# MisEty/RTG-SLAM

Measured on AMD Instinct MI355X. Metric: hot_path_units_per_sec, higher is better.
Workload: dtype f32; 1 GPU; `value` counts UNITS, not SLAM frames (the SLAM frame rate by the reference's definition is `slam_frames_per_sec`, from the `slam_sequence` leg of --full).  One UNIT per step = 1 ICP track (3 levels x 5 GN iters, 1200x680, on a second HIP stream) + 1 map-optimisation iteration (raster fwd + masked L1 colour / gated depth loss + attach regulariser + raster bwd + fused Adam) over 1200000 random Gaus; gaussians=1200000, mode=single, parallelism=1 GPU

## Files before the change

### include/rtgs_raster.h

```cpp
#ifndef RTGS_RASTER_H
#define RTGS_RASTER_H

#include <stddef.h>
#include <stdint.h>

#ifdef __cplusplus
extern "C" {
#endif

#define RTGS_OK 0
#define RTGS_E_INVALID (-1)
#define RTGS_E_HIP (-2)
#define RTGS_E_ALLOC (-3)

#define RTGS_TILE 16

typedef struct rtgs_raster_settings {
  int32_t image_height;
  int32_t image_width;
  float tanfovx;
  float tanfovy;
  const float* bg;
  float scale_modifier;
  const float* viewmatrix;
// ... 100 lines not shown
                                  const int32_t* out_depth_index,
                                  const float* dL_dcolor, const float* dL_ddepth,
                                  float* dL_dmeans3D, float* dL_dopacities, float* dL_dshs,
                                  float* dL_dscales, float* dL_drotations, float* dL_dnormal_w,
                                  void* grad_scratch, uint8_t* row_state, int32_t train_begin, int32_t train_end, void* stream);
int rtgs_raster_backward_walk_ctx(rtgs_ctx* ctx, const rtgs_raster_settings* settings, int32_t P, int32_t sh_coeffs,
                                  int64_t num_rendered,
                                  const float* means3D, const float* opacities, const float* shs,
                                  const float* scales, const float* rotations, const float* normal_w,
                                  void* geom_buffer, void* binning_buffer,
                                  const void* image_buffer, const float* out_color, const float* out_T,
                                  const int32_t* out_depth_index,
                                  const float* dL_dcolor, const float* dL_ddepth,
                                  float* dL_dmeans3D, float* dL_dopacities, float* dL_dshs,
                                  float* dL_dscales, float* dL_drotations, float* dL_dnormal_w,
                                  void* grad_scratch, uint8_t* row_state, int32_t train_begin, int32_t train_end, void* stream);

size_t rtgs_raster_geom_bytes(int32_t P, int32_t image_height, int32_t image_width);
size_t rtgs_raster_geom_bytes_ctx(rtgs_ctx* ctx, int32_t P, int32_t image_height, int32_t image_width);
size_t rtgs_raster_binning_bytes(int64_t num_rendered, int32_t image_height, int32_t image_width);
size_t rtgs_raster_image_bytes(int32_t image_height, int32_t image_width);

int rtgs_raster_last_stats(int64_t* stats8_host);
int rtgs_raster_last_stats_ctx(rtgs_ctx* ctx, int64_t* stats8_host);

int rtgs_raster_last_slice_stats(int64_t* out4_host);
int rtgs_raster_last_slice_stats_ctx(rtgs_ctx* ctx, int64_t* out4_host);
int rtgs_raster_forward_verify_ctx(rtgs_ctx* ctx, int64_t* num_rendered_host);
const uint32_t* rtgs_raster_spec_fail_ptr_ctx(rtgs_ctx* ctx);
void rtgs_raster_set_speculation_ctx(rtgs_ctx* ctx, int enable);
int rtgs_raster_speculation_stats_ctx(rtgs_ctx* ctx, int64_t* out3_host);
void rtgs_raster_set_plain_onepass_ctx(rtgs_ctx* ctx, int enable);
int rtgs_raster_plain_stats_ctx(rtgs_ctx* ctx, int64_t* out2_host);
int rtgs_raster_image_offsets(int32_t image_height, int32_t image_width, size_t* out6_host);

int rtgs_fused_adam(float* params, const float* grads, float* exp_avg, float* exp_avg_sq,
                    const float* lr_per_column, int64_t rows, int32_t cols, int32_t step,
                    float beta1, float beta2, float eps, void* stream);

int rtgs_fused_adam_rows(float* params, const float* grads, float* exp_avg, float* exp_avg_sq,
                         const float* lr_per_column, uint8_t* ever_touched, const uint8_t* row_state, int64_t rows,
                         int32_t cols, int32_t step, float beta1, float beta2, float eps, void* stream);

int rtgs_map_activate8_forward(const float* raw8, int64_t n, float* opacity, float* scales, float* rotations,
                               float* normal, void* stream);
int rtgs_map_activate8_backward(const float* raw8, int64_t n, const float* g_opacity, const float* g_scales,
                                const float* g_rotations, const float* g_normal, float* g_raw8, void* stream);
int rtgs_map_activate8_backward_rows(const float* raw8, int64_t n, const float* g_opacity, const float* g_scales,
                                     const float* g_rotations, const float* g_normal, const uint8_t* row_state,
                                     float* g_raw8, void* stream);

typedef struct rtgs_attach {
  const float* init_xyz;
  const float* init_raw8;
  float* attach_info;
} rtgs_attach;
int rtgs_attach_prepare(const float* xyz, const float* raw8, const rtgs_attach* attach, int64_t rows, void* stream);

int rtgs_history_merge(float* xyz, float* shs, float* raw8, const float* then_xyz, const float* then_shs,
                       const float* then_raw8, const float* conf_then, const float* conf_now, int64_t rows,
                       float max_weight, void* stream);

typedef struct rtgs_activated {
  float *opacity, *scales, *rotations, *normal;
} rtgs_activated;
int rtgs_map_tail_rows(float* xyz, float* shs, float* raw8, const float* g_opacity, const float* g_scales,
                       const float* g_rotations, const float* g_normal, const float* g_xyz, const float* g_shs,
                       float* g_raw8, const uint8_t* row_state, float* m_xyz, float* v_xyz, float* m_shs, float* v_shs,
                       float* m_raw8, float* v_raw8, const float* lr_xyz, const float* lr_shs, const float* lr_raw8,
                       uint8_t* ever_xyz, uint8_t* ever_shs, uint8_t* ever_raw8, int64_t rows, int32_t step, float beta1,
                       float beta2, float eps, const rtgs_attach* attach, float* confidence, const uint32_t* skip_flag,
                       const rtgs_activated* refresh, void* stream);

typedef struct rtgs_loss_cfg {
  float color_weight, depth_weight, ssim_weight, add_depth_thres;
  const uint8_t* render_mask;
  int32_t sums_zeroed;
} rtgs_loss_cfg;
size_t rtgs_slam_loss_scratch_bytes(int32_t H, int32_t W, int32_t with_ssim);
int rtgs_slam_loss(const float* color, const float* depth, const int32_t* depth_index, const float* gt_color,
                   const float* gt_depth, int32_t H, int32_t W, const rtgs_loss_cfg* cfg, void* scratch,
                   float* loss_out4, float* g_color, float* g_depth, void* stream);
int rtgs_slam_loss_sums(const float* color, const float* depth, const int32_t* depth_index, const float* gt_color,
                        const float* gt_depth, int32_t H, int32_t W, const rtgs_loss_cfg* cfg, void* scratch, void* stream);
int rtgs_slam_loss_grads(const float* color, const float* depth, const int32_t* depth_index, const float* gt_color,
                         const float* gt_depth, int32_t H, int32_t W, const rtgs_loss_cfg* cfg, void* scratch,
                         float* loss_out4, float* g_color, float* g_depth, void* stream);

typedef struct rtgs_map_step_args {
  const rtgs_raster_settings* settings;
  int32_t P, sh_coeffs;
  float *xyz, *shs, *raw8;
  const int32_t* tile_mask;
  const float *gt_color, *gt_depth;
  rtgs_loss_cfg loss;
  void* loss_scratch;
  float *opacity, *scales, *rotations, *normal;
  float *out_color, *out_depth;
  int32_t *out_color_index, *out_depth_index;
  float *out_color_weight, *out_depth_weight, *out_T;
  int32_t* out_radii;
  float *dL_dcolor, *dL_ddepth, *loss4;
  float *d_xyz, *d_opacity, *d_shs, *d_scales, *d_rotations, *d_normal, *d_raw8;
  void* grad_scratch;
  uint8_t* row_state;
  float *m_xyz, *v_xyz, *m_shs, *v_shs, *m_raw8, *v_raw8;
  const float *lr_xyz, *lr_shs, *lr_raw8;
  uint8_t *ever_xyz, *ever_shs, *ever_raw8;
  int32_t step;
  float beta1, beta2, eps;
  const rtgs_attach* attach;
  float* confidence;
  int32_t activated_valid;
  rtgs_resize_fn geom_resize; void* geom_user;
  rtgs_resize_fn binning_resize; void* binning_user;
  rtgs_resize_fn image_resize; void* image_user;
  float normal_weight;
  const float* gt_normal;
  int32_t train_begin, train_end;
  int32_t tail_mode;
  uint32_t* live_counts;
} rtgs_map_step_args;
int rtgs_slam_normal_loss(const float* normal_w, const int32_t* depth_index, const float* gt_normal,
                          const uint8_t* render_mask, int32_t H, int32_t W, float normal_weight, float* scratch2,
                          float* loss_out4, float* d_normal, uint8_t* row_state, const uint32_t* skip_flag, void* stream);
int rtgs_slam_normal_loss_range(const float* normal_w, const int32_t* depth_index, const float* gt_normal,
                                const uint8_t* render_mask, int32_t H, int32_t W, float normal_weight, float* scratch2,
                                float* loss_out4, float* d_normal, uint8_t* row_state, const uint32_t* skip_flag,
                                int32_t train_begin, int32_t train_end, void* stream);
int rtgs_slam_normal_loss_sums(const float* normal_w, const int32_t* depth_index, const float* gt_normal,
                               const uint8_t* render_mask, int32_t H, int32_t W, float* scratch2, const uint32_t* skip_flag,
                               void* stream);
int rtgs_slam_normal_loss_grads(const float* normal_w, const int32_t* depth_index, const float* gt_normal,
                                const uint8_t* render_mask, int32_t H, int32_t W, float normal_weight, const float* sums2,
                                float* loss_out4, float* d_normal, uint8_t* row_state, const uint32_t* skip_flag,
                                int32_t train_begin, int32_t train_end, void* stream);
int rtgs_slam_map_step(const rtgs_map_step_args* args, int64_t* num_rendered_host, void* stream);
void* rtgs_stream_create_reserving(int32_t reserve_cus);
void rtgs_stream_destroy(void* stream);
int rtgs_map_fused_tail(const rtgs_raster_settings* settings, const rtgs_map_step_args* args, void* geom_buffer,
                        const void* image_buffer, const uint32_t* spec_fail, uint32_t* live_counts2, void* stream);
int rtgs_map_fused_tail_hint(const rtgs_raster_settings* settings, const rtgs_map_step_args* args, void* geom_buffer,
                             const void* image_buffer, const uint32_t* spec_fail, uint32_t* live_counts2,
                             uint32_t listed_hint, void* stream);
uint32_t rtgs_raster_last_listed_ctx(rtgs_ctx* ctx);
int rtgs_raster_backward_buffers(int32_t P, int32_t image_height, int32_t image_width, size_t* out8_host);
int rtgs_raster_last_buffers_ctx(rtgs_ctx* ctx, void** out3_host);
void rtgs_raster_set_aux_zero_ctx(rtgs_ctx* ctx, void* eight_words);
int rtgs_slam_map_step_front(const rtgs_map_step_args* args, int64_t* num_rendered_host, void* stream);
int rtgs_slam_map_step_ctx(rtgs_ctx* ctx, const rtgs_map_step_args* args, int64_t* num_rendered_host, void* stream);
int rtgs_slam_map_step_front_ctx(rtgs_ctx* ctx, const rtgs_map_step_args* args, int64_t* num_rendered_host, void* stream);

int rtgs_rows_pack(const uint8_t* row_state, int32_t P, float* d_xyz, float* d_shs, float* d_opacity, float* d_scales,
                   float* d_rotations, float* d_normal, float* out_list, int32_t capacity, uint32_t* count_scratch,
                   void* stream);
int rtgs_rows_overflow(const float* gathered_lists, int32_t world, int32_t capacity, uint32_t* flag_and_counts, void* stream);
int rtgs_rows_apply(const float* list, int32_t capacity, int32_t mode, float* d_xyz, float* d_shs, float* d_opacity,
                    float* d_scales, float* d_rotations, float* d_normal, uint8_t* row_state, const uint32_t* skip_flag,
                    void* stream);

size_t rtgs_map_step_args_size(void);
size_t rtgs_raster_settings_size(void);

const char* rtgs_version(void);

#ifdef __cplusplus
}
#endif
#endif
```

### rtg_slam_amd/_lib.py

```python
from __future__ import annotations

import ctypes as C
import os
import threading

_HERE = os.path.dirname(os.path.abspath(__file__))
LIB_PATH = os.environ.get("RTGS_LIB_PATH") or os.path.join(_HERE, "librtgs_hip.so")

RESIZE_FN = C.CFUNCTYPE(C.c_void_p, C.c_void_p, C.c_size_t)
FWD_NO_BACKWARD = 1


class RasterSettingsC(C.Structure):
    _fields_ = [
        ("image_height", C.c_int32), ("image_width", C.c_int32),
        ("tanfovx", C.c_float), ("tanfovy", C.c_float),
        ("bg", C.c_void_p), ("scale_modifier", C.c_float),
        ("viewmatrix", C.c_void_p), ("projmatrix", C.c_void_p),
        ("sh_degree", C.c_int32), ("campos", C.c_void_p),
        ("opaque_threshold", C.c_float), ("depth_threshold", C.c_float),
        ("normal_threshold", C.c_float), ("color_sigma", C.c_float),
        ("prefiltered", C.c_int32), ("debug", C.c_int32),
        ("cx", C.c_float), ("cy", C.c_float), ("T_threshold", C.c_float),
    ]
# ... 12 lines not shown

_P = C.c_void_p


class LossCfgC(C.Structure):
    _fields_ = [("color_weight", C.c_float), ("depth_weight", C.c_float), ("ssim_weight", C.c_float),
                ("add_depth_thres", C.c_float), ("render_mask", C.c_void_p), ("sums_zeroed", C.c_int32)]


class AttachC(C.Structure):
    _fields_ = [("init_xyz", C.c_void_p), ("init_raw8", C.c_void_p), ("attach_info", C.c_void_p)]


class ActivatedC(C.Structure):
    _fields_ = [(n, C.c_void_p) for n in ("opacity", "scales", "rotations", "normal")]


class MapStepArgsC(C.Structure):
    _fields_ = (
        [("settings", C.POINTER(RasterSettingsC)), ("P", C.c_int32), ("sh_coeffs", C.c_int32)]
        + [(n, C.c_void_p) for n in ("xyz", "shs", "raw8", "tile_mask", "gt_color", "gt_depth")]
        + [("loss", LossCfgC), ("loss_scratch", C.c_void_p)]
        + [(n, C.c_void_p) for n in (
            "opacity", "scales", "rotations", "normal", "out_color", "out_depth", "out_color_index", "out_depth_index",
            "out_color_weight", "out_depth_weight", "out_T", "out_radii", "dL_dcolor", "dL_ddepth", "loss4",
            "d_xyz", "d_opacity", "d_shs", "d_scales", "d_rotations", "d_normal", "d_raw8", "grad_scratch", "row_state",
            "m_xyz", "v_xyz", "m_shs", "v_shs", "m_raw8", "v_raw8", "lr_xyz", "lr_shs", "lr_raw8",
            "ever_xyz", "ever_shs", "ever_raw8")]
        + [("step", C.c_int32), ("beta1", C.c_float), ("beta2", C.c_float), ("eps", C.c_float)]
        + [("attach", C.POINTER(AttachC)), ("confidence", C.c_void_p), ("activated_valid", C.c_int32)]
        + [("geom_resize", RESIZE_FN), ("geom_user", C.c_void_p), ("binning_resize", RESIZE_FN),
           ("binning_user", C.c_void_p), ("image_resize", RESIZE_FN), ("image_user", C.c_void_p)]
        + [("normal_weight", C.c_float), ("gt_normal", C.c_void_p), ("train_begin", C.c_int32), ("train_end", C.c_int32),
           ("tail_mode", C.c_int32), ("live_counts", C.c_void_p)])


_SIGNATURES = {
    "rtgs_version": (C.c_char_p, []),
    "rtgs_raster_forward": (C.c_int, [C.POINTER(RasterSettingsC), C.c_int32, C.c_int32] + [_P] * 6 + [_P]
                            + [_P] * 8 + [RESIZE_FN, _P, RESIZE_FN, _P, RESIZE_FN, _P,
                                          C.POINTER(C.c_int64), _P]),
    "rtgs_raster_backward": (C.c_int, [C.POINTER(RasterSettingsC), C.c_int32, C.c_int32, C.c_int64] + [_P] * 6
                             + [_P] * 3 + [_P, _P, _P] + [_P, _P] + [_P] * 6 + [_P, _P]),
    "rtgs_raster_backward_rows": (C.c_int, [C.POINTER(RasterSettingsC), C.c_int32, C.c_int32, C.c_int64] + [_P] * 6
                                  + [_P] * 3 + [_P, _P, _P] + [_P, _P] + [_P] * 6 + [_P, _P, _P]),
    "rtgs_raster_backward_scratch_bytes": (C.c_size_t, [C.c_int32]),
    "rtgs_raster_geom_bytes": (C.c_size_t, [C.c_int32, C.c_int32, C.c_int32]),
    "rtgs_raster_binning_bytes": (C.c_size_t, [C.c_int64, C.c_int32, C.c_int32]),
    "rtgs_raster_image_bytes": (C.c_size_t, [C.c_int32, C.c_int32]),
    "rtgs_raster_last_stats": (C.c_int, [C.POINTER(C.c_int64)]),
    "rtgs_raster_set_counters": (None, [_P]),
    "rtgs_fused_adam": (C.c_int, [_P, _P, _P, _P, _P, C.c_int64, C.c_int32, C.c_int32, C.c_float, C.c_float, C.c_float, _P]),
    "rtgs_fused_adam_rows": (C.c_int, [_P, _P, _P, _P, _P, _P, _P, C.c_int64, C.c_int32, C.c_int32, C.c_float, C.c_float, C.c_float, _P]),
    "rtgs_map_activate8_forward": (C.c_int, [_P, C.c_int64, _P, _P, _P, _P, _P]),
    "rtgs_map_activate8_backward": (C.c_int, [_P, C.c_int64, _P, _P, _P, _P, _P, _P]),
    "rtgs_map_activate8_backward_rows": (C.c_int, [_P, C.c_int64, _P, _P, _P, _P, _P, _P, _P]),
    "rtgs_map_tail_rows": (C.c_int, [_P] * 23 + [C.c_int64, C.c_int32, C.c_float, C.c_float, C.c_float,
                                     C.POINTER(AttachC), _P, _P, C.POINTER(ActivatedC), _P]),
    "rtgs_attach_prepare": (C.c_int, [_P, _P, C.POINTER(AttachC), C.c_int64, _P]),
    "rtgs_history_merge": (C.c_int, [_P] * 8 + [C.c_int64, C.c_float, _P]),
    "rtgs_map_fused_tail": (C.c_int, [C.POINTER(RasterSettingsC), C.POINTER(MapStepArgsC), _P, _P, _P, _P, _P]),
    "rtgs_map_fused_tail_hint": (C.c_int, [C.POINTER(RasterSettingsC), C.POINTER(MapStepArgsC), _P, _P, _P, _P, C.c_uint32, _P]),
    "rtgs_raster_last_listed_ctx": (C.c_uint32, [_P]),
    "rtgs_stream_create_reserving": (C.c_void_p, [C.c_int]),
    "rtgs_stream_destroy": (None, [_P]),
    "rtgs_raster_backward_buffers": (C.c_int, [C.c_int32, C.c_int32, C.c_int32, C.POINTER(C.c_size_t)]),
    "rtgs_raster_last_buffers_ctx": (C.c_int, [_P, C.POINTER(C.c_void_p)]),
    "rtgs_raster_set_aux_zero_ctx": (None, [_P, _P]),
    "rtgs_raster_backward_walk_ctx": (C.c_int, [_P, C.POINTER(RasterSettingsC), C.c_int32, C.c_int32, C.c_int64] + [_P] * 6
                                      + [_P] * 3 + [_P, _P, _P] + [_P, _P] + [_P] * 6 + [_P, _P, C.c_int32, C.c_int32, _P]),
    "rtgs_slam_loss_scratch_bytes": (C.c_size_t, [C.c_int32, C.c_int32, C.c_int32]),
    "rtgs_slam_map_step_front": (C.c_int, [C.POINTER(MapStepArgsC), C.POINTER(C.c_int64), _P]),
    "rtgs_rows_pack": (C.c_int, [_P, C.c_int32] + [_P] * 7 + [C.c_int32, _P, _P]),
    "rtgs_rows_overflow": (C.c_int, [_P, C.c_int32, C.c_int32, _P, _P]),
    "rtgs_rows_apply": (C.c_int, [_P, C.c_int32, C.c_int32] + [_P] * 7 + [_P, _P]),
    "rtgs_map_step_args_size": (C.c_size_t, []),
    "rtgs_raster_settings_size": (C.c_size_t, []),
    "rtgs_slam_map_step": (C.c_int, [C.POINTER(MapStepArgsC), C.POINTER(C.c_int64), _P]),
    "rtgs_slam_loss": (C.c_int, [_P, _P, _P, _P, _P, C.c_int32, C.c_int32, C.POINTER(LossCfgC), _P, _P, _P, _P, _P]),
    "rtgs_slam_normal_loss": (C.c_int, [_P, _P, _P, _P, C.c_int32, C.c_int32, C.c_float, _P, _P, _P, _P, _P, _P]),
    "rtgs_slam_loss_sums": (C.c_int, [_P, _P, _P, _P, _P, C.c_int32, C.c_int32, C.POINTER(LossCfgC), _P, _P]),
    "rtgs_slam_loss_grads": (C.c_int, [_P, _P, _P, _P, _P, C.c_int32, C.c_int32, C.POINTER(LossCfgC), _P, _P, _P, _P, _P]),
    "rtgs_raster_set_profiling": (None, [C.c_int]),
    "rtgs_raster_force_sort_path": (None, [C.c_int]),
    "rtgs_raster_set_near_slice": (None, [C.c_int, C.c_int]),
    "rtgs_raster_last_slice_stats": (C.c_int, [C.POINTER(C.c_int64)]),
    "rtgs_raster_last_timings": (C.c_int, [C.POINTER(C.c_float)]),
    "rtgs_ctx_create": (C.c_void_p, []),
    "rtgs_ctx_destroy": (None, [_P]),
    "rtgs_raster_forward_ctx": (C.c_int, [_P, C.POINTER(RasterSettingsC), C.c_int32, C.c_int32] + [_P] * 6 + [_P]
                                + [_P] * 8 + [RESIZE_FN, _P, RESIZE_FN, _P, RESIZE_FN, _P, C.POINTER(C.c_int64),
                                              C.c_int32, _P]),
    "rtgs_raster_backward_ctx": (C.c_int, [_P, C.POINTER(RasterSettingsC), C.c_int32, C.c_int32, C.c_int64] + [_P] * 6
                                 + [_P] * 3 + [_P, _P, _P] + [_P, _P] + [_P] * 6 + [_P, _P]),
    "rtgs_raster_backward_rows_ctx": (C.c_int, [_P, C.POINTER(RasterSettingsC), C.c_int32, C.c_int32, C.c_int64] + [_P] * 6
                                      + [_P] * 3 + [_P, _P, _P] + [_P, _P] + [_P] * 6 + [_P, _P, _P]),
# ... 141 lines not shown
```

### rtg_slam_amd/csrc/map_fused.hip

```cpp
#include "../../include/rtgs_raster.h"
#include "raster_common.h"
#include "raster_chain.h"
#include "adam_common.h"
#include "activate_common.h"

#include <math.h>

namespace rtgs {

struct FusedArgs {
  RasterParams p;
  const float *opac, *scales, *rots, *normal_w;
  const uint8_t* clamped;
  const BwdInfo* info;
  const uint32_t* gbase;
  uint32_t* slot_count;
  uint8_t* touched;
  SplatGrad* records;
  float *xyz, *shs, *raw8;
  float *m_xyz, *v_xyz, *m_shs, *v_shs, *m_raw8, *v_raw8;
  const float *lr_xyz, *lr_shs, *lr_raw8;
  uint8_t *ever_xyz, *ever_shs, *ever_raw8;
  float beta1, beta2, eps, bc1, bc2_sqrt;
  const float* init_xyz;
  const float4* init_raw8;
  const float* attach_info;
  float* confidence;
  float *act_opacity, *act_scales, *act_normal;
  float4* act_rots;
  uint32_t* live_counts;
  int t0, rows;
};

constexpr int BIG_RUN = 8;

__device__ __forceinline__ bool attach_sel(const float4 init_lo) {
  return 1.f / (1.f + __expf(-init_lo.x)) < 0.9f;
}

template <int FCHUNK, int RPW = 64>
__global__ void __launch_bounds__(256) map_fused_tail_kernel(FusedArgs a) {
  __shared__ uint32_t s_list[FCHUNK];
  __shared__ uint32_t s_n;
  __shared__ float s_big[4][64][16];
  __shared__ float s_sh[4][64][20];
  __shared__ int s_rows[4][64];
  if (spec_failed(a.p.spec_fail)) return;
  const int tid = threadIdx.x, lane = tid & 63, wv = tid >> 6;
  const bool use_slots = a.info->use_slots != 0;
  const float* __restrict__ slots = reinterpret_cast<const float*>(a.info->slot_grads);
  uint32_t n_grad = 0, n_step = 0;
  for (int c0 = blockIdx.x * FCHUNK; c0 < a.rows; c0 += gridDim.x * FCHUNK) {
    __syncthreads();
    if (tid == 0) s_n = 0;
    __syncthreads();
    constexpr int PASSES = FCHUNK >= 256 ? FCHUNK / 256 : 1;
    uint32_t flags = 0;
#pragma unroll
    for (int k = 0; k < PASSES; ++k) {
      const int rl = min(c0 + k * 256 + tid, a.rows - 1);
      const uint32_t f = (uint32_t)a.touched[a.t0 + rl] | (uint32_t)a.ever_raw8[rl] | (uint32_t)a.ever_xyz[rl] | (uint32_t)a.ever_shs[rl];
      flags |= (f != 0u ? 1u : 0u) << k;
    }
// ... 84 lines not shown
      } else if (rgrad) {
        g = a.records[r];
        float4* z = reinterpret_cast<float4*>(a.records + r);
        z[0] = z[1] = z[2] = z[3] = make_float4(0.f, 0.f, 0.f, 0.f);
      }
      if (rgrad) {
        a.touched[r] = 0;
        rgrad = (g.du != 0.f) | (g.dv != 0.f) | (g.dca != 0.f) | (g.dcb != 0.f) | (g.dcc != 0.f) | (g.dop != 0.f) |
                (g.dr != 0.f) | (g.dg != 0.f) | (g.db != 0.f) | (g.dnx != 0.f) | (g.dny != 0.f) | (g.dnz != 0.f) | (g.dpd != 0.f);
      }
      bool need_sh = false;
      if (have) {
        const uint8_t e_raw8 = a.ever_raw8[rl], e_xyz = a.ever_xyz[rl], e_shs = a.ever_shs[rl];
        ChainOut o{};
        if (rgrad) chain_rule(a.p, r, a.xyz, a.shs, a.scales, a.rots, a.normal_w, a.clamped, g, o, nullptr);
        const float4* raw8_4 = reinterpret_cast<const float4*>(a.raw8);
        float4 at_lo = make_float4(0.f, 0.f, 0.f, 0.f), at_hi = at_lo;
        float at[3] = {0.f, 0.f, 0.f};
        bool sel = false;
        if (a.init_raw8 && (rgrad || e_raw8 != 0 || e_xyz != 0)) {
          const float4 i_lo = a.init_raw8[2 * (size_t)rl];
          sel = attach_sel(i_lo);
          if (sel) {
            const float4 i_hi = a.init_raw8[2 * (size_t)rl + 1], c_lo = raw8_4[2 * (size_t)r], c_hi = raw8_4[2 * (size_t)r + 1];
            const float n = fmaxf(a.attach_info[0], 1.f);
            const float k3 = 2000.f / (n * 3.f), k4 = 2000.f / (n * 4.f);
            at_lo = make_float4(0.f, k3 * (c_lo.y - i_lo.y), k3 * (c_lo.z - i_lo.z), k3 * (c_lo.w - i_lo.w));
            at_hi = make_float4(k4 * (c_hi.x - i_hi.x), k4 * (c_hi.y - i_hi.y), k4 * (c_hi.z - i_hi.z), k4 * (c_hi.w - i_hi.w));
#pragma unroll
            for (int c = 0; c < 3; ++c) at[c] = k3 * (a.xyz[(size_t)r * 3 + c] - a.init_xyz[(size_t)rl * 3 + c]);
          }
        }
        const bool grad = rgrad || sel;
        if (grad || e_raw8 != 0) {
          float4 lo = make_float4(0.f, 0.f, 0.f, 0.f), hi = lo;
          if (rgrad)
            activate8_bwd_row(raw8_4[2 * (size_t)r], raw8_4[2 * (size_t)r + 1], o.dop, o.ds[0], o.ds[1], o.ds[2], o.dq, o.dn[0],
                              o.dn[1], o.dn[2], lo, hi);
          lo.y += at_lo.y; lo.z += at_lo.z; lo.w += at_lo.w;
          hi.x += at_hi.x; hi.y += at_hi.y; hi.z += at_hi.z; hi.w += at_hi.w;
          if (e_raw8 == 0) a.ever_raw8[rl] = 1;
          float4* p4 = reinterpret_cast<float4*>(a.raw8) + 2 * (size_t)r;
          float4* m4 = reinterpret_cast<float4*>(a.m_raw8) + 2 * (size_t)rl;
          float4* v4 = reinterpret_cast<float4*>(a.v_raw8) + 2 * (size_t)rl;
          const float gg[8] = {lo.x, lo.y, lo.z, lo.w, hi.x, hi.y, hi.z, hi.w};
          float4 pp[2] = {p4[0], p4[1]}, mm[2] = {m4[0], m4[1]}, vv[2] = {v4[0], v4[1]};
          float* pf = reinterpret_cast<float*>(pp); float* mf = reinterpret_cast<float*>(mm); float* vf = reinterpret_cast<float*>(vv);
#pragma unroll
          for (int c = 0; c < 8; ++c) pf[c] = adam1(pf[c], gg[c], mf[c], vf[c], a.lr_raw8[c], a.beta1, a.beta2, a.eps, a.bc1, a.bc2_sqrt);
          p4[0] = pp[0]; p4[1] = pp[1]; m4[0] = mm[0]; m4[1] = mm[1]; v4[0] = vv[0]; v4[1] = vv[1];
          if (a.act_opacity) activate8_row_store(pp[0], pp[1], r, a.act_opacity, a.act_scales, a.act_rots, a.act_normal);
        }
        if (grad || e_xyz != 0) {
          if (e_xyz == 0) a.ever_xyz[rl] = 1;
#pragma unroll
          for (int c = 0; c < 3; ++c) {
            const size_t op = (size_t)r * 3 + c, os = (size_t)rl * 3 + c;
            float mi = a.m_xyz[os], vi = a.v_xyz[os];
            a.xyz[op] = adam1(a.xyz[op], (rgrad ? o.dm[c] : 0.f) + at[c], mi, vi, a.lr_xyz[c], a.beta1, a.beta2, a.eps, a.bc1, a.bc2_sqrt);
            a.m_xyz[os] = mi; a.v_xyz[os] = vi;
          }
        }
        if (a.confidence && rgrad) {
          if (o.basis[0] * o.gc[0] != 0.f || o.basis[0] * o.gc[1] != 0.f || o.basis[0] * o.gc[2] != 0.f) a.confidence[rl] += 1.f;
        }
        need_sh = rgrad || e_shs != 0;
// ... 30 lines not shown
            gi.w = sh[3 + (c0 + 3) / 3] * sh[(c0 + 3) % 3];
          }
          const float4 pi = reinterpret_cast<const float4*>(a.shs)[op];
          float4 mi = reinterpret_cast<float4*>(a.m_shs)[os], vi = reinterpret_cast<float4*>(a.v_shs)[os], po;
          po.x = adam1(pi.x, gi.x, mi.x, vi.x, a.lr_shs[4 * sub], a.beta1, a.beta2, a.eps, a.bc1, a.bc2_sqrt);
          po.y = adam1(pi.y, gi.y, mi.y, vi.y, a.lr_shs[4 * sub + 1], a.beta1, a.beta2, a.eps, a.bc1, a.bc2_sqrt);
          po.z = adam1(pi.z, gi.z, mi.z, vi.z, a.lr_shs[4 * sub + 2], a.beta1, a.beta2, a.eps, a.bc1, a.bc2_sqrt);
          po.w = adam1(pi.w, gi.w, mi.w, vi.w, a.lr_shs[4 * sub + 3], a.beta1, a.beta2, a.eps, a.bc1, a.bc2_sqrt);
          reinterpret_cast<float4*>(a.shs)[op] = po;
          reinterpret_cast<float4*>(a.m_shs)[os] = mi;
          reinterpret_cast<float4*>(a.v_shs)[os] = vi;
        }
      }
      __builtin_amdgcn_wave_barrier();
    }
  }
  if (a.live_counts) {
#pragma unroll
    for (int off = 32; off > 0; off >>= 1) { n_grad += (uint32_t)__shfl_xor((int)n_grad, off); n_step += (uint32_t)__shfl_xor((int)n_step, off); }
    if (lane == 0 && (n_grad | n_step)) { atomicAdd(&a.live_counts[0], n_grad); atomicAdd(&a.live_counts[1], n_step); }
  }
}

}

extern "C" int rtgs_map_fused_tail(const rtgs_raster_settings* settings, const rtgs_map_step_args* s, void* geom_buffer,
                                   const void* image_buffer, const uint32_t* spec_fail, uint32_t* live_counts2, void* stream) {
  return rtgs_map_fused_tail_hint(settings, s, geom_buffer, image_buffer, spec_fail, live_counts2, 0, stream);
}

extern "C" int rtgs_map_fused_tail_hint(const rtgs_raster_settings* settings, const rtgs_map_step_args* s, void* geom_buffer,
                                        const void* image_buffer, const uint32_t* spec_fail, uint32_t* live_counts2,
                                        uint32_t listed_hint, void* stream) {
  using namespace rtgs;
  if (!settings || !s || !geom_buffer || !image_buffer) return RTGS_E_INVALID;
  const int32_t P = s->P;
  if (P <= 0 || s->sh_coeffs != 16 || s->step < 1) return RTGS_E_INVALID;
  int32_t t0 = 0, t1 = P;
  if (s->train_begin != 0 || s->train_end != 0) { t0 = s->train_begin; t1 = s->train_end; }
  if (t0 < 0 || t1 > P || t1 < t0) return RTGS_E_INVALID;
  if (t1 == t0) return RTGS_OK;
  FusedArgs a{};
  RasterParams& p = a.p;
  p.H = settings->image_height; p.W = settings->image_width;
  p.gx = (p.W + TILE - 1) / TILE; p.gy = (p.H + TILE - 1) / TILE;
  p.P = P; p.M = 16; p.deg = settings->sh_degree;
  p.tanfovx = settings->tanfovx; p.tanfovy = settings->tanfovy;
  p.fx = (float)(p.W / (2.0 * (double)settings->tanfovx));
  p.fy = (float)(p.H / (2.0 * (double)settings->tanfovy));
  p.cx = settings->cx > 0.f ? settings->cx : 0.5f * (float)(p.W - 1);
  p.cy = settings->cy > 0.f ? settings->cy : 0.5f * (float)(p.H - 1);
  p.scale_modifier = settings->scale_modifier;
  p.opaque_thr = settings->opaque_threshold; p.depth_thr = settings->depth_threshold; p.normal_thr = settings->normal_threshold;
  p.color_sigma = settings->color_sigma; p.T_thr = settings->T_threshold;
  p.view = settings->viewmatrix; p.campos = settings->campos; p.bg = settings->bg;
  p.spec_fail = spec_fail;
  size_t off[8];
  if (rtgs_raster_backward_buffers(P, p.H, p.W, off) != RTGS_OK) return RTGS_E_INVALID;
  const char* geom = (const char*)geom_buffer;
  const char* img = (const char*)image_buffer;
  a.opac = s->opacity; a.scales = s->scales; a.rots = s->rotations; a.normal_w = s->normal;
  a.clamped = (const uint8_t*)(geom + off[0]);
  a.gbase = (const uint32_t*)(geom + off[1]);
  a.slot_count = (uint32_t*)(geom + off[2]);
  a.info = (const BwdInfo*)(img + off[3]);
  a.records = (SplatGrad*)s->grad_scratch;
  a.touched = (uint8_t*)s->grad_scratch + off[4];
  a.xyz = s->xyz; a.shs = s->shs; a.raw8 = s->raw8;
  a.m_xyz = s->m_xyz; a.v_xyz = s->v_xyz; a.m_shs = s->m_shs; a.v_shs = s->v_shs; a.m_raw8 = s->m_raw8; a.v_raw8 = s->v_raw8;
  a.lr_xyz = s->lr_xyz; a.lr_shs = s->lr_shs; a.lr_raw8 = s->lr_raw8;
  a.ever_xyz = s->ever_xyz; a.ever_shs = s->ever_shs; a.ever_raw8 = s->ever_raw8;
  a.beta1 = s->beta1; a.beta2 = s->beta2; a.eps = s->eps;
  a.bc1 = 1.f - powf(s->beta1, (float)s->step);
  a.bc2_sqrt = sqrtf(1.f - powf(s->beta2, (float)s->step));
  if (s->attach) {
    if (!s->attach->init_xyz || !s->attach->init_raw8 || !s->attach->attach_info) return RTGS_E_INVALID;
    a.init_xyz = s->attach->init_xyz; a.init_raw8 = (const float4*)s->attach->init_raw8; a.attach_info = s->attach->attach_info;
  }
  a.confidence = s->confidence;
  a.act_opacity = s->opacity; a.act_scales = s->scales; a.act_normal = s->normal; a.act_rots = (float4*)s->rotations;
  a.live_counts = live_counts2;
  a.t0 = t0; a.rows = t1 - t0;
  static const int forced = [] { const char* e = getenv("RTGS_FUSED_CHUNK"); return e ? atoi(e) : 0; }();
  int chunk = 1024;
  if (forced == 512 || forced == 1024 || forced == 2048) chunk = forced;
  else if (listed_hint > 0u) {
    const double per_row = (double)listed_hint / (double)(P > 0 ? P : 1);
    chunk = per_row * 2048.0 <= 64.0 ? 2048 : (per_row * 1024.0 <= 64.0 ? 1024 : 512);
  }
  if (forced == 64 || (forced == 0 && a.rows <= 65536)) chunk = 64;
  int blocks = (a.rows + chunk - 1) / chunk;
  if (blocks > 4096) blocks = 4096;
  if (chunk == 64) hipLaunchKernelGGL((map_fused_tail_kernel<64, 16>), dim3(blocks), dim3(256), 0, (hipStream_t)stream, a);
  else if (chunk == 2048) hipLaunchKernelGGL(map_fused_tail_kernel<2048>, dim3(blocks), dim3(256), 0, (hipStream_t)stream, a);
  else if (chunk == 512) hipLaunchKernelGGL(map_fused_tail_kernel<512>, dim3(blocks), dim3(256), 0, (hipStream_t)stream, a);
  else hipLaunchKernelGGL(map_fused_tail_kernel<1024>, dim3(blocks), dim3(256), 0, (hipStream_t)stream, a);
  return hipGetLastError() == hipSuccess ? RTGS_OK : RTGS_E_HIP;
}
```

### rtg_slam_amd/csrc/map_ops.hip

```cpp
#include "../../include/rtgs_raster.h"
#include <hip/hip_runtime.h>
#include <math.h>
#include <stdint.h>
#include "adam_common.h"
#include "activate_common.h"


namespace rtgs {

__global__ void __launch_bounds__(256) activate8_fwd_kernel(const float4* __restrict__ raw8, int64_t n,
                                                            float* __restrict__ opacity, float* __restrict__ scales,
                                                            float4* __restrict__ rots, float* __restrict__ normal) {
  for (int64_t i = (int64_t)blockIdx.x * blockDim.x + threadIdx.x; i < n; i += (int64_t)gridDim.x * blockDim.x)
    activate8_row_store(raw8[2 * i], raw8[2 * i + 1], i, opacity, scales, rots, normal);
}

__global__ void __launch_bounds__(256) activate8_bwd_kernel(const float4* __restrict__ raw8, int64_t n,
                                                            const float* __restrict__ g_op, const float* __restrict__ g_sc,
                                                            const float4* __restrict__ g_rot, const float* __restrict__ g_nrm,
                                                            const uint8_t* __restrict__ row_state,
                                                            float4* __restrict__ g_raw8) {
  for (int64_t i = (int64_t)blockIdx.x * blockDim.x + threadIdx.x; i < n; i += (int64_t)gridDim.x * blockDim.x) {
    if (row_state) {
      const uint8_t s = row_state[i];
// ... 37 lines not shown
                                                const float* g_rotations, const float* g_normal, const uint8_t* row_state,
                                                float* g_raw8, void* stream) {
  if (n < 0 || (n > 0 && (!raw8 || !g_opacity || !g_scales || !g_rotations || !g_normal || !row_state || !g_raw8))) return -1;
  if (n == 0) return 0;
  int64_t blocks = (n + 255) / 256;
  if (blocks > 8192) blocks = 8192;
  hipLaunchKernelGGL(rtgs::activate8_bwd_kernel, dim3((unsigned)blocks), dim3(256), 0, (hipStream_t)stream,
                     (const float4*)raw8, n, g_opacity, g_scales, (const float4*)g_rotations, g_normal, row_state,
                     (float4*)g_raw8);
  return hipGetLastError() == hipSuccess ? 0 : -2;
}

namespace rtgs {

struct TailArgs {
  const float4* raw8_in;
  float *xyz, *shs, *raw8;
  const float *g_op, *g_sc, *g_nrm, *g_xyz, *g_shs;
  const float4* g_rot;
  float4* g_raw8;
  const uint8_t* row_state;
  float *m_xyz, *v_xyz, *m_shs, *v_shs, *m_raw8, *v_raw8;
  const float *lr_xyz, *lr_shs, *lr_raw8;
  uint8_t *ever_xyz, *ever_shs, *ever_raw8;
  long long rows;
  float beta1, beta2, eps, bc1, bc2_sqrt;
  const float* init_xyz;
  const float4* init_raw8;
  const float* attach_info;
  float* confidence;
  const uint32_t* skip_flag;
  float *act_opacity, *act_scales, *act_normal;
  float4* act_rots;
};

__device__ __forceinline__ bool attach_selected(const float4 init_lo) {
  return 1.f / (1.f + __expf(-init_lo.x)) < 0.9f;
}

__global__ void __launch_bounds__(256) map_tail_rows_kernel(TailArgs a) {
  __shared__ int s_rows[4][64];
  if (a.skip_flag && a.skip_flag[0] != 0u) return;
  const int lane = threadIdx.x & 63, wv = threadIdx.x >> 6;
  const long long wave0 = (long long)blockIdx.x * 4 + wv, nwaves = (long long)gridDim.x * 4;
  for (long long base = wave0 * 64; base < a.rows; base += nwaves * 64) {
    const long long r = base + lane;
    bool need_sh = false, has_grad = false;
    if (r < a.rows) {
      const uint8_t st = a.row_state[r];
      const uint8_t e_raw8 = a.ever_raw8[r], e_xyz = a.ever_xyz[r], e_shs = a.ever_shs[r];
      const bool rgrad = st == 1;
      has_grad = rgrad;
      float4 at_lo = make_float4(0.f, 0.f, 0.f, 0.f), at_hi = at_lo;
      float at_x = 0.f, at_y = 0.f, at_z = 0.f;
      bool sel = false;
      if (a.init_raw8 && (rgrad || e_raw8 != 0 || e_xyz != 0)) {
        const float4 i_lo = a.init_raw8[2 * r];
        sel = attach_selected(i_lo);
        if (sel) {
          const float4 i_hi = a.init_raw8[2 * r + 1], c_lo = a.raw8_in[2 * r], c_hi = a.raw8_in[2 * r + 1];
          const float n = fmaxf(a.attach_info[0], 1.f);
          const float k3 = 2000.f / (n * 3.f), k4 = 2000.f / (n * 4.f);
          at_lo = make_float4(0.f, k3 * (c_lo.y - i_lo.y), k3 * (c_lo.z - i_lo.z), k3 * (c_lo.w - i_lo.w));
          at_hi = make_float4(k4 * (c_hi.x - i_hi.x), k4 * (c_hi.y - i_hi.y), k4 * (c_hi.z - i_hi.z), k4 * (c_hi.w - i_hi.w));
          at_x = k3 * (a.xyz[(size_t)r * 3] - a.init_xyz[(size_t)r * 3]);
          at_y = k3 * (a.xyz[(size_t)r * 3 + 1] - a.init_xyz[(size_t)r * 3 + 1]);
          at_z = k3 * (a.xyz[(size_t)r * 3 + 2] - a.init_xyz[(size_t)r * 3 + 2]);
        }
      }
      const bool grad = rgrad || sel;
      float4 lo = make_float4(0.f, 0.f, 0.f, 0.f), hi = lo;
      if (st != 0 || sel) {
        if (rgrad)
          activate8_bwd_row(a.raw8_in[2 * r], a.raw8_in[2 * r + 1], a.g_op[r], a.g_sc[r * 3], a.g_sc[r * 3 + 1],
                            a.g_sc[r * 3 + 2], a.g_rot[r], a.g_nrm[r * 3], a.g_nrm[r * 3 + 1], a.g_nrm[r * 3 + 2], lo, hi);
        lo.y += at_lo.y; lo.z += at_lo.z; lo.w += at_lo.w;
        hi.x += at_hi.x; hi.y += at_hi.y; hi.z += at_hi.z; hi.w += at_hi.w;
        a.g_raw8[2 * r] = lo; a.g_raw8[2 * r + 1] = hi;
      }
      if (grad || e_raw8 != 0) {
        if (e_raw8 == 0) a.ever_raw8[r] = 1;
        const float4 g0 = lo, g1 = hi;
        float4* p4 = reinterpret_cast<float4*>(a.raw8) + 2 * r;
        float4* m4 = reinterpret_cast<float4*>(a.m_raw8) + 2 * r;
        float4* v4 = reinterpret_cast<float4*>(a.v_raw8) + 2 * r;
        const float gg[8] = {g0.x, g0.y, g0.z, g0.w, g1.x, g1.y, g1.z, g1.w};
        float4 pp[2] = {p4[0], p4[1]}, mm[2] = {m4[0], m4[1]}, vv[2] = {v4[0], v4[1]};
        float* pf = reinterpret_cast<float*>(pp); float* mf = reinterpret_cast<float*>(mm); float* vf = reinterpret_cast<float*>(vv);
#pragma unroll
        for (int c = 0; c < 8; ++c) pf[c] = adam1(pf[c], gg[c], mf[c], vf[c], a.lr_raw8[c], a.beta1, a.beta2, a.eps, a.bc1, a.bc2_sqrt);
        p4[0] = pp[0]; p4[1] = pp[1]; m4[0] = mm[0]; m4[1] = mm[1]; v4[0] = vv[0]; v4[1] = vv[1];
        if (a.act_opacity) activate8_row_store(pp[0], pp[1], r, a.act_opacity, a.act_scales, a.act_rots, a.act_normal);
      }
      if (grad || e_xyz != 0) {
        if (e_xyz == 0) a.ever_xyz[r] = 1;
        const float at[3] = {at_x, at_y, at_z};
#pragma unroll
        for (int c = 0; c < 3; ++c) {
          const size_t o = (size_t)r * 3 + c;
          float mi = a.m_xyz[o], vi = a.v_xyz[o];
          a.xyz[o] = adam1(a.xyz[o], (rgrad ? a.g_xyz[o] : 0.f) + at[c], mi, vi, a.lr_xyz[c], a.beta1, a.beta2, a.eps, a.bc1, a.bc2_sqrt);
          a.m_xyz[o] = mi; a.v_xyz[o] = vi;
        }
      }
      if (a.confidence && rgrad) {
        const size_t o = (size_t)r * 48;
        if (a.g_shs[o] != 0.f || a.g_shs[o + 1] != 0.f || a.g_shs[o + 2] != 0.f) a.confidence[r] += 1.f;
      }
      need_sh = rgrad || e_shs != 0;
      if (need_sh && e_shs == 0) a.ever_shs[r] = 1;
    }
    const unsigned long long mask = __builtin_amdgcn_ballot_w64(need_sh);
// ... 121 lines not shown
  if (!xyz || !shs || !raw8 || !then_xyz || !then_shs || !then_raw8 || !conf_then || !conf_now) return -1;
  long long blocks = (rows + 255) / 256;
  if (blocks > 8192) blocks = 8192;
  hipLaunchKernelGGL(rtgs::history_merge_kernel, dim3((unsigned)blocks), dim3(256), 0, (hipStream_t)stream, xyz, (float4*)shs,
                     (float4*)raw8, then_xyz, (const float4*)then_shs, (const float4*)then_raw8, conf_then, conf_now,
                     (long long)rows, max_weight);
  return hipGetLastError() == hipSuccess ? 0 : -2;
}

extern "C" int rtgs_attach_prepare(const float* xyz, const float* raw8, const rtgs_attach* attach, int64_t rows, void* stream) {
  if (!attach || !attach->init_xyz || !attach->init_raw8 || !attach->attach_info || rows < 0) return -1;
  if (rows > 0 && (!xyz || !raw8)) return -1;
  hipStream_t st = (hipStream_t)stream;
  float* info = attach->attach_info;
  if (hipMemsetAsync(info, 0, 6 * sizeof(float), st) != hipSuccess) return -2;
  if (rows > 0) {
    long long blocks = (rows + 255) / 256;
    if (blocks > 192) blocks = 192;
    hipLaunchKernelGGL(rtgs::attach_sums_kernel, dim3((unsigned)blocks), dim3(256), 0, st, xyz, (const float4*)raw8,
                       attach->init_xyz, (const float4*)attach->init_raw8, (long long)rows, info + 2);
  }
  hipLaunchKernelGGL(rtgs::attach_finish_kernel, dim3(1), dim3(1), 0, st, (const float*)(info + 2), info);
  return hipGetLastError() == hipSuccess ? 0 : -2;
}

extern "C" int rtgs_map_tail_rows(float* xyz, float* shs, float* raw8, const float* g_opacity, const float* g_scales,
                                  const float* g_rotations, const float* g_normal, const float* g_xyz, const float* g_shs,
                                  float* g_raw8, const uint8_t* row_state, float* m_xyz, float* v_xyz, float* m_shs,
                                  float* v_shs, float* m_raw8, float* v_raw8, const float* lr_xyz, const float* lr_shs,
                                  const float* lr_raw8, uint8_t* ever_xyz, uint8_t* ever_shs, uint8_t* ever_raw8,
                                  int64_t rows, int32_t step, float beta1, float beta2, float eps,
                                  const rtgs_attach* attach, float* confidence, const uint32_t* skip_flag,
                                  const rtgs_activated* refresh, void* stream) {
  if (rows < 0 || step < 1) return -1;
  if (rows == 0) return 0;
  if (!xyz || !shs || !raw8 || !g_opacity || !g_scales || !g_rotations || !g_normal || !g_xyz || !g_shs || !g_raw8 ||
      !row_state || !m_xyz || !v_xyz || !m_shs || !v_shs || !m_raw8 || !v_raw8 || !lr_xyz || !lr_shs || !lr_raw8 ||
      !ever_xyz || !ever_shs || !ever_raw8)
    return -1;
  rtgs::TailArgs a;
  a.raw8_in = (const float4*)raw8; a.xyz = xyz; a.shs = shs; a.raw8 = raw8;
  a.g_op = g_opacity; a.g_sc = g_scales; a.g_nrm = g_normal; a.g_xyz = g_xyz; a.g_shs = g_shs;
  a.g_rot = (const float4*)g_rotations; a.g_raw8 = (float4*)g_raw8; a.row_state = row_state;
  a.m_xyz = m_xyz; a.v_xyz = v_xyz; a.m_shs = m_shs; a.v_shs = v_shs; a.m_raw8 = m_raw8; a.v_raw8 = v_raw8;
  a.lr_xyz = lr_xyz; a.lr_shs = lr_shs; a.lr_raw8 = lr_raw8;
  a.ever_xyz = ever_xyz; a.ever_shs = ever_shs; a.ever_raw8 = ever_raw8;
  a.rows = rows; a.beta1 = beta1; a.beta2 = beta2; a.eps = eps;
  a.init_xyz = nullptr; a.init_raw8 = nullptr; a.attach_info = nullptr; a.confidence = confidence;
  a.skip_flag = skip_flag;
  a.act_opacity = a.act_scales = a.act_normal = nullptr; a.act_rots = nullptr;
  if (refresh) {
    if (!refresh->opacity || !refresh->scales || !refresh->rotations || !refresh->normal) return -1;
    a.act_opacity = refresh->opacity; a.act_scales = refresh->scales; a.act_normal = refresh->normal;
    a.act_rots = (float4*)refresh->rotations;
  }
  if (attach) {
    if (!attach->init_xyz || !attach->init_raw8 || !attach->attach_info) return -1;
    a.init_xyz = attach->init_xyz; a.init_raw8 = (const float4*)attach->init_raw8; a.attach_info = attach->attach_info;
  }
  a.bc1 = 1.f - powf(beta1, (float)step);
  a.bc2_sqrt = sqrtf(1.f - powf(beta2, (float)step));
  long long blocks = (rows + 255) / 256;
  if (blocks > 16384) blocks = 16384;
  hipLaunchKernelGGL(rtgs::map_tail_rows_kernel, dim3((unsigned)blocks), dim3(256), 0, (hipStream_t)stream, a);
  return hipGetLastError() == hipSuccess ? 0 : -2;
}

namespace rtgs {

constexpr int PACK_CHUNK = 8192;
constexpr int ROW_WORDS = 64;

struct ArenaPtrs {
  float *d_xyz, *d_shs, *d_opac, *d_scales, *d_rots, *d_normal;
};
__device__ __forceinline__ float* arena_word(const ArenaPtrs& a, uint32_t id, int w) {
  if (w < 4) return a.d_xyz + (size_t)id * 3 + (w - 1);
  if (w < 52) return a.d_shs + (size_t)id * 48 + (w - 4);
  if (w < 53) return a.d_opac + id;
  if (w < 56) return a.d_scales + (size_t)id * 3 + (w - 53);
  if (w < 60) return a.d_rots + (size_t)id * 4 + (w - 56);
  return a.d_normal + (size_t)id * 3 + (w - 60);
// ... 515 lines not shown
```

### rtg_slam_amd/csrc/map_step.hip

```cpp
#include <hip/hip_runtime.h>

#include "../../include/rtgs_raster.h"

static int map_step_front(rtgs_ctx* ctx, const rtgs_map_step_args* a, int64_t* num_rendered_host, int32_t fwd_flags,
                          void* stream, bool walk_only = false) {
  if (!a || !num_rendered_host || !a->settings) return RTGS_E_INVALID;
  const int32_t P = a->P, M = a->sh_coeffs;
  if (P <= 0 || M != 16 || a->step < 1) return RTGS_E_INVALID;
  if (!a->xyz || !a->shs || !a->raw8 || !a->tile_mask || !a->gt_color || !a->gt_depth) return RTGS_E_INVALID;
  const int32_t H = a->settings->image_height, W = a->settings->image_width;
  int rc = 0;
  if (!a->activated_valid) {
    rc = rtgs_map_activate8_forward(a->raw8, P, a->opacity, a->scales, a->rotations, a->normal, stream);
    if (rc != 0) return RTGS_E_HIP;
  }
  if (!a->loss_scratch || !a->loss4) return RTGS_E_INVALID;
  rtgs_raster_set_aux_zero_ctx(ctx, a->loss_scratch);
  rc = rtgs_raster_forward_ctx(ctx, a->settings, P, M, a->xyz, a->opacity, a->shs, a->scales, a->rotations, a->normal,
                           a->tile_mask, a->out_color, a->out_depth, a->out_color_index, a->out_depth_index,
                           a->out_color_weight, a->out_depth_weight, a->out_T, a->out_radii, a->geom_resize,
                           a->geom_user, a->binning_resize, a->binning_user, a->image_resize, a->image_user,
                           num_rendered_host, fwd_flags, stream);
  if (rc != RTGS_OK) return rc;
  void* bufs[3];
// ... 3 lines not shown
  lcfg.sums_zeroed = P > 0 ? 1 : 0;
  rc = rtgs_slam_loss(a->out_color, a->out_depth, a->out_depth_index, a->gt_color, a->gt_depth, H, W, &lcfg,
                      a->loss_scratch, a->loss4, a->dL_dcolor, a->dL_ddepth, stream);
  if (rc != 0) return RTGS_E_HIP;
  int32_t t0 = 0, t1 = P;
  if (a->train_begin != 0 || a->train_end != 0) { t0 = a->train_begin; t1 = a->train_end; }
  if (t0 < 0 || t1 > P || t1 < t0) return RTGS_E_INVALID;
  if (t1 == t0) return RTGS_OK;
  rc = (walk_only ? rtgs_raster_backward_walk_ctx : rtgs_raster_backward_range_ctx)(
      ctx, a->settings, P, M, *num_rendered_host, a->xyz, a->opacity, a->shs, a->scales, a->rotations, a->normal, geom, bin, img,
      a->out_color, a->out_T, a->out_depth_index, a->dL_dcolor, a->dL_ddepth, a->d_xyz, a->d_opacity, a->d_shs, a->d_scales,
      a->d_rotations, a->d_normal, a->grad_scratch, a->row_state, t0, t1, stream);
  if (rc != RTGS_OK) return rc;
  if (a->normal_weight > 0.f && a->gt_normal) {
    rc = rtgs_slam_normal_loss_range(a->normal, a->out_depth_index, a->gt_normal, a->loss.render_mask, H, W, a->normal_weight,
                                     reinterpret_cast<float*>(a->loss_scratch) + 5, a->loss4, a->d_normal, a->row_state,
                                     rtgs_raster_spec_fail_ptr_ctx(ctx), t0, t1, stream);
    if (rc != 0) return RTGS_E_HIP;
  }
  return RTGS_OK;
}

extern "C" int rtgs_slam_map_step_front_ctx(rtgs_ctx* ctx, const rtgs_map_step_args* a, int64_t* num_rendered_host,
                                            void* stream) {
  return map_step_front(ctx, a, num_rendered_host, 0, stream);
}

extern "C" int rtgs_slam_map_step_front(const rtgs_map_step_args* a, int64_t* num_rendered_host, void* stream) {
  return rtgs_slam_map_step_front_ctx(nullptr, a, num_rendered_host, stream);
}

static int map_step_once(rtgs_ctx* ctx, const rtgs_map_step_args* a, int64_t* num_rendered_host, bool speculate, void* stream) {
  const bool fused = a->tail_mode == 0 && !(a->normal_weight > 0.f && a->gt_normal);
  int rc = map_step_front(ctx, a, num_rendered_host, speculate ? RTGS_FWD_SPECULATE : 0, stream, fused);
  if (rc != RTGS_OK) return rc;
  if ((a->train_begin != 0 || a->train_end != 0) && a->train_end == a->train_begin) return RTGS_OK;
  if (fused) {
    void* bufs[3];
    if (rtgs_raster_last_buffers_ctx(ctx, bufs) != RTGS_OK) return RTGS_E_ALLOC;
    return rtgs_map_fused_tail_hint(a->settings, a, bufs[0], bufs[2], rtgs_raster_spec_fail_ptr_ctx(ctx), a->live_counts,
                                    rtgs_raster_last_listed_ctx(ctx), stream);
  }
  const int32_t P = a->P;
  int32_t t0 = 0, t1 = P;
  if (a->train_begin != 0 || a->train_end != 0) { t0 = a->train_begin; t1 = a->train_end; }
  const size_t o = (size_t)t0;
  const rtgs_activated act{a->opacity + o, a->scales + 3 * o, a->rotations + 4 * o, a->normal + 3 * o};
  rc = rtgs_map_tail_rows(a->xyz + 3 * o, a->shs + 48 * o, a->raw8 + 8 * o, a->d_opacity + o, a->d_scales + 3 * o,
                          a->d_rotations + 4 * o, a->d_normal + 3 * o, a->d_xyz + 3 * o, a->d_shs + 48 * o, a->d_raw8 + 8 * o,
                          a->row_state + o, a->m_xyz, a->v_xyz, a->m_shs, a->v_shs, a->m_raw8, a->v_raw8,
                          a->lr_xyz, a->lr_shs, a->lr_raw8, a->ever_xyz, a->ever_shs, a->ever_raw8, (int64_t)(t1 - t0), a->step,
                          a->beta1, a->beta2, a->eps, a->attach, a->confidence, rtgs_raster_spec_fail_ptr_ctx(ctx), &act, stream);
  return rc != 0 ? RTGS_E_HIP : RTGS_OK;
}

extern "C" int rtgs_slam_map_step_ctx(rtgs_ctx* ctx, const rtgs_map_step_args* a, int64_t* num_rendered_host, void* stream) {
  int rc = map_step_once(ctx, a, num_rendered_host, true, stream);
  const int v = rtgs_raster_forward_verify_ctx(ctx, num_rendered_host);
  if (rc != RTGS_OK) return rc;
  if (v < 0) return v;
  if (v == 1) rc = map_step_once(ctx, a, num_rendered_host, false, stream);
  return rc;
}

extern "C" int rtgs_slam_map_step(const rtgs_map_step_args* a, int64_t* num_rendered_host, void* stream) {
  return rtgs_slam_map_step_ctx(nullptr, a, num_rendered_host, stream);
}

extern "C" size_t rtgs_map_step_args_size(void) { return sizeof(rtgs_map_step_args); }
extern "C" size_t rtgs_raster_settings_size(void) { return sizeof(rtgs_raster_settings); }

extern "C" void* rtgs_stream_create_reserving(int32_t reserve_cus) {
  int dev = 0, cus = 0;
  if (hipGetDevice(&dev) != hipSuccess) return nullptr;
  if (hipDeviceGetAttribute(&cus, hipDeviceAttributeMultiprocessorCount, dev) != hipSuccess) return nullptr;
  if (reserve_cus <= 0 || reserve_cus >= cus || cus > 1024) return nullptr;
  uint32_t mask[32] = {0};
  const int words = (cus + 31) / 32;
  for (int i = 0; i < cus - reserve_cus; ++i) mask[i >> 5] |= 1u << (i & 31);
  hipStream_t s = nullptr;
  if (hipExtStreamCreateWithCUMask(&s, (uint32_t)words, mask) != hipSuccess) return nullptr;
  return (void*)s;
}
extern "C" void rtgs_stream_destroy(void* stream) {
  if (stream) (void)hipStreamDestroy((hipStream_t)stream);
// ... 2 lines not shown
```

### rtg_slam_amd/csrc/raster_api.hip

```cpp
#include "../../include/rtgs_raster.h"
#include "../../include/rtgs_debug.h"
#include "raster_common.h"

#include <rocprim/device/device_radix_sort.hpp>
#include <rocprim/device/device_scan.hpp>
#include <math.h>
#include <new>
#include <stdlib.h>
#include <string.h>

namespace rtgs {
void launch_mask_sat(const int32_t*, int, int, int32_t*, hipStream_t);
void launch_preprocess_fwd(const RasterParams&, const float*, const float*, const float*, const float*, const float*,
                           const float*, const int32_t*, Splat*, uint32_t*, int32_t*, uint8_t*, int32_t*, uint32_t*, int,
                           uint8_t*, hipStream_t);
void launch_emit_keys(const RasterParams&, const Splat*, const int32_t*, const uint32_t*, const int32_t*, uint64_t*,
                      uint32_t*, hipStream_t);
void launch_tile_ranges(int64_t, const uint64_t*, uint2*, hipStream_t);
void set_fwd_stamps(void* dev);
void set_bwd_debug(int bits);
void set_bwd_stamps(void* dev);
void launch_blend_fwd(const RasterParams&, const uint2*, const uint32_t*, const Splat*, float*, float*, int32_t*,
                      int32_t*, float*, float*, float*, uint32_t*, unsigned long long*, SlicePass, uint32_t*, uint32_t*, uint32_t*, int, uint32_t*,
                      TileCache, uint32_t, hipStream_t);
void launch_blend_bwd(const RasterParams&, const uint2*, const uint32_t*, const Splat*, const float*, const float*,
                      const uint32_t*, const int32_t*, const float*, const float*, const uint32_t*, uint32_t*,
                      const BwdInfo*, SplatGrad*, uint8_t*, const uint32_t*, int, uint32_t, uint32_t, hipStream_t);
void launch_blend_bwd_entry(const RasterParams&, const uint2*, const uint32_t*, const Splat*, const float*, const uint32_t*,
                            const int32_t*, const uint32_t*, const uint32_t*, const float*, const float*, const uint32_t*, uint32_t*,
                            const BwdInfo*, SplatGrad*, uint8_t*, const uint32_t*, uint32_t, uint32_t, TileCache, uint32_t, hipStream_t);
void launch_grad_reduce(int, const uint8_t*, const uint32_t*, uint32_t*, const BwdInfo*, SplatGrad*, const uint32_t*, hipStream_t);
void launch_preprocess_bwd(const RasterParams&, const float*, const float*, const float*, const float*, const float*,
                           const float*, const int32_t*, const uint8_t*, SplatGrad*, uint8_t*, uint8_t*, float*, float*,
                           float*, float*, float*, float*, hipStream_t);

size_t bin_lds_limit_tiles();
int bin_sort_capacity();
size_t bin_block_counts_bytes(int, int);
int launch_bin_count(const RasterParams&, const Splat*, const int32_t*, const int32_t*, uint32_t*, uint16_t*, SliceSel,
                     SliceList, size_t, hipStream_t);
size_t bin_slice_block_counts_bytes(int, size_t, int);
size_t bin_list_block_counts_bytes(int, int);
void launch_visible_compact(int, const uint8_t*, uint32_t*, uint32_t*, const uint32_t*, uint32_t*, uint32_t*, const uint32_t*, hipStream_t,
                            const SliceSel* = nullptr, int32_t* = nullptr, uint32_t* = nullptr);
void launch_slice_compact(int, SliceSel, uint32_t*, uint32_t*, const uint32_t*, uint32_t*, uint32_t*, uint32_t*, uint32_t, uint32_t*, hipStream_t);
void launch_slice_publish(int, const int32_t*, const int32_t*, const uint32_t*, uint32_t*, uint32_t*, uint32_t, uint32_t*, hipStream_t,
                          const uint32_t* seg_count = nullptr);
void launch_preprocess_cull(const RasterParams&, const float*, const float*, const float*, uint32_t*, int32_t*, int32_t*,
                            uint32_t*, int, uint8_t*, float2*, hipStream_t);
void launch_preprocess_shade(const RasterParams&, const float*, const float*, const float*, const float*, const float*,
                             const float*, Splat*, int32_t*, uint8_t*, float2*, SliceList, SliceSel, size_t, hipStream_t);
void launch_bin_tilescan(int, const uint32_t*, uint2*, uint32_t*, uint32_t*, uint32_t*, const uint32_t*, const uint32_t*,
                         const uint32_t*, const uint32_t*, uint32_t, SpecCaps, hipStream_t);
void launch_bin_scatter(const RasterParams&, const Splat*, const int32_t*, const int32_t*, const uint16_t*, uint32_t*,
                        unsigned long long*, SliceSel, SliceList, size_t, hipStream_t);
void launch_slice_hist(int, const uint8_t*, const uint32_t*, const int32_t*, uint32_t*, unsigned long long*, hipStream_t,
                       BwdInfoInit bi = BwdInfoInit{nullptr, nullptr, 0u, 0u});
void launch_bin_tilesort(int, uint32_t, const uint2*, const unsigned long long*, uint32_t*, const uint32_t*, hipStream_t,
                         const uint32_t* seg_count = nullptr, uint32_t seg = 0, uint2* ranges_out = nullptr,
                         const BinFinish* finish = nullptr);
void launch_bin_place(const RasterParams&, const Splat*, const int32_t*, const int32_t*, uint32_t*, unsigned long long*, uint32_t,
                      uint32_t*, SliceSel, SliceList, size_t, hipStream_t);

}

enum { EV_F0 = 0, EV_PRE, EV_SL_BIN, EV_SL_BLEND, EV_SCAN, EV_BIN0, EV_EMIT, EV_SORT, EV_RANGES, EV_BLEND0, EV_BLEND, EV_B0,
       EV_BWALK, EV_BBLEND, EV_BPRE, EV_N };
struct rtgs_ctx {
  int64_t stats[8] = {0};
  int slice_mode = 2;
  int slice_budget = 384;
  int64_t slice_stats[4] = {0};
  unsigned long long* counters = nullptr;
  uint32_t last_listed = 0;
  bool onepass = true;
  bool prof = false;
  bool force_sort_path = false;
  int bwd_walk = 0;
  bool ev_init = false;
  hipEvent_t ev[EV_N];
  bool ev_set[EV_N] = {false};
  uint32_t* info_host = nullptr;
// ... 4 lines not shown
  void *last_geom = nullptr, *last_bin = nullptr, *last_img = nullptr;
  uint32_t* aux_zero = nullptr;
  bool ask_first = false;
  struct Plan {
    bool valid = false;
    int32_t P = 0, H = 0, W = 0;
    int kind = -1;
    int slice_mode = 0, slice_budget = 0;
    uint32_t R = 0, R1 = 0, longest = 0, slots = 0, n_fin = 0;
    uint32_t R_hi = 0, longest_hi = 0, slots_hi = 0;
    void note(uint32_t r, uint32_t l, uint32_t s) {
      R = r; longest = l; slots = s;
      R_hi = r > R_hi - R_hi / 16 ? r : R_hi - R_hi / 16;
      longest_hi = l > longest_hi - longest_hi / 16 ? l : longest_hi - longest_hi / 16;
      slots_hi = s > slots_hi - slots_hi / 16 ? s : slots_hi - slots_hi / 16;
    }
  } plan;
  struct Spec {
    bool pending = false;
    int kind = -1;
    uint32_t seq = 0, capR = 0, capL = 0, capS = 0;
    const void* geom = nullptr;
    const uint32_t* fail_dev = nullptr;
    void* stream = nullptr;
    int32_t ntiles = 0;
    int64_t G_total = 0, B_total = 0, I_total = 0;
  } spec;
  bool speculation = true;
  int64_t spec_stats[3] = {0, 0, 0};
  Plan plan_plain;
  Plan plan_plain0;
  bool plain_onepass = true;
  int64_t plain_stats[2] = {0, 0};
};

namespace rtgs {

static rtgs_ctx* default_ctx() {
  static rtgs_ctx* c = [] {
    rtgs_ctx* n = new rtgs_ctx();
    if (const char* e = getenv("RTGS_NEAR_SLICE")) n->slice_mode = atoi(e);
    if (const char* e = getenv("RTGS_NEAR_SLICE_BUDGET")) { const int b = atoi(e); if (b > 0) n->slice_budget = b; }
    if (const char* e = getenv("RTGS_SPECULATE")) n->speculation = atoi(e) != 0;
    if (const char* e = getenv("RTGS_BIN_ONEPASS")) n->onepass = atoi(e) != 0;
    if (const char* e = getenv("RTGS_PLAIN_ONEPASS")) n->plain_onepass = atoi(e) != 0;
    if (const char* e = getenv("RTGS_BWD_WALK")) { const int m = atoi(e); n->bwd_walk = (m >= 1 && m <= 4) ? m : 0; }
    return n;
  }();
  return c;
}
static inline rtgs_ctx* use(rtgs_ctx* c) { return c ? c : default_ctx(); }

static void prof_mark(rtgs_ctx* c, int which, hipStream_t st) {
  if (!c->prof) return;
  if (!c->ev_init) {
    for (int i = 0; i < EV_N; ++i) (void)hipEventCreate(&c->ev[i]);
    c->ev_init = true;
  }
  (void)hipEventRecord(c->ev[which], st);
  c->ev_set[which] = true;
}

static int bits_for(uint32_t n) {
  int b = 0;
  while ((1ull << b) < (unsigned long long)n) ++b;
  return b < 1 ? 1 : b;
}

static int wait_published_words(uint32_t* info_host, uint32_t seq, hipStream_t st, uint32_t (&pub)[7]) {
  volatile uint32_t* h = info_host;
  auto snapshot_ok = [&]() -> bool {
    if (h[7] != seq) return false;
    __atomic_thread_fence(__ATOMIC_ACQUIRE);
    uint32_t w[7];
    for (int k = 0; k < 7; ++k) w[k] = h[k];
    if (h[8] != host_checksum(seq, w)) return false;
    for (int k = 0; k < 7; ++k) pub[k] = w[k];
    return true;
  };
// ... 11 lines not shown
  for (uint32_t c : classes) if (want <= c) return c;
  return 16384u;
}

__global__ void bwd_info_kernel(BwdInfo* dst, SplatGrad* slot_grads, uint32_t slots, uint32_t use_slots) {
  dst->slot_grads = slot_grads; dst->slots = slots; dst->use_slots = use_slots;
}

static int large_map_min() {
  static const int v = [] { const char* e = getenv("RTGS_LARGE_MAP_MIN"); const int x = e ? atoi(e) : 100000; return x > 0 ? x : 100000; }();
  return v;
}

static GeomLayout geom_layout(int32_t P, int gx, int gy, int budget) {
  GeomLayout L{};
  size_t off = 0;
  const size_t Pn = (size_t)(P > 0 ? P : 1);
  L.splats = off; off = align_up(off + Pn * sizeof(Splat));
  L.tiles_touched = off; off = align_up(off + Pn * sizeof(uint32_t));
  L.offsets = off; off = align_up(off + Pn * sizeof(uint32_t));
  L.radii = off; off = align_up(off + Pn * sizeof(int32_t));
  L.clamped = off; off = align_up(off + Pn);
  L.sat = off; off = align_up(off + (size_t)(gx + 1) * (gy + 1) * sizeof(int32_t));
  L.tile_count = off; off = align_up(off + (size_t)gx * gy * sizeof(uint32_t));
  L.cursor = off; off = align_up(off + (size_t)gx * gy * sizeof(uint32_t));
  L.info = off; off = align_up(off + 4 * sizeof(uint32_t));
  L.block_counts = off; off = align_up(off + bin_block_counts_bytes((int)Pn, gx * gy));
  {
    const size_t nt = (size_t)gx * gy;
    L.zero_begin = L.tile_count;
    off = L.tile_count + nt * sizeof(uint32_t);
    L.tile_count1 = off; off += nt * sizeof(uint32_t);
    L.ranges1_bwd = off; off += nt * sizeof(uint2);
    L.slice_hist = off; off += 2 * SLICE_BINS * sizeof(uint32_t);
    L.slice_cover = off; off += SLICE_BINS * sizeof(unsigned long long);
    L.slice_ctr = off; off += 8 * sizeof(uint32_t);
    L.slot_count = off; off += Pn * sizeof(uint32_t);
    L.zero_end = off; off = align_up(off);
    L.cursor = off; off = align_up(off + nt * sizeof(uint32_t));
    L.info = off; off = align_up(off + 4 * sizeof(uint32_t));
    L.block_counts = off; off = align_up(off + bin_block_counts_bytes((int)Pn, gx * gy));
    L.zbin = off; off = align_up(off + Pn);
    L.cursor1 = off; off = align_up(off + nt * sizeof(uint32_t));
    L.ranges1 = off; off = align_up(off + nt * sizeof(uint2));
    L.mask2 = off; off = align_up(off + nt * sizeof(int32_t));
    L.uv = off; off = align_up(off + Pn * sizeof(float2));
    L.slice_cap = nt * (size_t)(budget > 0 ? budget : 1);
    L.slice_max_list = L.slice_cap < 65536 ? L.slice_cap : 65536;
    if (L.slice_max_list > Pn) L.slice_max_list = Pn;
    L.vis_ids = off; off = align_up(off + Pn * sizeof(uint32_t));
    L.block_counts_vis = off; off = align_up(off + bin_list_block_counts_bytes((int)Pn, gx * gy));
    L.slice_seg = (Pn >= (size_t)large_map_min() && nt >= 256) ? (size_t)SLICE_MAX_LIST : 0;
    const size_t cap1 = L.slice_seg ? (nt * L.slice_seg > L.slice_cap ? nt * L.slice_seg : L.slice_cap) : L.slice_cap;
    L.list1 = off; off = align_up(off + cap1 * sizeof(uint32_t));
    L.block_counts1 = off; off = align_up(off + bin_slice_block_counts_bytes((int)Pn, L.slice_max_list, gx * gy));
    L.slice_ids = off; off = align_up(off + L.slice_max_list * sizeof(uint32_t));
    L.bucket1 = off; off = align_up(off + cap1 * sizeof(uint64_t));
  }
  size_t tb = 0, tb2 = 0;
  (void)rocprim::inclusive_scan(nullptr, tb, (uint32_t*)nullptr, (uint32_t*)nullptr, Pn, rocprim::plus<uint32_t>());
  (void)rocprim::exclusive_scan(nullptr, tb2, (uint32_t*)nullptr, (uint32_t*)nullptr, 0u, Pn, rocprim::plus<uint32_t>());
  if (tb2 > tb) tb = tb2;
  L.scan_temp_bytes = tb;
  L.scan_temp = off; off = align_up(off + tb);
  L.total = off;
  return L;
}

static BinLayout bin_layout(int64_t R, int ntiles, bool sort_path, size_t slots) {
  BinLayout L{};
  size_t off = 0;
  const size_t Rn = (size_t)(R > 0 ? R : 1);
  L.vals_b = off; off = align_up(off + Rn * sizeof(uint32_t));
  L.keys_a = off; off = align_up(off + Rn * sizeof(uint64_t));
  if (!sort_path) {
    L.keys_b = L.vals_a = L.sort_temp = off; L.sort_temp_bytes = 0;
    if (slots > 0) { L.slot_grads = off; off = align_up(off + slots * sizeof(SplatGrad)); }
    L.total = off;
    return L;
// ... 45 lines not shown
  p.spec_fail = nullptr;
  return RTGS_OK;
}

#define HIP_TRY(expr)                         \
  do {                                        \
    hipError_t e_ = (expr);                   \
    if (e_ != hipSuccess) return RTGS_E_HIP;  \
  } while (0)

static int dbg_sync(const rtgs_raster_settings* s, hipStream_t st) {
  if (s->debug) {
    HIP_TRY(hipStreamSynchronize(st));
    HIP_TRY(hipGetLastError());
  }
  return RTGS_OK;
}
#define DBG(s, st)                              \
  do {                                          \
    int r_ = dbg_sync(s, st);                   \
    if (r_ != RTGS_OK) return r_;               \
  } while (0)

}

using namespace rtgs;

extern "C" {

const char* rtgs_version(void) { return "rtgs-hip 0.2.0 (gfx950)"; }

rtgs_ctx* rtgs_ctx_create(void) {
  rtgs_ctx* c = new (std::nothrow) rtgs_ctx();
  if (c) { c->slice_mode = default_ctx()->slice_mode; c->slice_budget = default_ctx()->slice_budget; c->bwd_walk = default_ctx()->bwd_walk; c->onepass = default_ctx()->onepass; c->speculation = default_ctx()->speculation; c->plain_onepass = default_ctx()->plain_onepass; }
  return c;
}
void rtgs_ctx_destroy(rtgs_ctx* c) {
  if (!c || c == default_ctx()) return;
  if (c->ev_init) for (int i = 0; i < EV_N; ++i) (void)hipEventDestroy(c->ev[i]);
  if (c->info_host) (void)hipHostFree(c->info_host);
  delete c;
}

size_t rtgs_raster_geom_bytes_ctx(rtgs_ctx* c, int32_t P, int32_t H, int32_t W) {
  return geom_layout(P, (W + TILE - 1) / TILE, (H + TILE - 1) / TILE, use(c)->slice_budget).total;
}
size_t rtgs_raster_geom_bytes(int32_t P, int32_t H, int32_t W) { return rtgs_raster_geom_bytes_ctx(nullptr, P, H, W); }
size_t rtgs_raster_binning_bytes(int64_t R, int32_t H, int32_t W) {
  const int gx = (W + TILE - 1) / TILE, gy = (H + TILE - 1) / TILE;
  return bin_layout(R, gx * gy, true, 0).total;
}
size_t rtgs_raster_image_bytes(int32_t H, int32_t W) {
  const int gx = (W + TILE - 1) / TILE, gy = (H + TILE - 1) / TILE;
  return img_layout(H, W, gx * gy).total;
}
size_t rtgs_raster_backward_scratch_bytes(int32_t P) {
  const size_t n = (size_t)(P > 0 ? P : 1);
  return align_up(n * sizeof(SplatGrad)) + align_up(n);
}

int rtgs_raster_last_stats_ctx(rtgs_ctx* c, int64_t* out) {
  if (!out) return RTGS_E_INVALID;
  memcpy(out, use(c)->stats, sizeof(use(c)->stats));
  return RTGS_OK;
}
void rtgs_raster_set_counters_ctx(rtgs_ctx* c, void* counters) { use(c)->counters = (unsigned long long*)counters; }

int rtgs_raster_forward_ctx(rtgs_ctx* ctx, const rtgs_raster_settings* s, int32_t P, int32_t M, const float* means3D,
                            const float* opacities, const float* shs, const float* scales, const float* rotations,
                            const float* normal_w, const int32_t* tile_mask, float* out_color, float* out_depth,
                            int32_t* out_cidx, int32_t* out_didx, float* out_cw, float* out_dw, float* out_T,
                            int32_t* out_radii, rtgs_resize_fn geom_resize, void* geom_user,
                            rtgs_resize_fn binning_resize, void* binning_user, rtgs_resize_fn image_resize,
                            void* image_user, int64_t* num_rendered_host, int32_t flags, void* stream) {
  rtgs_ctx* c = use(ctx);
  uint32_t* const aux_zero = c->aux_zero;
  c->aux_zero = nullptr;
  RasterParams p;
  int rc = make_params(s, P, M, p);
  if (rc != RTGS_OK) return rc;
  if (P > 0 && (!means3D || !opacities || !shs || !scales || !rotations || !normal_w)) return RTGS_E_INVALID;
  if (!tile_mask || !out_color || !out_depth || !out_cidx || !out_didx || !out_cw || !out_dw || !out_T)
    return RTGS_E_INVALID;
  if (!geom_resize || !binning_resize || !image_resize || !num_rendered_host) return RTGS_E_INVALID;
  hipStream_t st = (hipStream_t)stream;
  const int ntiles = p.gx * p.gy;

  const GeomLayout G = geom_layout(P, p.gx, p.gy, c->slice_budget);
  char* geom = (char*)geom_resize(geom_user, G.total);
  const ImgLayout I = img_layout(p.H, p.W, ntiles);
  char* img = (char*)image_resize(image_user, I.total);
  if (!geom || !img) return RTGS_E_ALLOC;
  Splat* splats = (Splat*)(geom + G.splats);
  uint32_t* tiles_touched = (uint32_t*)(geom + G.tiles_touched);
  uint32_t* offsets = (uint32_t*)(geom + G.offsets);
  int32_t* radii = (int32_t*)(geom + G.radii);
  uint8_t* clamped = (uint8_t*)(geom + G.clamped);
  int32_t* sat = (int32_t*)(geom + G.sat);
  uint2* ranges = (uint2*)(img + I.ranges);
  uint32_t* n_contrib = (uint32_t*)(img + I.n_contrib);
  uint32_t* depth_pos = (uint32_t*)(img + I.depth_pos);
  uint32_t* tile_last = (uint32_t*)(img + I.tile_last);
  uint32_t* const tile_mode = (uint32_t*)(img + I.tile_mode);
  const int fwd_walk = c->bwd_walk == 0 || c->bwd_walk == 3 ? 2 : (c->bwd_walk == 4 ? -1 : c->bwd_walk - 1);
  c->last_geom = geom; c->last_img = img; c->last_bin = nullptr;
  const TileCache tcache = (flags & RTGS_FWD_NO_BACKWARD) ? TileCache{nullptr, nullptr, nullptr}
                                                          : TileCache{(float4*)(img + I.tile_recs), (uint16_t*)(img + I.tile_masks), (float2*)(img + I.depth_aux)};

  int64_t R = 0, R1 = 0;
  for (int i = 0; i < EV_B0; ++i) c->ev_set[i] = false;
// ... 32 lines not shown
  if (!c->info_host) {
    HIP_TRY(hipHostMalloc((void**)&c->info_host, HOST_WORDS * sizeof(uint32_t), hipHostMallocCoherent));
    memset(c->info_host, 0, HOST_WORDS * sizeof(uint32_t));
  }
  uint32_t* const info_host = c->info_host;
  uint32_t pub[7] = {0, 0, 0, 0, 0, 0, 0};
  auto wait_published = [&](uint32_t seq) -> int { return wait_published_words(info_host, seq, st, pub); };
  const int32_t* mask_main = tile_mask;
  uint32_t n_left = 0, n_fin = 0;

  if (c->spec.pending) return RTGS_E_INVALID;
  c->spec.geom = nullptr; c->spec.fail_dev = nullptr;
  {
    rtgs_ctx::Plan& pp = sliced ? c->plan_plain : c->plan_plain0;
    const bool immediate = !(flags & RTGS_FWD_SPECULATE) && !want_bwd && c->speculation && c->plain_onepass && c->onepass &&
                           P > 0 && !sort_path && !s->debug && pp.valid && (sliced ? (pp.kind == 2 && G.slice_seg) : pp.kind == 0) &&
                           pp.H == p.H && pp.W == p.W && pp.slice_mode == c->slice_mode && pp.slice_budget == c->slice_budget;
    const rtgs_ctx::Plan& pl = immediate ? pp : c->plan;
    const bool eligible = immediate ||
                          ((flags & RTGS_FWD_SPECULATE) && c->speculation && want_bwd && P > 0 && !sort_path && !s->debug &&
                           pl.valid && pl.P == P && pl.H == p.H && pl.W == p.W && pl.slice_mode == c->slice_mode &&
                           pl.slice_budget == c->slice_budget && (pl.kind == 0 ? !sliced : (pl.kind == 1 || pl.kind == 2) && sliced));
    const uint32_t capR = pl.R_hi + pl.R_hi / 8u + 8192u, capL = sort_class_cap(pl.longest_hi),
                   capS = immediate ? 0u : pl.slots_hi + pl.slots_hi / 8u + 8192u;
    if ((flags & RTGS_FWD_SPECULATE) && !(eligible && (pl.kind == 1 || capS <= SLOTS_MAX))) ++c->spec_stats[2];
    if (eligible && (pl.kind == 1 || capS <= SLOTS_MAX)) {
      uint32_t* const fail = slice_ctr + 6;
      const SliceSel sel1{1, zbin, slice_hist, (uint32_t)G.slice_cap, (uint32_t)G.slice_max_list, slice_ctr, nullptr, nullptr,
                          slice_cover, (uint32_t)ntiles * (uint32_t)(TILE * TILE), slice_auto ? 1 : 0};
      const SpecCaps nocaps{nullptr, 0u, 0u, 0u, nullptr};
      if (++c->seq == 0u) c->seq = 1u;
      size_t b_total = 0;
      bool seg_main = false;
      if (pl.kind == 1) {
        launch_preprocess_cull(p, means3D, scales, rotations, tiles_touched, radii, out_radii, zero_words, zero_n, zbin,
                               (float2*)(geom + G.uv), st);
        prof_mark(c, EV_PRE, st);
        const uint32_t sl = (uint32_t)G.slice_cap;
        const bool use_sl = sl > 0 && sl <= SLOTS_MAX;
        const BinLayout B = bin_layout(0, ntiles, false, use_sl ? (size_t)sl : 0);
        char* bin = (char*)binning_resize(binning_user, B.total);
        if (!bin) return RTGS_E_ALLOC;
        c->last_bin = bin;
        b_total = B.total;
        launch_slice_hist(P, zbin, tiles_touched, radii, slice_hist, slice_cover, st,
                          BwdInfoInit{(BwdInfo*)(img + I.bwd_info), (SplatGrad*)(bin + B.slot_grads), use_sl ? sl : 0u, use_sl ? 1u : 0u});
        launch_slice_compact(P, sel1, (uint32_t*)(geom + G.slice_ids), slice_ctr + 2, tiles_touched, offsets, slice_ctr + 4,
                             nullptr, 0u, nullptr, st);
        const SliceList work{(const uint32_t*)(geom + G.slice_ids), slice_ctr + 2};
        launch_preprocess_shade(p, means3D, opacities, shs, scales, rotations, normal_w, splats, radii, clamped,
                                (float2*)(geom + G.uv), work, sel1, G.slice_max_list, st);
        if (seg1) {
          launch_bin_place(p, splats, radii, tile_mask, tile_count1, (unsigned long long*)(geom + G.bucket1), seg1, nullptr,
                           sel1, work, G.slice_max_list, st);
          launch_bin_tilesort(ntiles, (uint32_t)SLICE_MAX_LIST, ranges1, (const unsigned long long*)(geom + G.bucket1), list1,
                              nullptr, st, tile_count1, seg1, ranges1);
        } else {
        if (launch_bin_count(p, splats, radii, tile_mask, tile_count1, (uint16_t*)(geom + G.block_counts1), sel1, work,
                             G.slice_max_list, st) != 0)
          return RTGS_E_HIP;
        launch_bin_tilescan(ntiles, tile_count1, ranges1, (uint32_t*)(geom + G.cursor1), info + 2, nullptr, nullptr,
                            nullptr, nullptr, nullptr, 0u, nocaps, st);
        launch_bin_scatter(p, splats, radii, tile_mask, (const uint16_t*)(geom + G.block_counts1),
                           (uint32_t*)(geom + G.cursor1), (unsigned long long*)(geom + G.bucket1), sel1, work,
                           G.slice_max_list, st);
        launch_bin_tilesort(ntiles, (uint32_t)SLICE_MAX_LIST, ranges1, (const unsigned long long*)(geom + G.bucket1), list1,
                            nullptr, st);
        }
        prof_mark(c, EV_SL_BIN, st);
        const SlicePass pass1{1, tile_mask, mask2, ranges1_bwd, ranges};
        launch_blend_fwd(p, ranges1, list1, splats, out_color, out_depth, out_cidx, out_didx, out_cw, out_dw, out_T,
                         n_contrib, c->counters, pass1, tile_mode, depth_pos, tile_last, fwd_walk, aux_zero, tcache, seg1, st);
        prof_mark(c, EV_SL_BLEND, st);
        launch_slice_publish(ntiles, tile_mask, mask2, info + 2, slice_ctr, info_host, c->seq, fail, st, seg1 ? tile_count1 : nullptr);
        prof_mark(c, EV_BLEND0, st); prof_mark(c, EV_BLEND, st);
        c->hint_slice_lists = true; c->hint_main_lists = false;
        c->slice_stats[0] = 1; c->slice_stats[1] = pl.R1; c->slice_stats[2] = pl.n_fin; c->slice_stats[3] = 0;
      } else {
        const uint32_t seg2 = (c->onepass && ((pl.kind == 2 && G.slice_seg) || (immediate && pl.kind == 0))) ? capL : 0u;
        const BinLayout B = bin_layout(seg2 ? (int64_t)ntiles * (int64_t)seg2 : (int64_t)capR, ntiles, false, (size_t)capS);
        seg_main = seg2 != 0u;
        char* bin = (char*)binning_resize(binning_user, B.total);
        if (!bin) return RTGS_E_ALLOC;
        c->last_bin = bin;
        b_total = B.total;
        RasterParams pg = p;
        pg.spec_fail = fail;
        SliceList vl{nullptr, nullptr};
        if (pl.kind == 2) {
          launch_preprocess_cull(p, means3D, scales, rotations, tiles_touched, radii, out_radii, zero_words, zero_n, zbin,
                                 (float2*)(geom + G.uv), st);
          prof_mark(c, EV_PRE, st);
          launch_slice_hist(P, zbin, tiles_touched, radii, slice_hist, slice_cover, st,
                            BwdInfoInit{(BwdInfo*)(img + I.bwd_info), (SplatGrad*)(bin + B.slot_grads), capS, immediate ? 0u : 1u});
          vl = SliceList{(const uint32_t*)(geom + G.vis_ids), slice_ctr + 4};
          launch_visible_compact(P, zbin, (uint32_t*)(geom + G.vis_ids), slice_ctr + 4, tiles_touched, offsets, slice_ctr + 5, fail, st,
                                 &sel1, (int32_t*)(slice_ctr + 3), fail);
          launch_preprocess_shade(pg, means3D, opacities, shs, scales, rotations, normal_w, splats, radii, clamped,
                                  (float2*)(geom + G.uv), vl, sel1, (size_t)P, st);
        } else {
          launch_preprocess_fwd(p, means3D, opacities, shs, scales, rotations, normal_w, nullptr, splats, tiles_touched, radii,
                                clamped, out_radii, zero_words, zero_n, nullptr, st);
          if (!immediate && (rc = scan_all()) != RTGS_OK) return rc;
          prof_mark(c, EV_PRE, st);
        }
        const SliceSel sel2{0, nullptr, nullptr, 0u, 0u, slice_ctr, nullptr, (const float2*)(geom + G.uv), nullptr, 0u, 0};
        if (seg2) {
          if (pl.kind != 2)
            hipLaunchKernelGGL(bwd_info_kernel, dim3(1), dim3(1), 0, st, (BwdInfo*)(img + I.bwd_info),
                               (SplatGrad*)(bin + B.slot_grads), capS, immediate ? 0u : 1u);
          launch_bin_place(pg, splats, radii, tile_mask, tile_count, (unsigned long long*)(bin + B.keys_a), seg2, fail, sel2, vl,
                           (size_t)P, st);
          prof_mark(c, EV_SCAN, st); prof_mark(c, EV_BIN0, st); prof_mark(c, EV_EMIT, st);
          const BinFinish fin{tile_count, ntiles, info, info_host, slice_ctr + 5, nullptr, slice_ctr + 4, c->seq,
                              SpecCaps{fail, 0xffffffffu, capL, immediate ? 0xffffffffu : capS,
                                       pl.kind == 2 ? (const int32_t*)(slice_ctr + 3) : nullptr}};
          launch_bin_tilesort(ntiles, capL, ranges, (const unsigned long long*)(bin + B.keys_a), (uint32_t*)(bin + B.vals_b), fail, st,
                              tile_count, seg2, ranges, &fin);
        } else {
        if (launch_bin_count(pg, splats, radii, tile_mask, tile_count, vl.ids ? (uint16_t*)(geom + G.block_counts_vis) : block_counts,
                             sel2, vl, (size_t)P, st) != 0)
          return RTGS_E_HIP;
        const SpecCaps caps{fail, capR, capL, immediate ? 0xffffffffu : capS, pl.kind == 2 ? (const int32_t*)(slice_ctr + 3) : nullptr};
        launch_bin_tilescan(ntiles, tile_count, ranges, cursor, info, info_host, nullptr, nullptr,
                            vl.ids ? slice_ctr + 5 : offsets + (P - 1), vl.ids ? nullptr : tiles_touched + (P - 1), c->seq, caps, st);
        prof_mark(c, EV_SCAN, st);
        if (pl.kind != 2)
// ... 27 lines not shown
          c->stats[0] = (int64_t)pub[0]; c->stats[1] = 32 + bits_for((uint32_t)ntiles); c->stats[2] = ntiles;
          c->stats[3] = (int64_t)G.total; c->stats[4] = (int64_t)b_total; c->stats[5] = (int64_t)I.total; c->stats[6] = 1;
          c->stats[7] = (int64_t)pub[1];
          *num_rendered_host = (int64_t)pub[0];
          return RTGS_OK;
        }
        pp.valid = false;
        ++c->plain_stats[1];
      } else {
      c->spec.pending = true; c->spec.kind = pl.kind; c->spec.seq = c->seq; c->spec.capR = seg_main ? 0xffffffffu : capR; c->spec.capL = capL;
      c->spec.capS = capS; c->spec.geom = geom; c->spec.fail_dev = fail; c->spec.stream = stream; c->spec.ntiles = ntiles;
      c->spec.G_total = (int64_t)G.total; c->spec.B_total = (int64_t)b_total; c->spec.I_total = (int64_t)I.total;
      ++c->spec_stats[0];
      *num_rendered_host = (int64_t)pl.R + (int64_t)pl.R1;
      if (*num_rendered_host < 1) *num_rendered_host = 1;
      return RTGS_OK;
      }
    }
  }
  if (P == 0) HIP_TRY(hipMemsetAsync(zero_words, 0, (size_t)zero_n * sizeof(uint32_t), st));
  if (P > 0) {
    if (sort_path) {
      launch_mask_sat(tile_mask, p.gx, p.gy, sat, st);
      DBG(s, st);
    }
    const SliceSel sel1{1, zbin, slice_hist, (uint32_t)G.slice_cap, (uint32_t)G.slice_max_list, slice_ctr, nullptr, nullptr,
                        slice_cover, (uint32_t)ntiles * (uint32_t)(TILE * TILE), slice_auto ? 1 : 0};
    if (!sliced) {
      launch_preprocess_fwd(p, means3D, opacities, shs, scales, rotations, normal_w, sort_path ? sat : nullptr, splats,
                            tiles_touched, radii, clamped, out_radii, zero_words, zero_n, nullptr, st);
      if (!sort_path && want_bwd && (rc = scan_all()) != RTGS_OK) return rc;
    } else {
      launch_preprocess_cull(p, means3D, scales, rotations, tiles_touched, radii, out_radii, zero_words, zero_n, zbin,
                             (float2*)(geom + G.uv), st);
    }
    DBG(s, st);
    prof_mark(c, EV_PRE, st);
    if (sliced) {
      launch_slice_hist(P, zbin, tiles_touched, radii, slice_hist, slice_cover, st);
      const bool ask = slice_auto && c->ask_first;
      if (ask && ++c->seq == 0u) c->seq = 1u;
      launch_slice_compact(P, sel1, (uint32_t*)(geom + G.slice_ids), slice_ctr + 2, tiles_touched, offsets, slice_ctr + 4,
                           ask ? info_host : nullptr, c->seq, nullptr, st);
      if (ask) {
        if ((rc = wait_published(c->seq)) != RTGS_OK) return rc;
        declined = (int32_t)pub[6] < 0;
      }
    }
    if (sliced && declined) {
      vis = SliceList{(const uint32_t*)(geom + G.vis_ids), slice_ctr + 4};
      launch_visible_compact(P, zbin, (uint32_t*)(geom + G.vis_ids), slice_ctr + 4, tiles_touched, offsets, slice_ctr + 5, nullptr, st);
      launch_preprocess_shade(p, means3D, opacities, shs, scales, rotations, normal_w, splats, radii, clamped,
                              (float2*)(geom + G.uv), vis, sel1, (size_t)P, st);
      sliced = false;
      considered = true;
    }
    if (sliced) {
      const SliceList work{(const uint32_t*)(geom + G.slice_ids), slice_ctr + 2};
      launch_preprocess_shade(p, means3D, opacities, shs, scales, rotations, normal_w, splats, radii, clamped,
                              (float2*)(geom + G.uv), work, sel1, G.slice_max_list, st);
      if (seg1) {
        launch_bin_place(p, splats, radii, tile_mask, tile_count1, (unsigned long long*)(geom + G.bucket1), seg1, nullptr,
                         sel1, work, G.slice_max_list, st);
        launch_bin_tilesort(ntiles, (uint32_t)SLICE_MAX_LIST, ranges1, (const unsigned long long*)(geom + G.bucket1), list1,
                            nullptr, st, tile_count1, seg1, ranges1);
      } else {
      if (launch_bin_count(p, splats, radii, tile_mask, tile_count1, (uint16_t*)(geom + G.block_counts1), sel1, work,
// ... 269 lines not shown
                                   const float* rotations, const float* normal_w, void* geom_buffer,
                                   void* binning_buffer, const void* image_buffer, const float* out_color,
                                   const float* out_T, const int32_t* out_didx, const float* dL_dcolor,
                                   const float* dL_ddepth, float* dL_dmeans3D, float* dL_dopacities, float* dL_dshs,
                                   float* dL_dscales, float* dL_drotations, float* dL_dnormal_w, void* grad_scratch,
                                   uint8_t* row_state, int32_t train_begin, int32_t train_end, void* stream) {
  return backward_impl(ctx, s, P, M, R, means3D, opacities, shs, scales, rotations, normal_w, geom_buffer, binning_buffer,
                       image_buffer, out_color, out_T, out_didx, dL_dcolor, dL_ddepth, dL_dmeans3D, dL_dopacities,
                       dL_dshs, dL_dscales, dL_drotations, dL_dnormal_w, grad_scratch, row_state, train_begin, train_end, stream, true);
}

void rtgs_raster_set_profiling_ctx(rtgs_ctx* c, int enable) { use(c)->prof = enable != 0; }
void rtgs_raster_set_near_slice_ctx(rtgs_ctx* c, int mode, int budget_per_tile) {
  use(c)->slice_mode = mode;
  if (budget_per_tile > 0) use(c)->slice_budget = budget_per_tile;
}
int rtgs_raster_last_slice_stats_ctx(rtgs_ctx* c, int64_t* out) {
  if (!out) return RTGS_E_INVALID;
  memcpy(out, use(c)->slice_stats, sizeof(use(c)->slice_stats));
  return RTGS_OK;
}
void rtgs_raster_force_sort_path_ctx(rtgs_ctx* c, int enable) { use(c)->force_sort_path = enable != 0; }
int rtgs_raster_forward_verify_ctx(rtgs_ctx* ctx, int64_t* num_rendered_host) {
  rtgs_ctx* c = use(ctx);
  if (!c->spec.pending) return 0;
  c->spec.pending = false;
  uint32_t pub[7] = {0, 0, 0, 0, 0, 0, 0};
  const int rc = wait_published_words(c->info_host, c->spec.seq, (hipStream_t)c->spec.stream, pub);
  if (rc != RTGS_OK) { c->plan.valid = false; return rc; }
  rtgs_ctx::Plan& pl = c->plan;
  bool ok;
  if (c->spec.kind == 1) {
    const uint32_t n_left = pub[2];
    ok = n_left == 0u;
    pl.R1 = pub[4]; pl.n_fin = pub[3]; pl.R = 0; pl.longest = 0;
    c->last_listed = pub[0];
    c->slice_stats[1] = pub[4]; c->slice_stats[2] = pub[3]; c->slice_stats[3] = n_left;
  } else {
    ok = pub[0] <= c->spec.capR && pub[1] <= c->spec.capL && pub[5] <= c->spec.capS && (c->spec.kind != 2 || (int32_t)pub[6] < 0);
    pl.note(pub[0], pub[1], pub[5]); pl.R1 = 0;
    c->last_listed = pub[2];
  }
  c->stats[0] = (int64_t)pl.R + (int64_t)pl.R1; c->stats[1] = 32 + bits_for((uint32_t)c->spec.ntiles); c->stats[2] = c->spec.ntiles;
  c->stats[3] = c->spec.G_total; c->stats[4] = c->spec.B_total; c->stats[5] = c->spec.I_total; c->stats[6] = 1;
  c->stats[7] = (int64_t)pl.longest;
  if (num_rendered_host) *num_rendered_host = c->stats[0] > 0 ? c->stats[0] : 1;
  if (!ok) { pl.valid = false; ++c->spec_stats[1]; }
  return ok ? 0 : 1;
}
const uint32_t* rtgs_raster_spec_fail_ptr_ctx(rtgs_ctx* ctx) {
  rtgs_ctx* c = use(ctx);
  return c->spec.pending ? c->spec.fail_dev : nullptr;
}
void rtgs_raster_set_speculation_ctx(rtgs_ctx* ctx, int enable) {
  rtgs_ctx* c = use(ctx);
  c->speculation = enable != 0;
  c->plan = rtgs_ctx::Plan();
}
int rtgs_raster_speculation_stats_ctx(rtgs_ctx* ctx, int64_t* out3) {
  if (!out3) return RTGS_E_INVALID;
  memcpy(out3, use(ctx)->spec_stats, sizeof(use(ctx)->spec_stats));
  return RTGS_OK;
}
int rtgs_raster_plain_stats_ctx(rtgs_ctx* ctx, int64_t* out2) {
  if (!out2) return RTGS_E_INVALID;
  memcpy(out2, use(ctx)->plain_stats, sizeof(use(ctx)->plain_stats));
  return RTGS_OK;
}
void rtgs_raster_set_plain_onepass_ctx(rtgs_ctx* ctx, int enable) {
  rtgs_ctx* c = use(ctx);
  c->plain_onepass = enable != 0;
  c->plan_plain = rtgs_ctx::Plan();
  c->plan_plain0 = rtgs_ctx::Plan();
}
uint32_t rtgs_raster_last_listed_ctx(rtgs_ctx* c) { return use(c)->last_listed; }
void rtgs_raster_set_bwd_debug(int bits) { rtgs::set_bwd_debug(bits); }
void rtgs_raster_set_bwd_stamps(void* dev) { rtgs::set_bwd_stamps(dev); }
void rtgs_raster_set_fwd_stamps(void* dev) { rtgs::set_fwd_stamps(dev); }
void rtgs_raster_set_onepass_ctx(rtgs_ctx* c, int on) { use(c)->onepass = on != 0; use(c)->plan.valid = false; }
void rtgs_raster_set_bwd_walk_ctx(rtgs_ctx* c, int mode) { use(c)->bwd_walk = (mode >= 1 && mode <= 4) ? mode : 0; }
void rtgs_raster_set_aux_zero_ctx(rtgs_ctx* ctx, void* eight_words) { use(ctx)->aux_zero = (uint32_t*)eight_words; }
int rtgs_raster_last_buffers_ctx(rtgs_ctx* ctx, void** out3) {
  rtgs_ctx* c = use(ctx);
  if (!out3 || !c->last_geom || !c->last_bin || !c->last_img) return RTGS_E_INVALID;
  out3[0] = c->last_geom; out3[1] = c->last_bin; out3[2] = c->last_img;
  return RTGS_OK;
}
int rtgs_raster_backward_buffers(int32_t P, int32_t H, int32_t W, size_t* out) {
  if (!out || P < 0 || H <= 0 || W <= 0) return RTGS_E_INVALID;
  const int gx = (W + TILE - 1) / TILE, gy = (H + TILE - 1) / TILE;
  const GeomLayout G = geom_layout(P, gx, gy, 1);
  const ImgLayout I = img_layout(H, W, gx * gy);
  out[0] = G.clamped; out[1] = G.offsets; out[2] = G.slot_count; out[3] = I.bwd_info;
  out[4] = align_up((size_t)(P > 0 ? P : 1) * sizeof(SplatGrad)); out[5] = G.radii; out[6] = 0; out[7] = 0;
  return RTGS_OK;
}
int rtgs_raster_image_offsets(int32_t H, int32_t W, size_t* out) {
  if (!out || H <= 0 || W <= 0) return RTGS_E_INVALID;
  const int gx = (W + TILE - 1) / TILE, gy = (H + TILE - 1) / TILE;
  const ImgLayout I = img_layout(H, W, gx * gy);
  out[0] = I.ranges; out[1] = I.n_contrib; out[2] = I.bwd_info; out[3] = I.tile_mode; out[4] = I.total; out[5] = I.depth_pos;
  return RTGS_OK;
}

int rtgs_raster_last_timings_ctx(rtgs_ctx* ctx, float* ms) {
  rtgs_ctx* c = use(ctx);
  if (!ms) return RTGS_E_INVALID;
  for (int i = 0; i < 12; ++i) ms[i] = -1.f;
  if (!c->ev_init) return RTGS_OK;
  const int pre_end = c->ev_set[EV_SL_BLEND] ? EV_SL_BLEND : EV_PRE;
  const int pairs[11][2] = {{EV_F0, EV_PRE}, {pre_end, EV_SCAN}, {EV_BIN0, EV_EMIT}, {EV_EMIT, EV_SORT},
                            {EV_SORT, EV_RANGES}, {EV_BLEND0, EV_BLEND}, {EV_B0, EV_BWALK}, {EV_BBLEND, EV_BPRE},
                            {EV_PRE, EV_SL_BIN}, {EV_SL_BIN, EV_SL_BLEND}, {EV_BWALK, EV_BBLEND}};
  for (int i = 0; i < 11; ++i) {
    const int a = pairs[i][0], b = pairs[i][1];
    if (!c->ev_set[a] || !c->ev_set[b]) continue;
    if (hipEventSynchronize(c->ev[b]) != hipSuccess) return RTGS_E_HIP;
    float t = 0.f;
    if (hipEventElapsedTime(&t, c->ev[a], c->ev[b]) == hipSuccess) ms[i] = t;
  }
  return RTGS_OK;
}

int rtgs_raster_forward(const rtgs_raster_settings* s, int32_t P, int32_t M, const float* means3D,
                        const float* opacities, const float* shs, const float* scales, const float* rotations,
                        const float* normal_w, const int32_t* tile_mask, float* out_color, float* out_depth,
                        int32_t* out_cidx, int32_t* out_didx, float* out_cw, float* out_dw, float* out_T,
// ... 41 lines not shown
```

### rtg_slam_amd/csrc/raster_bin.hip

```cpp
#include "raster_common.h"
#include <mutex>

namespace rtgs {

struct LdsGrant {
  std::mutex m;
  size_t got[64];
  explicit LdsGrant(size_t base) { for (size_t& g : got) g = base; }
  void ensure(const void* fn, size_t lds) {
    int dev = 0;
    (void)hipGetDevice(&dev);
    if (dev < 0 || dev >= 64) { (void)hipFuncSetAttribute(fn, hipFuncAttributeMaxDynamicSharedMemorySize, (int)lds); return; }
    std::lock_guard<std::mutex> lk(m);
    if (lds > got[dev]) {
      (void)hipFuncSetAttribute(fn, hipFuncAttributeMaxDynamicSharedMemorySize, (int)lds);
      got[dev] = lds;
    }
  }
};

constexpr int GPB = 1024;
#ifndef RTGS_SLICE_GPB
#define RTGS_SLICE_GPB 32
#endif
// ... 171 lines not shown
                                                            SpecCaps caps) {
  __shared__ uint32_t s_sum[1024];
  __shared__ uint32_t s_max[1024];
  const int tid = threadIdx.x;
  const int per = (ntiles + 1023) / 1024;
  const int lo = min(ntiles, tid * per), hi = min(ntiles, lo + per);
  uint32_t sum = 0, mx = 0;
  for (int t = lo; t < hi; ++t) { const uint32_t c = tile_count[t]; sum += c; mx = max(mx, c); }
  s_sum[tid] = sum; s_max[tid] = mx;
  __syncthreads();
  for (int off = 1; off < 1024; off <<= 1) {
    const uint32_t a = (tid >= off) ? s_sum[tid - off] : 0u;
    const uint32_t m = (tid >= off) ? s_max[tid - off] : 0u;
    __syncthreads();
    s_sum[tid] += a; s_max[tid] = max(s_max[tid], m);
    __syncthreads();
  }
  uint32_t start = s_sum[tid] - sum;
  for (int t = lo; t < hi; ++t) {
    const uint32_t c = tile_count[t];
    ranges[t] = make_uint2(start, start + c);
    cursor[t] = start;
    start += c;
  }
  if (tid == 1023) {
    info[0] = s_sum[1023]; info[1] = s_max[1023];
    const uint32_t slots_total = (slot_a ? slot_a[0] : 0u) + (slot_b ? slot_b[0] : 0u);
    const int32_t cut = caps.cut ? *caps.cut : 0;
    if (caps.fail)
      *caps.fail = (*caps.fail != 0u || s_sum[1023] > caps.R || s_max[1023] > caps.longest || slots_total > caps.slots ||
                    (caps.cut && cut >= 0)) ? 1u : 0u;
    if (info_host) {
      const uint32_t w[7] = {s_sum[1023], s_max[1023], extra_src ? extra_src[0] : 0u, extra_src ? extra_src[1] : 0u,
                             extra_src2 ? extra_src2[0] : 0u,
                             slots_total, (uint32_t)cut};
      publish_to_host(info_host, w, seq);
    }
  }
}

__global__ void __launch_bounds__(256) bin_scatter_kernel(RasterParams p, const Splat* __restrict__ splats,
                                                          const int32_t* __restrict__ radii,
                                                          const int32_t* __restrict__ mask,
                                                          const uint16_t* __restrict__ block_counts,
                                                          uint32_t* __restrict__ cursor,
                                                          unsigned long long* __restrict__ bucket, SliceSel sel,
                                                          SliceList list, int gpb) {
  extern __shared__ uint32_t s_mem[];
  __shared__ WaveBin s_wb[BLOCK / 64];
  const int ntiles = p.gx * p.gy;
  if (spec_failed(p.spec_fail)) return;
  if (list.ids && blockIdx.x * gpb >= (int)*list.count) return;
  uint32_t* s_cnt = s_mem;
  uint32_t* s_base = s_mem + ntiles;
  const uint16_t* row = block_counts + (size_t)blockIdx.x * ntiles;
  for (int t = threadIdx.x; t < ntiles; t += BLOCK) {
    const uint32_t c = row[t];
    s_base[t] = c ? atomicAdd(&cursor[t], c) : 0xffffffffu;
    s_cnt[t] = 0;
  }
  __syncthreads();
  enumerate_balanced(p, splats, radii, mask, nullptr, 0, list, gpb, sel.mode == 2 ? sel.sat : nullptr, sel.uv,
                     &s_wb[threadIdx.x >> 6], [&](bool hit, int t, int owner) {
    const uint32_t base = hit ? s_base[t] : 0xffffffffu;
    if (base != 0xffffffffu) {
      const uint32_t* r = s_wb[threadIdx.x >> 6].rec + owner * GREC;
      const uint32_t slot = base + atomicAdd(&s_cnt[t], 1u);
// ... 62 lines not shown
    const uint32_t e = stage[k];
    const uint32_t t = (e >> 6) & 0x3fffu;
    const uint32_t slot = s_cnt[t] + (e >> 20);
    const uint32_t* r = rec + (e & 63u) * GREC;
    if (slot < sb.seg) sb.bucket[(size_t)t * sb.seg + slot] = ((unsigned long long)r[11] << 32) | r[10];
  }
}

struct TileSeg { const uint32_t* count; uint32_t seg; uint2* ranges_out; };
__device__ __forceinline__ uint2 tile_range(const uint2* __restrict__ ranges, const TileSeg& ts, bool writer) {
  if (!ts.count) return ranges[blockIdx.x];
  const uint32_t x = blockIdx.x * ts.seg;
  const uint2 r = make_uint2(x, x + ts.count[blockIdx.x]);
  if (writer && ts.ranges_out) ts.ranges_out[blockIdx.x] = r;
  return r;
}

__device__ __forceinline__ void bin_finish(const BinFinish& f) {
  __shared__ uint32_t s_sum[2], s_max[2];
  uint32_t sum = 0, mx = 0;
  for (int t = threadIdx.x; t < f.ntiles; t += 128) { const uint32_t c = f.count[t]; sum += c; mx = max(mx, c); }
#pragma unroll
  for (int off = 32; off > 0; off >>= 1) { sum += (uint32_t)__shfl_xor((int)sum, off); mx = max(mx, (uint32_t)__shfl_xor((int)mx, off)); }
  if ((threadIdx.x & 63) == 0) { s_sum[threadIdx.x >> 6] = sum; s_max[threadIdx.x >> 6] = mx; }
  __syncthreads();
  if (threadIdx.x != 0) return;
  const uint32_t R = s_sum[0] + s_sum[1], longest = max(s_max[0], s_max[1]);
  f.info[0] = R; f.info[1] = longest;
  const uint32_t slots_total = (f.slot_a ? f.slot_a[0] : 0u) + (f.slot_b ? f.slot_b[0] : 0u);
  const int32_t cut = f.caps.cut ? *f.caps.cut : 0;
  if (f.caps.fail && (R > f.caps.R || longest > f.caps.longest || slots_total > f.caps.slots || (f.caps.cut && cut >= 0)))
    *f.caps.fail = 1u;
  if (f.info_host) {
    const uint32_t w[7] = {R, longest, f.listed ? f.listed[0] : 0u, 0u, 0u, slots_total, (uint32_t)cut};
    publish_to_host(f.info_host, w, f.seq);
  }
}

template <int THREADS>
__global__ void __launch_bounds__(THREADS) bin_tilesort_kernel(const uint2* __restrict__ ranges,
                                                               const unsigned long long* __restrict__ bucket,
                                                               uint32_t* __restrict__ point_list, int lo, int hi,
                                                               const uint32_t* __restrict__ spec_fail, TileSeg ts,
                                                               BinFinish fin) {
  extern __shared__ unsigned long long s_key[];
  if (fin.count && (int)blockIdx.x == fin.ntiles) { bin_finish(fin); return; }
  if (spec_failed(spec_fail)) return;
  const uint2 r = tile_range(ranges, ts, threadIdx.x == 0);
  const int n = (int)(r.y - r.x);
  if (n < lo || n >= hi) return;
  const int tid = threadIdx.x;
  if (n == 1) { if (tid == 0) point_list[r.x] = (uint32_t)bucket[r.x]; return; }
  int n2 = 2;
  while (n2 < n) n2 <<= 1;
  for (int i = tid; i < n2; i += THREADS) s_key[i] = (i < n) ? bucket[r.x + i] : ~0ull;
  __syncthreads();
  for (int k = 2; k <= n2; k <<= 1) {
    for (int j = k >> 1; j > 0; j >>= 1) {
      for (int i = tid; i < (n2 >> 1); i += THREADS) {
        const int a = ((i & ~(j - 1)) << 1) | (i & (j - 1));
        const int b = a | j;
        const unsigned long long ka = s_key[a], kb = s_key[b];
        const bool up = (a & k) == 0;
        if ((ka > kb) == up) { s_key[a] = kb; s_key[b] = ka; }
      }
      __syncthreads();
    }
// ... 436 lines not shown
```

### rtg_slam_amd/csrc/raster_common.h

```cpp
#pragma once
#include <hip/hip_runtime.h>
#include <stdint.h>
#include <stddef.h>

namespace rtgs {

constexpr int TILE = 16;
constexpr int BLOCK = TILE * TILE;
constexpr int WAVE = 64;
#ifndef RTGS_BWD_BATCH
#define RTGS_BWD_BATCH 128
#endif
constexpr int BATCH = RTGS_BWD_BATCH;

struct __attribute__((aligned(16))) Splat {
  float u, v;
  float ca, cb, cc;
  float o;
  float r, g, b;
  float nx, ny, nz;
  float pd;
  float z;
  float hx, hy;
};
// ... 9 lines not shown
  float pad0, pad1, pad2;
};
static_assert(sizeof(SplatGrad) == 64, "SplatGrad must be one 64-byte line");

struct RasterParams {
  int H, W, gx, gy, P, M, deg;
  float fx, fy, cx, cy, tanfovx, tanfovy, scale_modifier;
  float opaque_thr, depth_thr, normal_thr, color_sigma, T_thr;
  const float* view;
  const float* campos;
  const float* bg;
  const uint32_t* spec_fail;
};
__device__ __forceinline__ bool spec_failed(const uint32_t* f) { return f != nullptr && *f != 0u; }
struct SpecCaps {
  uint32_t* fail;
  uint32_t R, longest, slots;
  const int32_t* cut;
};

struct BinFinish {
  const uint32_t* count; int ntiles;
  uint32_t* info; uint32_t* info_host; const uint32_t* slot_a; const uint32_t* slot_b;
  const uint32_t* listed;
  uint32_t seq; SpecCaps caps;
};

inline size_t align_up(size_t x, size_t a = 256) { return (x + a - 1) / a * a; }

struct GeomLayout {
  size_t splats, tiles_touched, offsets, radii, clamped, sat, tile_count, cursor, info, block_counts, scan_temp, total;
  size_t scan_temp_bytes;
  size_t zero_begin, zero_end;
  size_t tile_count1, ranges1_bwd, slice_hist, slice_cover, slice_ctr;
  size_t zbin, cursor1, ranges1, mask2, block_counts1, bucket1, list1, uv, slice_ids;
  size_t vis_ids, block_counts_vis;
  size_t slot_count;
  size_t slice_seg;
  size_t slice_cap, slice_max_list;
};

constexpr int SLICE_BINS = 256;
constexpr int SLICE_MAX_LIST = 3072;
constexpr float SLICE_MIN_COVER = 24.f;
constexpr float SLICE_MIN_RATIO = 2.f;
struct SliceSel {
  int mode;
  const uint8_t* zbin;
  const uint32_t* hist;
  uint32_t cap;
  uint32_t max_list;
  const uint32_t* ctr;
  const int32_t* sat;
  const float2* uv;
  const unsigned long long* cover;
  uint32_t npix;
  int decide;
};
__device__ __forceinline__ int sat_count(const int32_t* __restrict__ sat, int gx, int x0, int y0, int x1, int y1) {
  const int sw = gx + 1;
  return sat[y1 * sw + x1] - sat[y0 * sw + x1] - sat[y1 * sw + x0] + sat[y0 * sw + x0];
}
struct SlicePass {
  int mode;
  const int32_t* user_mask;
  int32_t* mask2;
  uint2* ranges_bwd;
  uint2* ranges_main;
};
struct SliceList {
  const uint32_t* ids;
  const uint32_t* count;
};
__device__ __forceinline__ uint32_t slice_bin_of(float z) {
  const int b = (int)(__float_as_uint(z) >> 18) - (int)(0x3E4CCCCDu >> 18);
// ... 179 lines not shown
```

### rtg_slam_amd/csrc/raster_fwd.hip

```cpp
#include "raster_common.h"
#include <stdlib.h>

namespace rtgs {

constexpr int SAT_LDS = 12288;
__global__ void __launch_bounds__(256) mask_sat_kernel(const int32_t* __restrict__ mask, int gx, int gy,
                                                       int32_t* __restrict__ sat) {
  __shared__ int32_t s_sat[SAT_LDS];
  const int sw = gx + 1, n = (gy + 1) * sw;
  int32_t* const w = n <= SAT_LDS ? s_sat : sat;
  for (int i = threadIdx.x; i < n; i += blockDim.x) {
    int y = i / sw, x = i % sw;
    w[i] = (y == 0 || x == 0) ? 0 : (mask[(y - 1) * gx + (x - 1)] != 0);
  }
  __syncthreads();
  for (int y = 1 + threadIdx.x; y <= gy; y += blockDim.x) {
    int acc = 0;
    for (int x = 1; x <= gx; ++x) { acc += w[y * sw + x]; w[y * sw + x] = acc; }
  }
  __syncthreads();
  for (int x = 1 + threadIdx.x; x <= gx; x += blockDim.x) {
    int acc = 0;
    for (int y = 1; y <= gy; ++y) { acc += w[y * sw + x]; w[y * sw + x] = acc; }
  }
  if (w != sat) {
    __syncthreads();
    for (int i = threadIdx.x; i < n; i += blockDim.x) sat[i] = w[i];
  }
}

template <int MODE>
__global__ void __launch_bounds__(256) preprocess_fwd_kernel(
    RasterParams p, const float* __restrict__ means, const float* __restrict__ opac,
    const float* __restrict__ shs, const float* __restrict__ scales, const float* __restrict__ rots,
    const float* __restrict__ normal_w, const int32_t* __restrict__ sat,
    Splat* __restrict__ splats, uint32_t* __restrict__ tiles_touched, int32_t* __restrict__ radii,
    uint8_t* __restrict__ clamped, int32_t* __restrict__ out_radii, uint32_t* __restrict__ zero_words, int zero_n,
    uint8_t* __restrict__ zbin, float2* __restrict__ uv, SliceList list, SliceSel sel) {
#pragma clang fp contract(off)
  int i = blockIdx.x * blockDim.x + threadIdx.x;
  if constexpr (MODE != 2) {
    for (int t = i; t < zero_n; t += gridDim.x * blockDim.x) zero_words[t] = 0u;
    if (i >= p.P) return;
    tiles_touched[i] = 0;
    radii[i] = 0;
    if (out_radii) out_radii[i] = 0;
    if (zbin) zbin[i] = 255;
  } else {
    if (spec_failed(p.spec_fail)) return;
    if (list.ids) {
      if (i >= (int)*list.count) return;
      i = (int)list.ids[i];
    } else {
      if (sel.ctr && sel.ctr[0] == 0u) return;
      const int cut = slice_cut(sel);
      if (i >= p.P) return;
      const int zb = (int)sel.zbin[i];
      if (zb == 255 || zb <= cut) return;
      if (sel.sat) {
        const float2 c = uv[i];
        int x0, y0, x1, y1;
        tile_rect_of(c.x, c.y, radii[i], p.gx, p.gy, x0, y0, x1, y1);
        if (sat_count(sel.sat, p.gx, x0, y0, x1, y1) == 0) return;
      }
    }
  }

  const float* V = p.view;
  const float mx = means[3 * i], my = means[3 * i + 1], mz = means[3 * i + 2];
  const float pcx = V[0] * mx + V[4] * my + V[8] * mz + V[12];
  const float pcy = V[1] * mx + V[5] * my + V[9] * mz + V[13];
  const float pcz = V[2] * mx + V[6] * my + V[10] * mz + V[14];
  if (!(pcz > 0.2f)) return;

  const float4 q4 = reinterpret_cast<const float4*>(rots)[i];
  const float qr = q4.x, qx = q4.y, qy = q4.z, qz = q4.w;
  const float sx = scales[3 * i] * p.scale_modifier, sy = scales[3 * i + 1] * p.scale_modifier,
              sz = scales[3 * i + 2] * p.scale_modifier;
  const float R00 = 1.f - 2.f * (qy * qy + qz * qz), R01 = 2.f * (qx * qy - qr * qz), R02 = 2.f * (qx * qz + qr * qy);
  const float R10 = 2.f * (qx * qy + qr * qz), R11 = 1.f - 2.f * (qx * qx + qz * qz), R12 = 2.f * (qy * qz - qr * qx);
  const float R20 = 2.f * (qx * qz - qr * qy), R21 = 2.f * (qy * qz + qr * qx), R22 = 1.f - 2.f * (qx * qx + qy * qy);
  const float M00 = R00 * sx, M01 = R01 * sy, M02 = R02 * sz;
  const float M10 = R10 * sx, M11 = R11 * sy, M12 = R12 * sz;
  const float M20 = R20 * sx, M21 = R21 * sy, M22 = R22 * sz;
  const float S00 = M00 * M00 + M01 * M01 + M02 * M02;
  const float S01 = M00 * M10 + M01 * M11 + M02 * M12;
  const float S02 = M00 * M20 + M01 * M21 + M02 * M22;
  const float S11 = M10 * M10 + M11 * M11 + M12 * M12;
  const float S12 = M10 * M20 + M11 * M21 + M12 * M22;
  const float S22 = M20 * M20 + M21 * M21 + M22 * M22;

  const float limx = 1.3f * p.tanfovx, limy = 1.3f * p.tanfovy;
  const float txtz = pcx / pcz, tytz = pcy / pcz;
  const float tx = fminf(limx, fmaxf(-limx, txtz)) * pcz;
  const float ty = fminf(limy, fmaxf(-limy, tytz)) * pcz;
  const float iz = 1.f / pcz;
  const float J00 = p.fx * iz, J02 = -p.fx * tx * iz * iz;
  const float J11 = p.fy * iz, J12 = -p.fy * ty * iz * iz;
  const float T00 = J00 * V[0] + J02 * V[2], T01 = J00 * V[4] + J02 * V[6], T02 = J00 * V[8] + J02 * V[10];
  const float T10 = J11 * V[1] + J12 * V[2], T11 = J11 * V[5] + J12 * V[6], T12 = J11 * V[9] + J12 * V[10];
  const float a0 = S00 * T00 + S01 * T01 + S02 * T02;
  const float a1 = S01 * T00 + S11 * T01 + S12 * T02;
  const float a2 = S02 * T00 + S12 * T01 + S22 * T02;
  const float b0 = S00 * T10 + S01 * T11 + S02 * T12;
  const float b1 = S01 * T10 + S11 * T11 + S12 * T12;
  const float b2 = S02 * T10 + S12 * T11 + S22 * T12;
  const float ca = T00 * a0 + T01 * a1 + T02 * a2 + 0.3f;
  const float cb = T00 * b0 + T01 * b1 + T02 * b2;
  const float cc = T10 * b0 + T11 * b1 + T12 * b2 + 0.3f;
  const float det = ca * cc - cb * cb;
  if (det == 0.f) return;
  const float idet = 1.f / det;
  const float mid = 0.5f * (ca + cc);
  const float lam = mid + sqrtf(fmaxf(0.1f, mid * mid - det));
  int radius = (int)ceilf(p.color_sigma * sqrtf(lam));
  float u = p.fx * pcx / pcz + p.cx;
  float v = p.fy * pcy / pcz + p.cy;
  int touched = 0;
  if constexpr (MODE == 2) {
    const float2 t = uv[i];
    u = t.x; v = t.y; radius = radii[i];
  } else {
    int x0, y0, x1, y1;
    tile_rect_of(u, v, radius, p.gx, p.gy, x0, y0, x1, y1);
    if ((x1 - x0) * (y1 - y0) == 0) return;
    const int sw = p.gx + 1;
    touched = sat ? sat[y1 * sw + x1] - sat[y0 * sw + x1] - sat[y1 * sw + x0] + sat[y0 * sw + x0]
                  : (x1 - x0) * (y1 - y0);
  }
  if constexpr (MODE == 1) {
    radii[i] = radius;
    if (out_radii) out_radii[i] = radius;
    tiles_touched[i] = (uint32_t)touched;
    zbin[i] = (uint8_t)slice_bin_of(pcz);
    uv[i] = make_float2(u, v);
    return;
  }

  float dxw = mx - p.campos[0], dyw = my - p.campos[1], dzw = mz - p.campos[2];
  const float il = 1.f / sqrtf(dxw * dxw + dyw * dyw + dzw * dzw);
  dxw *= il; dyw *= il; dzw *= il;
  float shv[48];
  if (p.M == 16) {
    const float4* sh4 = reinterpret_cast<const float4*>(shs + (size_t)i * 48);
#pragma unroll
    for (int q = 0; q < 12; ++q) {
      const float4 t = sh4[q];
      shv[4 * q] = t.x; shv[4 * q + 1] = t.y; shv[4 * q + 2] = t.z; shv[4 * q + 3] = t.w;
    }
  } else {
    const float* shp = shs + (size_t)i * p.M * 3;
#pragma unroll
    for (int q = 0; q < 48; ++q) shv[q] = (q < p.M * 3) ? shp[q] : 0.f;
  }
  const float* sh = shv;
  float col[3];
#pragma unroll
  for (int c = 0; c < 3; ++c) {
    float r = RTGS_SH_C0 * sh[c];
    if (p.deg > 0) {
      r = r - RTGS_SH_C1 * dyw * sh[3 + c] + RTGS_SH_C1 * dzw * sh[6 + c] - RTGS_SH_C1 * dxw * sh[9 + c];
      if (p.deg > 1) {
        const float xx = dxw * dxw, yy = dyw * dyw, zz = dzw * dzw, xy = dxw * dyw, yz = dyw * dzw, xz = dxw * dzw;
        r = r + RTGS_SH_C2_0 * xy * sh[12 + c] + RTGS_SH_C2_1 * yz * sh[15 + c] +
            RTGS_SH_C2_2 * (2.f * zz - xx - yy) * sh[18 + c] + RTGS_SH_C2_3 * xz * sh[21 + c] +
            RTGS_SH_C2_4 * (xx - yy) * sh[24 + c];
        if (p.deg > 2) {
          r = r + RTGS_SH_C3_0 * dyw * (3.f * xx - yy) * sh[27 + c] + RTGS_SH_C3_1 * xy * dzw * sh[30 + c] +
// ... 406 lines not shown
    __syncthreads();
    if (tid == 0) {
      const bool add = sp.mode == 2;
      counters[2 * tile] = (add ? counters[2 * tile] : 0ull) + (unsigned long long)s_max;
      counters[2 * tile + 1] = (add ? counters[2 * tile + 1] : 0ull) + s_ev;
    }
  }
  if constexpr (STAMP) {
    if (lane == 0 && stamps != nullptr) {
      unsigned long long* o = stamps + (size_t)(tile * 4 + wv) * 8;
      o[0] = st_wall; o[1] = wall_clock64(); o[2] = st_range; o[3] = st_first; o[4] = st_walk;
      o[5] = __builtin_readcyclecounter() - st_cyc; o[6] = st_steps; o[7] = st_batches;
    }
  }
}
#undef RI


static int g_f1_occ = [] { const char* e = getenv("RTGS_F1_OCC"); const int v = e ? atoi(e) : 6; return v == 5 ? 5 : 6; }();
static int g_f1_asm = [] { const char* e = getenv("RTGS_F1_ASM"); return e ? atoi(e) : 1; }();
static unsigned long long* g_fwd_stamps = nullptr;
void set_fwd_stamps(void* dev) { g_fwd_stamps = (unsigned long long*)dev; }

void launch_mask_sat(const int32_t* mask, int gx, int gy, int32_t* sat, hipStream_t st) {
  hipLaunchKernelGGL(mask_sat_kernel, dim3(1), dim3(256), 0, st, mask, gx, gy, sat);
}
void launch_preprocess_fwd(const RasterParams& p, const float* means, const float* opac, const float* shs,
                           const float* scales, const float* rots, const float* normal_w, const int32_t* sat,
                           Splat* splats, uint32_t* tiles_touched, int32_t* radii, uint8_t* clamped,
                           int32_t* out_radii, uint32_t* zero_words, int zero_n, uint8_t* zbin, hipStream_t st) {
  if (p.P == 0) return;
  hipLaunchKernelGGL(preprocess_fwd_kernel<0>, dim3((p.P + 255) / 256), dim3(256), 0, st, p, means, opac, shs, scales,
                     rots, normal_w, sat, splats, tiles_touched, radii, clamped, out_radii, zero_words, zero_n, zbin,
                     (float2*)nullptr, SliceList{nullptr, nullptr}, SliceSel{0, nullptr, nullptr, 0u, 0u, nullptr, nullptr, nullptr});
}
void launch_preprocess_cull(const RasterParams& p, const float* means, const float* scales, const float* rots,
                            uint32_t* tiles_touched, int32_t* radii, int32_t* out_radii, uint32_t* zero_words, int zero_n,
                            uint8_t* zbin, float2* uv, hipStream_t st) {
  if (p.P == 0) return;
  hipLaunchKernelGGL(preprocess_fwd_kernel<1>, dim3((p.P + 255) / 256), dim3(256), 0, st, p, means, (const float*)nullptr,
                     (const float*)nullptr, scales, rots, (const float*)nullptr, (const int32_t*)nullptr, (Splat*)nullptr,
                     tiles_touched, radii, (uint8_t*)nullptr, out_radii, zero_words, zero_n, zbin, uv,
                     SliceList{nullptr, nullptr}, SliceSel{0, nullptr, nullptr, 0u, 0u, nullptr, nullptr, nullptr});
}
void launch_preprocess_shade(const RasterParams& p, const float* means, const float* opac, const float* shs,
                             const float* scales, const float* rots, const float* normal_w, Splat* splats,
                             int32_t* radii, uint8_t* clamped, float2* uv, SliceList list, SliceSel sel, size_t max_items,
                             hipStream_t st) {
  if (p.P == 0) return;
  const size_t n = list.ids ? (max_items < (size_t)p.P ? max_items : (size_t)p.P) : (size_t)p.P;
  hipLaunchKernelGGL(preprocess_fwd_kernel<2>, dim3((unsigned)((n + 255) / 256)), dim3(256), 0, st, p, means, opac, shs,
                     scales, rots, normal_w, (const int32_t*)nullptr, splats, (uint32_t*)nullptr, radii, clamped,
                     (int32_t*)nullptr, (uint32_t*)nullptr, 0, (uint8_t*)nullptr, uv, list, sel);
}
void launch_emit_keys(const RasterParams& p, const Splat* splats, const int32_t* radii, const uint32_t* offsets,
                      const int32_t* mask, uint64_t* keys, uint32_t* vals, hipStream_t st) {
  if (p.P == 0) return;
  hipLaunchKernelGGL(emit_keys_kernel, dim3((p.P + 255) / 256), dim3(256), 0, st, p, splats, radii, offsets, mask,
                     keys, vals);
}
void launch_tile_ranges(int64_t R, const uint64_t* keys, uint2* ranges, hipStream_t st) {
  if (R == 0) return;
  hipLaunchKernelGGL(tile_ranges_kernel, dim3((unsigned)((R + 255) / 256)), dim3(256), 0, st, R, keys, ranges);
}
__global__ void __launch_bounds__(256) slice_publish_kernel(int ntiles, const int32_t* __restrict__ user_mask,
                                                            const int32_t* __restrict__ mask2,
                                                            const uint32_t* __restrict__ r1, uint32_t* __restrict__ ctr,
                                                            uint32_t* __restrict__ host, uint32_t seq,
                                                            uint32_t* __restrict__ spec_fail,
                                                            const uint32_t* __restrict__ seg_count) {
  int left = 0, fin = 0, inst = 0;
  for (int t = threadIdx.x; t < ntiles; t += 256) {
    const bool on = user_mask[t] != 0, l = mask2[t] != 0;
    left += l ? 1 : 0;
    fin += (on && !l) ? 1 : 0;
    if (seg_count) inst += (int)seg_count[t];
  }
  __shared__ int s_l[4], s_f[4], s_i[4];
#pragma unroll
  for (int off = 32; off > 0; off >>= 1) { left += __shfl_xor(left, off); fin += __shfl_xor(fin, off); inst += __shfl_xor(inst, off); }
  if ((threadIdx.x & 63) == 0) { s_l[threadIdx.x >> 6] = left; s_f[threadIdx.x >> 6] = fin; s_i[threadIdx.x >> 6] = inst; }
  __syncthreads();
  if (threadIdx.x == 0) {
    const uint32_t L = (uint32_t)(s_l[0] + s_l[1] + s_l[2] + s_l[3]), F = (uint32_t)(s_f[0] + s_f[1] + s_f[2] + s_f[3]);
    ctr[0] = L; ctr[1] = F;
    if (spec_fail) *spec_fail = L != 0u ? 1u : 0u;
    const uint32_t R1 = seg_count ? (uint32_t)(s_i[0] + s_i[1] + s_i[2] + s_i[3]) : r1[0];
    const uint32_t w[7] = {ctr[2], 0u, L, F, R1, 0u, 0u};
    publish_to_host(host, w, seq);
  }
}
void launch_slice_publish(int ntiles, const int32_t* user_mask, const int32_t* mask2, const uint32_t* r1, uint32_t* ctr,
                          uint32_t* host, uint32_t seq, uint32_t* spec_fail, hipStream_t st, const uint32_t* seg_count) {
  hipLaunchKernelGGL(slice_publish_kernel, dim3(1), dim3(256), 0, st, ntiles, user_mask, mask2, r1, ctr, host, seq, spec_fail,
                     seg_count);
}

void launch_blend_fwd(const RasterParams& p, const uint2* ranges, const uint32_t* point_list, const Splat* splats,
                      float* out_color, float* out_depth, int32_t* out_cidx, int32_t* out_didx, float* out_cw,
                      float* out_dw, float* out_T, uint32_t* n_contrib, unsigned long long* counters,
                      SlicePass sp, uint32_t* tile_mode, uint32_t* depth_pos, uint32_t* tile_last, int walk, uint32_t* aux_zero,
                      TileCache tc, uint32_t seg, hipStream_t st) {
#define RTGS_FWD1(OCC, STAMP, COUNT, ASMW) hipLaunchKernelGGL((blend_fwd_kernel<OCC, STAMP, COUNT, ASMW>), dim3(p.gx, p.gy), dim3(BLOCK), 0, st, p, ranges, point_list, splats, \
                       out_color, out_depth, out_cidx, out_didx, out_cw, out_dw, out_T, n_contrib, counters, sp, tile_mode, \
                       depth_pos, tile_last, walk, aux_zero, tc, g_fwd_stamps, seg)
  if (g_f1_asm == 0) RTGS_FWD1(6, false, true, false);
  else if (counters) RTGS_FWD1(6, false, true, true);
  else if (g_fwd_stamps) RTGS_FWD1(6, true, false, true);
  else if (g_f1_occ == 5) RTGS_FWD1(5, false, false, true); else RTGS_FWD1(6, false, false, true);
#undef RTGS_FWD1
}

}
```

### rtg_slam_amd/map_optim.py

```python
from __future__ import annotations

import ctypes as C
import math
from typing import Callable, Dict, Optional

import torch
import torch.distributed as dist

COLS = 59
BLOCKS = (("xyz", 0, 3), ("shs", 3, 51), ("raw8", 51, 59))


def default_lr_columns(position_lr=1e-3, feature_lr=5e-4, opacity_lr=0.0, scaling_lr=4e-3, rotation_lr=1e-3):
    lr = torch.zeros(COLS)
    lr[0:3] = position_lr
    lr[3:6] = feature_lr
    lr[6:51] = feature_lr / 20.0
    lr[51:52] = opacity_lr
    lr[52:55] = scaling_lr
    lr[55:59] = rotation_lr
    return lr


def global_lr_scale(final: bool = False, feature_lr_coef: float = 1.0, scaling_lr_coef: float = 1.0,
# ... 137 lines not shown


class ShardedMapOptimizer:

    def __init__(self, packed: torch.Tensor, lr_col: Optional[torch.Tensor] = None, eps: float = 1e-15,
                 group=None, adam_fn: Optional[Callable] = None, activate_fn: Optional[Callable] = None,
                 n_frozen: int = 0, capacity: Optional[int] = None):
        self.group = group
        self.row_skip = adam_fn is None and packed.is_cuda
        self.adam_fn = adam_fn if adam_fn is not None else _adam_hip
        self.activate_fn = activate_fn if activate_fn is not None else activate8_hip
        self.world = dist.get_world_size(group) if dist.is_initialized() else 1
        self.rank = dist.get_rank(group) if dist.is_initialized() else 0
        self.backend = dist.get_backend(group) if dist.is_initialized() else "none"
        self.N = int(packed.shape[0])
        self.n_frozen = int(n_frozen)
        if not 0 <= self.n_frozen <= self.N:
            raise ValueError("n_frozen must be in [0, N]")
        self.device = packed.device
        self.lr_full = (default_lr_columns() if lr_col is None else lr_col).to(self.device).float()
        self.eps = eps
        self._use_arena = self.row_skip and activate_fn is None
        self.state = {}
        self.grad_rows = None
        self.act = None
        self._slam_ws = None
        self._slam_state = None
        self.capacity = 0
        self.aux = {}
        self._aux_spec = {}
        self._scope = "local"
        self._lr_scope = None
        self.version = 0
        self._gd_views = {}
        self._adam_dirty = None
        self._frozen_version = 0
        self._allocate(max(int(capacity) if capacity is not None else self.N, self.N, 1), packed)
        self.step_count = 0
        self.total_steps = getattr(self, "total_steps", 0)
        self.last_render = None
        self.last_num_rendered = 0
        self.attach_init = None
        self._history = None
        self._row_capacity = 16384
        self._pending = None
        self.overflow_redos = 0
        self._cap_peak, self._cap_steps, self._shrink_every = 0, 0, 32
        self._act_valid = False
        self.tail_mode = 1 if __import__("os").environ.get("RTGS_TAIL_MODE", "0") == "1" else 0
        self.live_counts = torch.zeros(2, dtype=torch.int32, device=self.device) if packed.is_cuda else None
        self._mode = None

    @property
    def n_train(self) -> int:
        return self.N - self.n_frozen

    def _active(self):
        return (self.n_frozen, 0) if self._scope == "global" else (self.N, self.n_frozen)

    @property
    def frozen_key(self):
        return (self.state["xyz"]["p"].data_ptr(), int(self.n_frozen), int(self._frozen_version))

    @property
    def n_active_train(self) -> int:
        n, t0 = self._active()
# ... 376 lines not shown
        ai, st, (N, nf) = self.attach_init, self.state, self._active()
        dev = st["xyz"]["p"].device
        attach = _lib.AttachC(ai["xyz"].data_ptr(), ai["raw8"].data_ptr(), ai["info"].data_ptr())
        with torch.cuda.device(dev):
            rc = lib.rtgs_attach_prepare(C.c_void_p(st["xyz"]["p"].data_ptr() + 12 * nf), C.c_void_p(st["raw8"]["p"].data_ptr() + 32 * nf),
                                         C.byref(attach), N - nf, C.c_void_p(torch.cuda.current_stream(dev).cuda_stream))
        _lib.check(rc, "rtgs_attach_prepare")
        return ai["info"][1]

    def step_slam(self, raster_settings, gt_color: torch.Tensor, gt_depth: torch.Tensor,
                  tile_mask: Optional[torch.Tensor] = None, color_weight: float = 0.8,
                  depth_weight: float = 1.0, ssim_weight: float = 0.2, add_depth_thres: float = 0.1,
                  render_mask: Optional[torch.Tensor] = None, confidence: Optional[torch.Tensor] = None,
                  tile_band: bool = False, normal_weight: float = 0.0,
                  gt_normal: Optional[torch.Tensor] = None) -> torch.Tensor:
        from . import _lib
        from .rasterizer import GaussianRasterizer, _Keep, current_context
        self._clean()
        if self.grad_rows is None:
            rast = GaussianRasterizer(raster_settings)

            def loss_fn(gd):
                out = rast(means3D=gd["xyz"], opacities=gd["opacity"], shs=gd["shs"], scales=gd["scales"],
                           rotations=gd["rotations"], normal_w=gd["normal"], tile_mask=tile_mask)
                return slam_losses_hip(out, gt_color, gt_depth, color_weight, depth_weight, ssim_weight, add_depth_thres,
                                       render_mask, normal_weight if gt_normal is not None else 0.0, gd["normal"], gt_normal)
            return self.step(loss_fn)
        lib = _lib.load()
        rs = raster_settings
        (N, nf), st, a = self._active(), self.state, self.grad_rows
        dev = st["xyz"]["p"].device
        if N == 0:
            raise RuntimeError("step_slam() on an empty map")
        self.version += 1
        if self._scope == "global":
            self._frozen_version += 1
        if self.world > 1:
            if self._mode == "sharded":
                raise RuntimeError("ShardedMapOptimizer: step_slam() after step() on more than one rank - the two keep "
                                   "different Adam state (replicated vs row-sharded); use one of them per optimizer")
            self._mode = "replicated"
            self._resolve_pending()
            if self._slam_state is None:
                cap = self.capacity
                self._slam_state = {
                    n: dict(m=torch.zeros(cap, c1 - c0, dtype=torch.float32, device=dev),
                            v=torch.zeros(cap, c1 - c0, dtype=torch.float32, device=dev),
                            ever=torch.zeros(cap, dtype=torch.uint8, device=dev)) for n, c0, c1 in BLOCKS}
        ad = self._slam_state if self.world > 1 else st
        H, W = int(rs.image_height), int(rs.image_width)
        ws = self._slam_ws
        if ws is None or ws["hw"] != (H, W):
            f = dict(dtype=torch.float32, device=dev)
            i = dict(dtype=torch.int32, device=dev)
            ws = self._slam_ws = dict(
                hw=(H, W), color=torch.empty(3, H, W, **f), depth=torch.empty(1, H, W, **f),
                cidx=torch.empty(1, H, W, **i), didx=torch.empty(1, H, W, **i), cw=torch.empty(1, H, W, **f),
                dw=torch.empty(1, H, W, **f), T=torch.empty(1, H, W, **f), radii=torch.empty(st["xyz"]["p"].shape[0], **i),
                g_color=torch.empty(3, H, W, **f), g_depth=torch.empty(1, H, W, **f), loss=torch.empty(4, **f),
                loss_scratch=None,
                ones=torch.ones((H + 15) // 16, (W + 15) // 16, **i),
                arenas=[_GrowArena(dev), _GrowArena(dev), _GrowArena(dev)])
        act = self.act
        if tile_mask is None:
            tile_mask = ws["ones"]
        tile_mask = tile_mask.to(device=dev, dtype=torch.int32).contiguous()
        gt_color, gt_depth = gt_color.contiguous(), gt_depth.contiguous()
        if normal_weight > 0 and gt_normal is not None:
            gt_normal = gt_normal.to(device=dev, dtype=torch.float32).contiguous()
        else:
            gt_normal = None
        rm = None if render_mask is None else (render_mask if render_mask.dtype == torch.uint8 else (render_mask != 0).to(torch.uint8)).contiguous()
        need = lib.rtgs_slam_loss_scratch_bytes(H, W, int(rm is None))
        if ws["loss_scratch"] is None or ws["loss_scratch"].numel() < need:
            ws["loss_scratch"] = torch.empty(need, dtype=torch.uint8, device=dev)
        attach = None
        if getattr(self, "attach_init", None) is not None:
            ai = self.attach_init
            attach = _lib.AttachC(ai["xyz"].data_ptr(), ai["raw8"].data_ptr(), ai["info"].data_ptr())
        keep = _Keep(rs, dev)
        self.step_count += 1
        self.total_steps = getattr(self, "total_steps", 0) + 1
        P = lambda t: t.data_ptr()
        geom, binning, img = ws["arenas"]
        args = _lib.MapStepArgsC(
            C.pointer(keep.c), N, 16, P(st["xyz"]["p"]), P(st["shs"]["p"]), P(st["raw8"]["p"]), P(tile_mask), P(gt_color),
            P(gt_depth), _lib.LossCfgC(float(color_weight), float(depth_weight), float(ssim_weight), float(add_depth_thres),
                                       rm.data_ptr() if rm is not None else None),
            P(ws["loss_scratch"]), P(act["opacity"]), P(act["scales"]), P(act["rotations"]),
            P(act["normal"]), P(ws["color"]), P(ws["depth"]), P(ws["cidx"]), P(ws["didx"]), P(ws["cw"]), P(ws["dw"]),
            P(ws["T"]), P(ws["radii"]), P(ws["g_color"]), P(ws["g_depth"]), P(ws["loss"]), P(a.d_means), P(a.d_opac),
            P(a.d_shs), P(a.d_scales), P(a.d_rots), P(a.d_normal), P(a.d_raw8), P(a.scratch), P(a.row_state),
            P(ad["xyz"]["m"]), P(ad["xyz"]["v"]), P(ad["shs"]["m"]), P(ad["shs"]["v"]), P(ad["raw8"]["m"]),
            P(ad["raw8"]["v"]), P(self._lr("xyz")), P(self._lr("shs")), P(self._lr("raw8")), P(ad["xyz"]["ever"]),
            P(ad["shs"]["ever"]), P(ad["raw8"]["ever"]), int(self.step_count), 0.9, 0.999, float(self.eps),
            C.pointer(attach) if attach is not None else None, P(confidence) if confidence is not None else None,
            int(self._act_valid), geom.cb, None, binning.cb, None, img.cb, None,
            float(normal_weight) if gt_normal is not None else 0.0, P(gt_normal) if gt_normal is not None else None,
            int(nf), int(N), int(self.tail_mode), P(self.live_counts) if self.live_counts is not None else None)
        R = C.c_int64(0)
        stream = torch.cuda.current_stream(dev).cuda_stream
        if tile_band and self.world > 1:
            if rm is None:
                raise RuntimeError("step_slam(tile_band=True) needs a render_mask (the SSIM window of the unmasked loss "
                                   "crosses band boundaries; the reference always passes one, mapper.py:196-203)")
            self._front_tileband(lib, args, ws, keep, tile_mask, rm, R, dev)
            self._exchange_and_tail(dict(step=int(self.step_count), attach=attach, confidence=confidence, keep=(keep, attach)))
        elif self.world == 1:
            self._mark_adam(0, N - nf)
            with torch.cuda.device(dev):
                rc = lib.rtgs_slam_map_step_ctx(current_context().ptr, C.byref(args), C.byref(R), C.c_void_p(stream))
            _lib.check(rc, "rtgs_slam_map_step")
        else:
            with torch.cuda.device(dev):
                rc = lib.rtgs_slam_map_step_front_ctx(current_context().ptr, C.byref(args), C.byref(R), C.c_void_p(stream))
            _lib.check(rc, "rtgs_slam_map_step_front")
            self._exchange_and_tail(dict(step=int(self.step_count), attach=attach, confidence=confidence, keep=(keep, attach)))
        a.calls = 1
        self._act_valid = True
        self.last_render = (ws["color"], ws["depth"], ws["cidx"], ws["didx"], ws["cw"], ws["dw"], ws["T"])
        self.last_num_rendered = int(R.value)
        self.last_losses = ws["loss"]
        return ws["loss"][0]

    def band_tile_mask(self, tile_mask: torch.Tensor, with_region: bool = False):
        on = (tile_mask.reshape(-1) != 0)
        cum = torch.cumsum(on.to(torch.int64), 0) - on.to(torch.int64)
        owner = ((cum * self.world) // on.sum().clamp_min(1)).clamp_max(self.world - 1)
        mine = owner == self.rank
        band = (on & mine).to(torch.int32).reshape(tile_mask.shape).contiguous()
        return (band, mine.reshape(tile_mask.shape)) if with_region else band

    def _front_tileband(self, lib, args, ws, keep, tile_mask, rm, R, dev):
        from . import _lib
        from .rasterizer import current_context
        N, t0 = self._active()
        H, W = ws["hw"]
        objs = ws.get("band_objs")
        same = (objs is not None and objs[0] is tile_mask and objs[1] is rm and objs[2] == (tile_mask._version, rm._version))
        if not same:
            band, region = self.band_tile_mask(tile_mask, with_region=True)
            pix = region.repeat_interleave(16, 0).repeat_interleave(16, 1)[:H, :W].to(torch.uint8)
            ws["band"], ws["band_rm"] = band, (pix * (rm != 0).to(torch.uint8)).contiguous()
            ws["band_objs"] = (tile_mask, rm, (tile_mask._version, rm._version))
        band, band_rm = ws["band"], ws["band_rm"]
        V = lambda t: C.c_void_p(t.data_ptr())
        st = lambda: C.c_void_p(torch.cuda.current_stream(dev).cuda_stream)
        geom, binning, img = ws["arenas"]
        x = self.state
        a = self.grad_rows
        cfg = _lib.LossCfgC(args.loss.color_weight, args.loss.depth_weight, args.loss.ssim_weight, args.loss.add_depth_thres,
                            band_rm.data_ptr())
        ctx = current_context().ptr
        act = self.act
        self._activate_rows(0, N)
        with torch.cuda.device(dev):
# ... 268 lines not shown
```

### rtg_slam_amd/rasterizer.py

```python
from __future__ import annotations

import ctypes as C
import threading
from typing import NamedTuple, Optional

import torch
import torch.nn as nn

from . import _lib


class GaussianRasterizationSettings(NamedTuple):
    image_height: int
    image_width: int
    tanfovx: float
    tanfovy: float
    bg: torch.Tensor
    scale_modifier: float
    viewmatrix: torch.Tensor
    projmatrix: torch.Tensor
    sh_degree: int
    campos: torch.Tensor
    opaque_threshold: float
    depth_threshold: float
# ... 20 lines not shown
        return cls(h, owned=True)

    def __del__(self):
        try:
            if self._owned and self.handle:
                _lib.load().rtgs_ctx_destroy(C.c_void_p(self.handle))
                self.handle = None
        except Exception:
            pass

    @property
    def ptr(self):
        return C.c_void_p(self.handle)

    def set_near_slice(self, mode: int, budget_per_tile: int = 0):
        _lib.load().rtgs_raster_set_near_slice_ctx(self.ptr, int(mode), int(budget_per_tile))

    def force_sort_path(self, enable: bool):
        _lib.load().rtgs_raster_force_sort_path_ctx(self.ptr, int(bool(enable)))

    def set_bwd_walk(self, mode: int):
        _lib.load().rtgs_raster_set_bwd_walk_ctx(self.ptr, int(mode))

    def set_onepass(self, enable: bool):
        _lib.load().rtgs_raster_set_onepass_ctx(self.ptr, int(bool(enable)))

    def set_speculation(self, enable: bool):
        _lib.load().rtgs_raster_set_speculation_ctx(self.ptr, int(bool(enable)))

    def speculation_stats(self):
        out = (C.c_int64 * 3)()
        _lib.check(_lib.load().rtgs_raster_speculation_stats_ctx(self.ptr, out), "rtgs_raster_speculation_stats")
        return dict(speculative=int(out[0]), failed=int(out[1]), not_eligible=int(out[2]))

    def set_plain_onepass(self, enable: bool):
        _lib.load().rtgs_raster_set_plain_onepass_ctx(self.ptr, int(bool(enable)))

    def plain_stats(self):
        out = (C.c_int64 * 2)()
        _lib.check(_lib.load().rtgs_raster_plain_stats_ctx(self.ptr, out), "rtgs_raster_plain_stats")
        return dict(onepass=int(out[0]), redone=int(out[1]))

    def set_profiling(self, enable: bool):
        _lib.load().rtgs_raster_set_profiling_ctx(self.ptr, int(bool(enable)))

    def set_counters(self, counters: Optional[torch.Tensor]):
        _lib.load().rtgs_raster_set_counters_ctx(self.ptr, C.c_void_p(counters.data_ptr() if counters is not None else 0))

    def last_stats(self):
        out = (C.c_int64 * 8)()
        _lib.check(_lib.load().rtgs_raster_last_stats_ctx(self.ptr, out), "rtgs_raster_last_stats")
        return [int(v) for v in out]

    def last_slice_stats(self):
        out = (C.c_int64 * 4)()
        _lib.check(_lib.load().rtgs_raster_last_slice_stats_ctx(self.ptr, out), "rtgs_raster_last_slice_stats")
        return dict(used=int(out[0]), instances=int(out[1]), tiles_finished=int(out[2]), tiles_left_to_pass2=int(out[3]))

    def last_timings(self):
        out = (C.c_float * 12)()
        _lib.check(_lib.load().rtgs_raster_last_timings_ctx(self.ptr, out), "rtgs_raster_last_timings")
        return [float(v) for v in out]


def image_buffer_views(img: torch.Tensor, H: int, W: int):
    off = (C.c_size_t * 6)()
# ... 262 lines not shown
```

Before: 2656 units/s.

## Cache preprocess cull results across map steps and recull only updated rows

```diff
diff --git a/include/rtgs_raster.h b/include/rtgs_raster.h
--- a/include/rtgs_raster.h
+++ b/include/rtgs_raster.h
@@ -156,6 +156,11 @@
 int rtgs_raster_speculation_stats_ctx(rtgs_ctx* ctx, int64_t* out3_host);
 void rtgs_raster_set_plain_onepass_ctx(rtgs_ctx* ctx, int enable);
 int rtgs_raster_plain_stats_ctx(rtgs_ctx* ctx, int64_t* out2_host);
+void rtgs_raster_set_cull_cache_ctx(rtgs_ctx* ctx, int enable);
+void rtgs_raster_set_cull_cache_check_ctx(rtgs_ctx* ctx, int enable);
+void rtgs_raster_set_map_epoch_ctx(rtgs_ctx* ctx, uint64_t epoch);
+uint8_t* rtgs_raster_cull_marks_ctx(rtgs_ctx* ctx);
+int rtgs_raster_cull_cache_stats_ctx(rtgs_ctx* ctx, int64_t* out5_host);
 int rtgs_raster_image_offsets(int32_t image_height, int32_t image_width, size_t* out6_host);
 
 int rtgs_fused_adam(float* params, const float* grads, float* exp_avg, float* exp_avg_sq,
@@ -195,6 +200,14 @@
                        uint8_t* ever_xyz, uint8_t* ever_shs, uint8_t* ever_raw8, int64_t rows, int32_t step, float beta1,
                        float beta2, float eps, const rtgs_attach* attach, float* confidence, const uint32_t* skip_flag,
                        const rtgs_activated* refresh, void* stream);
+int rtgs_map_tail_rows_marked(float* xyz, float* shs, float* raw8, const float* g_opacity, const float* g_scales,
+                              const float* g_rotations, const float* g_normal, const float* g_xyz, const float* g_shs,
+                              float* g_raw8, const uint8_t* row_state, float* m_xyz, float* v_xyz, float* m_shs,
+                              float* v_shs, float* m_raw8, float* v_raw8, const float* lr_xyz, const float* lr_shs,
+                              const float* lr_raw8, uint8_t* ever_xyz, uint8_t* ever_shs, uint8_t* ever_raw8, int64_t rows,
+                              int32_t step, float beta1, float beta2, float eps, const rtgs_attach* attach,
+                              float* confidence, const uint32_t* skip_flag, const rtgs_activated* refresh, uint8_t* marks,
+                              void* stream);
 
 typedef struct rtgs_loss_cfg {
   float color_weight, depth_weight, ssim_weight, add_depth_thres;
@@ -244,6 +257,7 @@
   int32_t train_begin, train_end;
   int32_t tail_mode;
   uint32_t* live_counts;
+  uint64_t map_epoch;
 } rtgs_map_step_args;
 int rtgs_slam_normal_loss(const float* normal_w, const int32_t* depth_index, const float* gt_normal,
                           const uint8_t* render_mask, int32_t H, int32_t W, float normal_weight, float* scratch2,
@@ -267,6 +281,9 @@
 int rtgs_map_fused_tail_hint(const rtgs_raster_settings* settings, const rtgs_map_step_args* args, void* geom_buffer,
                              const void* image_buffer, const uint32_t* spec_fail, uint32_t* live_counts2,
                              uint32_t listed_hint, void* stream);
+int rtgs_map_fused_tail_marked(const rtgs_raster_settings* settings, const rtgs_map_step_args* args, void* geom_buffer,
+                               const void* image_buffer, const uint32_t* spec_fail, uint32_t* live_counts2,
+                               uint32_t listed_hint, uint8_t* marks, void* stream);
 uint32_t rtgs_raster_last_listed_ctx(rtgs_ctx* ctx);
 int rtgs_raster_backward_buffers(int32_t P, int32_t image_height, int32_t image_width, size_t* out8_host);
 int rtgs_raster_last_buffers_ctx(rtgs_ctx* ctx, void** out3_host);
diff --git a/rtg_slam_amd/_lib.py b/rtg_slam_amd/_lib.py
--- a/rtg_slam_amd/_lib.py
+++ b/rtg_slam_amd/_lib.py
@@ -68,7 +68,7 @@
         + [("geom_resize", RESIZE_FN), ("geom_user", C.c_void_p), ("binning_resize", RESIZE_FN),
            ("binning_user", C.c_void_p), ("image_resize", RESIZE_FN), ("image_user", C.c_void_p)]
         + [("normal_weight", C.c_float), ("gt_normal", C.c_void_p), ("train_begin", C.c_int32), ("train_end", C.c_int32),
-           ("tail_mode", C.c_int32), ("live_counts", C.c_void_p)])
+           ("tail_mode", C.c_int32), ("live_counts", C.c_void_p), ("map_epoch", C.c_uint64)])
 
 
 _SIGNATURES = {
@@ -98,6 +98,14 @@
     "rtgs_map_fused_tail": (C.c_int, [C.POINTER(RasterSettingsC), C.POINTER(MapStepArgsC), _P, _P, _P, _P, _P]),
     "rtgs_map_fused_tail_hint": (C.c_int, [C.POINTER(RasterSettingsC), C.POINTER(MapStepArgsC), _P, _P, _P, _P, C.c_uint32, _P]),
     "rtgs_raster_last_listed_ctx": (C.c_uint32, [_P]),
+    "rtgs_raster_set_cull_cache_ctx": (None, [_P, C.c_int]),
+    "rtgs_raster_set_cull_cache_check_ctx": (None, [_P, C.c_int]),
+    "rtgs_raster_cull_cache_stats_ctx": (C.c_int, [_P, C.POINTER(C.c_int64)]),
+    "rtgs_raster_set_map_epoch_ctx": (None, [_P, C.c_uint64]),
+    "rtgs_raster_cull_marks_ctx": (C.c_void_p, [_P]),
+    "rtgs_map_tail_rows_marked": (C.c_int, [_P] * 23 + [C.c_int64, C.c_int32, C.c_float, C.c_float, C.c_float,
+                                            C.POINTER(AttachC), _P, _P, C.POINTER(ActivatedC), _P, _P]),
+    "rtgs_map_fused_tail_marked": (C.c_int, [C.POINTER(RasterSettingsC), C.POINTER(MapStepArgsC), _P, _P, _P, _P, C.c_uint32, _P, _P]),
     "rtgs_stream_create_reserving": (C.c_void_p, [C.c_int]),
     "rtgs_stream_destroy": (None, [_P]),
     "rtgs_raster_backward_buffers": (C.c_int, [C.c_int32, C.c_int32, C.c_int32, C.POINTER(C.c_size_t)]),
diff --git a/rtg_slam_amd/csrc/map_fused.hip b/rtg_slam_amd/csrc/map_fused.hip
--- a/rtg_slam_amd/csrc/map_fused.hip
+++ b/rtg_slam_amd/csrc/map_fused.hip
@@ -29,6 +29,7 @@
   float *act_opacity, *act_scales, *act_normal;
   float4* act_rots;
   uint32_t* live_counts;
+  uint8_t* marks;
   int t0, rows;
 };
 
@@ -179,6 +180,7 @@
           }
         }
         const bool grad = rgrad || sel;
+        if (a.marks && (grad || e_raw8 != 0 || e_xyz != 0)) a.marks[r] = 1;
         if (grad || e_raw8 != 0) {
           float4 lo = make_float4(0.f, 0.f, 0.f, 0.f), hi = lo;
           if (rgrad)
@@ -275,6 +277,12 @@
 extern "C" int rtgs_map_fused_tail_hint(const rtgs_raster_settings* settings, const rtgs_map_step_args* s, void* geom_buffer,
                                         const void* image_buffer, const uint32_t* spec_fail, uint32_t* live_counts2,
                                         uint32_t listed_hint, void* stream) {
+  return rtgs_map_fused_tail_marked(settings, s, geom_buffer, image_buffer, spec_fail, live_counts2, listed_hint, nullptr, stream);
+}
+
+extern "C" int rtgs_map_fused_tail_marked(const rtgs_raster_settings* settings, const rtgs_map_step_args* s, void* geom_buffer,
+                                          const void* image_buffer, const uint32_t* spec_fail, uint32_t* live_counts2,
+                                          uint32_t listed_hint, uint8_t* marks, void* stream) {
   using namespace rtgs;
   if (!settings || !s || !geom_buffer || !image_buffer) return RTGS_E_INVALID;
   const int32_t P = s->P;
@@ -323,6 +331,7 @@
   a.confidence = s->confidence;
   a.act_opacity = s->opacity; a.act_scales = s->scales; a.act_normal = s->normal; a.act_rots = (float4*)s->rotations;
   a.live_counts = live_counts2;
+  a.marks = marks;
   a.t0 = t0; a.rows = t1 - t0;
   static const int forced = [] { const char* e = getenv("RTGS_FUSED_CHUNK"); return e ? atoi(e) : 0; }();
   int chunk = 1024;
diff --git a/rtg_slam_amd/csrc/map_ops.hip b/rtg_slam_amd/csrc/map_ops.hip
--- a/rtg_slam_amd/csrc/map_ops.hip
+++ b/rtg_slam_amd/csrc/map_ops.hip
@@ -93,6 +93,7 @@
   const uint32_t* skip_flag;
   float *act_opacity, *act_scales, *act_normal;
   float4* act_rots;
+  uint8_t* marks;
 };
 
 __device__ __forceinline__ bool attach_selected(const float4 init_lo) {
@@ -139,6 +140,7 @@
         hi.x += at_hi.x; hi.y += at_hi.y; hi.z += at_hi.z; hi.w += at_hi.w;
         a.g_raw8[2 * r] = lo; a.g_raw8[2 * r + 1] = hi;
       }
+      if (a.marks && (grad || e_raw8 != 0 || e_xyz != 0)) a.marks[r] = 1;
       if (grad || e_raw8 != 0) {
         if (e_raw8 == 0) a.ever_raw8[r] = 1;
         const float4 g0 = lo, g1 = hi;
@@ -326,6 +328,21 @@
                                   int64_t rows, int32_t step, float beta1, float beta2, float eps,
                                   const rtgs_attach* attach, float* confidence, const uint32_t* skip_flag,
                                   const rtgs_activated* refresh, void* stream) {
+  return rtgs_map_tail_rows_marked(xyz, shs, raw8, g_opacity, g_scales, g_rotations, g_normal, g_xyz, g_shs, g_raw8, row_state,
+                                   m_xyz, v_xyz, m_shs, v_shs, m_raw8, v_raw8, lr_xyz, lr_shs, lr_raw8, ever_xyz, ever_shs,
+                                   ever_raw8, rows, step, beta1, beta2, eps, attach, confidence, skip_flag, refresh, nullptr,
+                                   stream);
+}
+
+extern "C" int rtgs_map_tail_rows_marked(float* xyz, float* shs, float* raw8, const float* g_opacity, const float* g_scales,
+                                         const float* g_rotations, const float* g_normal, const float* g_xyz,
+                                         const float* g_shs, float* g_raw8, const uint8_t* row_state, float* m_xyz,
+                                         float* v_xyz, float* m_shs, float* v_shs, float* m_raw8, float* v_raw8,
+                                         const float* lr_xyz, const float* lr_shs, const float* lr_raw8, uint8_t* ever_xyz,
+                                         uint8_t* ever_shs, uint8_t* ever_raw8, int64_t rows, int32_t step, float beta1,
+                                         float beta2, float eps, const rtgs_attach* attach, float* confidence,
+                                         const uint32_t* skip_flag, const rtgs_activated* refresh, uint8_t* marks,
+                                         void* stream) {
   if (rows < 0 || step < 1) return -1;
   if (rows == 0) return 0;
   if (!xyz || !shs || !raw8 || !g_opacity || !g_scales || !g_rotations || !g_normal || !g_xyz || !g_shs || !g_raw8 ||
@@ -342,6 +359,7 @@
   a.rows = rows; a.beta1 = beta1; a.beta2 = beta2; a.eps = eps;
   a.init_xyz = nullptr; a.init_raw8 = nullptr; a.attach_info = nullptr; a.confidence = confidence;
   a.skip_flag = skip_flag;
+  a.marks = marks;
   a.act_opacity = a.act_scales = a.act_normal = nullptr; a.act_rots = nullptr;
   if (refresh) {
     if (!refresh->opacity || !refresh->scales || !refresh->rotations || !refresh->normal) return -1;
diff --git a/rtg_slam_amd/csrc/map_step.hip b/rtg_slam_amd/csrc/map_step.hip
--- a/rtg_slam_amd/csrc/map_step.hip
+++ b/rtg_slam_amd/csrc/map_step.hip
@@ -59,25 +59,28 @@
 
 static int map_step_once(rtgs_ctx* ctx, const rtgs_map_step_args* a, int64_t* num_rendered_host, bool speculate, void* stream) {
   const bool fused = a->tail_mode == 0 && !(a->normal_weight > 0.f && a->gt_normal);
+  rtgs_raster_set_map_epoch_ctx(ctx, speculate ? a->map_epoch : 0u);
   int rc = map_step_front(ctx, a, num_rendered_host, speculate ? RTGS_FWD_SPECULATE : 0, stream, fused);
   if (rc != RTGS_OK) return rc;
   if ((a->train_begin != 0 || a->train_end != 0) && a->train_end == a->train_begin) return RTGS_OK;
   if (fused) {
     void* bufs[3];
     if (rtgs_raster_last_buffers_ctx(ctx, bufs) != RTGS_OK) return RTGS_E_ALLOC;
-    return rtgs_map_fused_tail_hint(a->settings, a, bufs[0], bufs[2], rtgs_raster_spec_fail_ptr_ctx(ctx), a->live_counts,
-                                    rtgs_raster_last_listed_ctx(ctx), stream);
+    return rtgs_map_fused_tail_marked(a->settings, a, bufs[0], bufs[2], rtgs_raster_spec_fail_ptr_ctx(ctx), a->live_counts,
+                                      rtgs_raster_last_listed_ctx(ctx), rtgs_raster_cull_marks_ctx(ctx), stream);
   }
   const int32_t P = a->P;
   int32_t t0 = 0, t1 = P;
   if (a->train_begin != 0 || a->train_end != 0) { t0 = a->train_begin; t1 = a->train_end; }
   const size_t o = (size_t)t0;
   const rtgs_activated act{a->opacity + o, a->scales + 3 * o, a->rotations + 4 * o, a->normal + 3 * o};
-  rc = rtgs_map_tail_rows(a->xyz + 3 * o, a->shs + 48 * o, a->raw8 + 8 * o, a->d_opacity + o, a->d_scales + 3 * o,
+  uint8_t* const marks = rtgs_raster_cull_marks_ctx(ctx);
+  rc = rtgs_map_tail_rows_marked(a->xyz + 3 * o, a->shs + 48 * o, a->raw8 + 8 * o, a->d_opacity + o, a->d_scales + 3 * o,
                           a->d_rotations + 4 * o, a->d_normal + 3 * o, a->d_xyz + 3 * o, a->d_shs + 48 * o, a->d_raw8 + 8 * o,
                           a->row_state + o, a->m_xyz, a->v_xyz, a->m_shs, a->v_shs, a->m_raw8, a->v_raw8,
                           a->lr_xyz, a->lr_shs, a->lr_raw8, a->ever_xyz, a->ever_shs, a->ever_raw8, (int64_t)(t1 - t0), a->step,
-                          a->beta1, a->beta2, a->eps, a->attach, a->confidence, rtgs_raster_spec_fail_ptr_ctx(ctx), &act, stream);
+                          a->beta1, a->beta2, a->eps, a->attach, a->confidence, rtgs_raster_spec_fail_ptr_ctx(ctx), &act,
+                          marks ? marks + o : nullptr, stream);
   return rc != 0 ? RTGS_E_HIP : RTGS_OK;
 }
 
diff --git a/rtg_slam_amd/csrc/raster_api.hip b/rtg_slam_amd/csrc/raster_api.hip
--- a/rtg_slam_amd/csrc/raster_api.hip
+++ b/rtg_slam_amd/csrc/raster_api.hip
@@ -47,7 +47,13 @@
 void launch_slice_publish(int, const int32_t*, const int32_t*, const uint32_t*, uint32_t*, uint32_t*, uint32_t, uint32_t*, hipStream_t,
                           const uint32_t* seg_count = nullptr);
 void launch_preprocess_cull(const RasterParams&, const float*, const float*, const float*, uint32_t*, int32_t*, int32_t*,
-                            uint32_t*, int, uint8_t*, float2*, hipStream_t);
+                            uint32_t*, int, uint8_t*, float2*, uint32_t*, hipStream_t);
+void launch_recull_rows(const RasterParams&, const float*, const float*, const float*, uint32_t*, int32_t*, int32_t*, uint32_t*,
+                        int, uint8_t*, float2*, uint32_t*, unsigned long long*, uint8_t*, const float*, int, BwdInfoInit,
+                        hipStream_t);
+void launch_cull_check(int, const uint32_t*, const uint32_t*, const int32_t*, const int32_t*, const int32_t*, const int32_t*,
+                       const uint8_t*, const uint8_t*, const float2*, const float2*, const uint32_t*, const uint32_t*,
+                       const uint32_t*, unsigned long long*, hipStream_t);
 void launch_preprocess_shade(const RasterParams&, const float*, const float*, const float*, const float*, const float*,
                              const float*, Splat*, int32_t*, uint8_t*, float2*, SliceList, SliceSel, size_t, hipStream_t);
 void launch_bin_tilescan(int, const uint32_t*, uint2*, uint32_t*, uint32_t*, uint32_t*, const uint32_t*, const uint32_t*,
@@ -118,6 +124,22 @@
   Plan plan_plain0;
   bool plain_onepass = true;
   int64_t plain_stats[2] = {0, 0};
+  struct CullKey {
+    const void *geom, *view, *means, *scales, *rots, *out_radii, *stream;
+    uint64_t geom_bytes, epoch;
+    int32_t P, H, W, kind, slice_mode, slice_budget;
+    float fx, fy, cx, cy, tanfovx, tanfovy, scale_modifier, color_sigma;
+  };
+  struct CullCache {
+    bool enabled = true, check = false, armed = false;
+    CullKey key = {};
+    uint8_t* marks = nullptr;
+    uint64_t next_epoch = 0;
+    int64_t stats[4] = {0, 0, 0, 0};
+    char* scratch = nullptr;
+    size_t scratch_bytes = 0;
+    unsigned long long* mismatches = nullptr;
+  } cull;
 };
 
 namespace rtgs {
@@ -131,6 +153,8 @@
     if (const char* e = getenv("RTGS_BIN_ONEPASS")) n->onepass = atoi(e) != 0;
     if (const char* e = getenv("RTGS_PLAIN_ONEPASS")) n->plain_onepass = atoi(e) != 0;
     if (const char* e = getenv("RTGS_BWD_WALK")) { const int m = atoi(e); n->bwd_walk = (m >= 1 && m <= 4) ? m : 0; }
+    if (const char* e = getenv("RTGS_CULL_CACHE")) n->cull.enabled = atoi(e) != 0;
+    if (const char* e = getenv("RTGS_CULL_CACHE_CHECK")) n->cull.check = atoi(e) != 0;
     return n;
   }();
   return c;
@@ -208,8 +232,6 @@
     off = L.tile_count + nt * sizeof(uint32_t);
     L.tile_count1 = off; off += nt * sizeof(uint32_t);
     L.ranges1_bwd = off; off += nt * sizeof(uint2);
-    L.slice_hist = off; off += 2 * SLICE_BINS * sizeof(uint32_t);
-    L.slice_cover = off; off += SLICE_BINS * sizeof(unsigned long long);
     L.slice_ctr = off; off += 8 * sizeof(uint32_t);
     L.slot_count = off; off += Pn * sizeof(uint32_t);
     L.zero_end = off; off = align_up(off);
@@ -221,6 +243,10 @@
     L.ranges1 = off; off = align_up(off + nt * sizeof(uint2));
     L.mask2 = off; off = align_up(off + nt * sizeof(int32_t));
     L.uv = off; off = align_up(off + Pn * sizeof(float2));
+    L.slice_hist = off; off += 2 * SLICE_BINS * sizeof(uint32_t);
+    L.slice_cover = off; off = align_up(off + SLICE_BINS * sizeof(unsigned long long));
+    L.cull_marks = off; off = align_up(off + Pn + 16);
+    L.cull_view = off; off = align_up(off + 16 * sizeof(float));
     L.slice_cap = nt * (size_t)(budget > 0 ? budget : 1);
     L.slice_max_list = L.slice_cap < 65536 ? L.slice_cap : 65536;
     if (L.slice_max_list > Pn) L.slice_max_list = Pn;
@@ -332,13 +358,15 @@
 
 rtgs_ctx* rtgs_ctx_create(void) {
   rtgs_ctx* c = new (std::nothrow) rtgs_ctx();
-  if (c) { c->slice_mode = default_ctx()->slice_mode; c->slice_budget = default_ctx()->slice_budget; c->bwd_walk = default_ctx()->bwd_walk; c->onepass = default_ctx()->onepass; c->speculation = default_ctx()->speculation; c->plain_onepass = default_ctx()->plain_onepass; }
+  if (c) { c->slice_mode = default_ctx()->slice_mode; c->slice_budget = default_ctx()->slice_budget; c->bwd_walk = default_ctx()->bwd_walk; c->onepass = default_ctx()->onepass; c->speculation = default_ctx()->speculation; c->plain_onepass = default_ctx()->plain_onepass; c->cull.enabled = default_ctx()->cull.enabled; c->cull.check = default_ctx()->cull.check; }
   return c;
 }
 void rtgs_ctx_destroy(rtgs_ctx* c) {
   if (!c || c == default_ctx()) return;
   if (c->ev_init) for (int i = 0; i < EV_N; ++i) (void)hipEventDestroy(c->ev[i]);
   if (c->info_host) (void)hipHostFree(c->info_host);
+  if (c->cull.scratch) (void)hipFree(c->cull.scratch);
+  if (c->cull.mismatches) (void)hipFree(c->cull.mismatches);
   delete c;
 }
 
@@ -376,6 +404,11 @@
   rtgs_ctx* c = use(ctx);
   uint32_t* const aux_zero = c->aux_zero;
   c->aux_zero = nullptr;
+  const uint64_t cull_epoch = c->cull.next_epoch;
+  c->cull.next_epoch = 0;
+  const bool cull_was_armed = c->cull.armed;
+  c->cull.armed = false;
+  if (cull_was_armed) ++c->cull.stats[2];
   RasterParams p;
   int rc = make_params(s, P, M, p);
   if (rc != RTGS_OK) return rc;
@@ -474,10 +507,63 @@
       if (++c->seq == 0u) c->seq = 1u;
       size_t b_total = 0;
       bool seg_main = false;
+      auto cull_stage = [&](const BwdInfoInit& bi) -> int {
+        rtgs_ctx::CullCache& cc = c->cull;
+        rtgs_ctx::CullKey key;
+        memset(&key, 0, sizeof(key));
+        key.geom = geom; key.view = s->viewmatrix; key.means = means3D; key.scales = scales; key.rots = rotations;
+        key.out_radii = out_radii; key.stream = stream; key.geom_bytes = (uint64_t)G.total; key.epoch = cull_epoch;
+        key.P = P; key.H = p.H; key.W = p.W; key.kind = pl.kind; key.slice_mode = c->slice_mode; key.slice_budget = c->slice_budget;
+        key.fx = p.fx; key.fy = p.fy; key.cx = p.cx; key.cy = p.cy; key.tanfovx = p.tanfovx; key.tanfovy = p.tanfovy;
+        key.scale_modifier = p.scale_modifier; key.color_sigma = p.color_sigma;
+        const bool usable = cc.enabled && !immediate && cull_epoch != 0;
+        uint8_t* const marks = (uint8_t*)(geom + G.cull_marks);
+        float* const view_copy = (float*)(geom + G.cull_view);
+        float2* const uv = (float2*)(geom + G.uv);
+        if (usable && cull_was_armed && memcmp(&key, &cc.key, sizeof(key)) == 0) {
+          launch_recull_rows(p, means3D, scales, rotations, tiles_touched, radii, out_radii, zero_words, zero_n, zbin, uv,
+                             slice_hist, slice_cover, marks, view_copy, (int)(fail - zero_words), bi, st);
+          cc.armed = true;
+          ++cc.stats[0]; --cc.stats[2];
+          if (cc.check) {
+            const size_t Pn = (size_t)P;
+            const size_t o_tt = 0, o_rad = align_up(o_tt + Pn * 4), o_orad = align_up(o_rad + Pn * 4), o_zb = align_up(o_orad + Pn * 4),
+                         o_uv = align_up(o_zb + Pn), o_hist = align_up(o_uv + Pn * 8), need = align_up(o_hist + CULL_HIST_WORDS * 4);
+            if (cc.scratch_bytes < need) {
+              if (cc.scratch) (void)hipFree(cc.scratch);
+              cc.scratch = nullptr; cc.scratch_bytes = 0;
+              HIP_TRY(hipMalloc((void**)&cc.scratch, need));
+              cc.scratch_bytes = need;
+            }
+            if (!cc.mismatches) {
+              HIP_TRY(hipMalloc((void**)&cc.mismatches, sizeof(unsigned long long)));
+              HIP_TRY(hipMemset(cc.mismatches, 0, sizeof(unsigned long long)));
+            }
+            char* sc = cc.scratch;
+            HIP_TRY(hipMemcpyAsync(sc + o_uv, uv, Pn * 8, hipMemcpyDeviceToDevice, st));
+            launch_preprocess_cull(p, means3D, scales, rotations, (uint32_t*)(sc + o_tt), (int32_t*)(sc + o_rad),
+                                   out_radii ? (int32_t*)(sc + o_orad) : nullptr, nullptr, 0, (uint8_t*)(sc + o_zb),
+                                   (float2*)(sc + o_uv), (uint32_t*)(sc + o_hist), st);
+            launch_slice_hist(P, (const uint8_t*)(sc + o_zb), (const uint32_t*)(sc + o_tt), (const int32_t*)(sc + o_rad),
+                              (uint32_t*)(sc + o_hist), (unsigned long long*)(sc + o_hist + 2 * SLICE_BINS * 4), st);
+            launch_cull_check(P, tiles_touched, (const uint32_t*)(sc + o_tt), radii, (const int32_t*)(sc + o_rad), out_radii,
+                              (const int32_t*)(sc + o_orad), zbin, (const uint8_t*)(sc + o_zb), uv, (const float2*)(sc + o_uv),
+                              slice_hist, (const uint32_t*)(sc + o_hist), fail + 1, cc.mismatches, st);
+          }
+          return RTGS_OK;
+        }
+        launch_preprocess_cull(p, means3D, scales, rotations, tiles_touched, radii, out_radii, zero_words, zero_n, zbin, uv,
+                               slice_hist, st);
+        launch_slice_hist(P, zbin, tiles_touched, radii, slice_hist, slice_cover, st, bi);
+        if (usable) {
+          HIP_TRY(hipMemsetAsync(marks, 0, align_up((size_t)P + 16), st));
+          HIP_TRY(hipMemcpyAsync(view_copy, s->viewmatrix, 16 * sizeof(float), hipMemcpyDeviceToDevice, st));
+          memcpy(&cc.key, &key, sizeof(key)); cc.marks = marks; cc.armed = true;
+          ++cc.stats[1];
+        }
+        return RTGS_OK;
+      };
       if (pl.kind == 1) {
-        launch_preprocess_cull(p, means3D, scales, rotations, tiles_touched, radii, out_radii, zero_words, zero_n, zbin,
-                               (float2*)(geom + G.uv), st);
-        prof_mark(c, EV_PRE, st);
         const uint32_t sl = (uint32_t)G.slice_cap;
         const bool use_sl = sl > 0 && sl <= SLOTS_MAX;
         const BinLayout B = bin_layout(0, ntiles, false, use_sl ? (size_t)sl : 0);
@@ -485,8 +571,10 @@
         if (!bin) return RTGS_E_ALLOC;
         c->last_bin = bin;
         b_total = B.total;
-        launch_slice_hist(P, zbin, tiles_touched, radii, slice_hist, slice_cover, st,
-                          BwdInfoInit{(BwdInfo*)(img + I.bwd_info), (SplatGrad*)(bin + B.slot_grads), use_sl ? sl : 0u, use_sl ? 1u : 0u});
+        if ((rc = cull_stage(BwdInfoInit{(BwdInfo*)(img + I.bwd_info), (SplatGrad*)(bin + B.slot_grads), use_sl ? sl : 0u,
+                                         use_sl ? 1u : 0u})) != RTGS_OK)
+          return rc;
+        prof_mark(c, EV_PRE, st);
         launch_slice_compact(P, sel1, (uint32_t*)(geom + G.slice_ids), slice_ctr + 2, tiles_touched, offsets, slice_ctr + 4,
                              nullptr, 0u, nullptr, st);
         const SliceList work{(const uint32_t*)(geom + G.slice_ids), slice_ctr + 2};
@@ -530,11 +618,10 @@
         pg.spec_fail = fail;
         SliceList vl{nullptr, nullptr};
         if (pl.kind == 2) {
-          launch_preprocess_cull(p, means3D, scales, rotations, tiles_touched, radii, out_radii, zero_words, zero_n, zbin,
-                                 (float2*)(geom + G.uv), st);
+          if ((rc = cull_stage(BwdInfoInit{(BwdInfo*)(img + I.bwd_info), (SplatGrad*)(bin + B.slot_grads), capS,
+                                           immediate ? 0u : 1u})) != RTGS_OK)
+            return rc;
           prof_mark(c, EV_PRE, st);
-          launch_slice_hist(P, zbin, tiles_touched, radii, slice_hist, slice_cover, st,
-                            BwdInfoInit{(BwdInfo*)(img + I.bwd_info), (SplatGrad*)(bin + B.slot_grads), capS, immediate ? 0u : 1u});
           vl = SliceList{(const uint32_t*)(geom + G.vis_ids), slice_ctr + 4};
           launch_visible_compact(P, zbin, (uint32_t*)(geom + G.vis_ids), slice_ctr + 4, tiles_touched, offsets, slice_ctr + 5, fail, st,
                                  &sel1, (int32_t*)(slice_ctr + 3), fail);
@@ -628,7 +715,7 @@
       if (!sort_path && want_bwd && (rc = scan_all()) != RTGS_OK) return rc;
     } else {
       launch_preprocess_cull(p, means3D, scales, rotations, tiles_touched, radii, out_radii, zero_words, zero_n, zbin,
-                             (float2*)(geom + G.uv), st);
+                             (float2*)(geom + G.uv), slice_hist, st);
     }
     DBG(s, st);
     prof_mark(c, EV_PRE, st);
@@ -964,12 +1051,15 @@
   bool ok;
   if (c->spec.kind == 1) {
     const uint32_t n_left = pub[2];
-    ok = n_left == 0u;
+    ok = n_left == 0u && pub[5] == 0u;
+    if (pub[5] != 0u) ++c->cull.stats[3];
     pl.R1 = pub[4]; pl.n_fin = pub[3]; pl.R = 0; pl.longest = 0;
     c->last_listed = pub[0];
     c->slice_stats[1] = pub[4]; c->slice_stats[2] = pub[3]; c->slice_stats[3] = n_left;
   } else {
-    ok = pub[0] <= c->spec.capR && pub[1] <= c->spec.capL && pub[5] <= c->spec.capS && (c->spec.kind != 2 || (int32_t)pub[6] < 0);
+    ok = pub[0] <= c->spec.capR && pub[1] <= c->spec.capL && pub[5] <= c->spec.capS && (c->spec.kind != 2 || (int32_t)pub[6] < 0) &&
+         pub[4] == 0u;
+    if (pub[4] != 0u) ++c->cull.stats[3];
     pl.note(pub[0], pub[1], pub[5]); pl.R1 = 0;
     c->last_listed = pub[2];
   }
@@ -1006,6 +1096,26 @@
   c->plan_plain0 = rtgs_ctx::Plan();
 }
 uint32_t rtgs_raster_last_listed_ctx(rtgs_ctx* c) { return use(c)->last_listed; }
+void rtgs_raster_set_cull_cache_ctx(rtgs_ctx* ctx, int enable) {
+  rtgs_ctx* c = use(ctx);
+  c->cull.enabled = enable != 0;
+  c->cull.armed = false;
+}
+void rtgs_raster_set_cull_cache_check_ctx(rtgs_ctx* ctx, int enable) { use(ctx)->cull.check = enable != 0; }
+void rtgs_raster_set_map_epoch_ctx(rtgs_ctx* ctx, uint64_t epoch) { use(ctx)->cull.next_epoch = epoch; }
+uint8_t* rtgs_raster_cull_marks_ctx(rtgs_ctx* ctx) {
+  rtgs_ctx* c = use(ctx);
+  return c->cull.armed ? c->cull.marks : nullptr;
+}
+int rtgs_raster_cull_cache_stats_ctx(rtgs_ctx* ctx, int64_t* out5) {
+  rtgs_ctx* c = use(ctx);
+  if (!out5) return RTGS_E_INVALID;
+  memcpy(out5, c->cull.stats, sizeof(c->cull.stats));
+  unsigned long long bad = 0;
+  if (c->cull.mismatches) HIP_TRY(hipMemcpy(&bad, c->cull.mismatches, sizeof(bad), hipMemcpyDeviceToHost));
+  out5[4] = (int64_t)bad;
+  return RTGS_OK;
+}
 void rtgs_raster_set_bwd_debug(int bits) { rtgs::set_bwd_debug(bits); }
 void rtgs_raster_set_bwd_stamps(void* dev) { rtgs::set_bwd_stamps(dev); }
 void rtgs_raster_set_fwd_stamps(void* dev) { rtgs::set_fwd_stamps(dev); }
@@ -1024,7 +1134,7 @@
   const GeomLayout G = geom_layout(P, gx, gy, 1);
   const ImgLayout I = img_layout(H, W, gx * gy);
   out[0] = G.clamped; out[1] = G.offsets; out[2] = G.slot_count; out[3] = I.bwd_info;
-  out[4] = align_up((size_t)(P > 0 ? P : 1) * sizeof(SplatGrad)); out[5] = G.radii; out[6] = 0; out[7] = 0;
+  out[4] = align_up((size_t)(P > 0 ? P : 1) * sizeof(SplatGrad)); out[5] = G.radii; out[6] = G.cull_marks; out[7] = 0;
   return RTGS_OK;
 }
 int rtgs_raster_image_offsets(int32_t H, int32_t W, size_t* out) {
diff --git a/rtg_slam_amd/csrc/raster_bin.hip b/rtg_slam_amd/csrc/raster_bin.hip
--- a/rtg_slam_amd/csrc/raster_bin.hip
+++ b/rtg_slam_amd/csrc/raster_bin.hip
@@ -227,7 +227,7 @@
                     (caps.cut && cut >= 0)) ? 1u : 0u;
     if (info_host) {
       const uint32_t w[7] = {s_sum[1023], s_max[1023], extra_src ? extra_src[0] : 0u, extra_src ? extra_src[1] : 0u,
-                             extra_src2 ? extra_src2[0] : 0u,
+                             extra_src2 ? extra_src2[0] : (caps.fail ? caps.fail[1] : 0u),
                              slots_total, (uint32_t)cut};
       publish_to_host(info_host, w, seq);
     }
@@ -356,7 +356,7 @@
   if (f.caps.fail && (R > f.caps.R || longest > f.caps.longest || slots_total > f.caps.slots || (f.caps.cut && cut >= 0)))
     *f.caps.fail = 1u;
   if (f.info_host) {
-    const uint32_t w[7] = {R, longest, f.listed ? f.listed[0] : 0u, 0u, 0u, slots_total, (uint32_t)cut};
+    const uint32_t w[7] = {R, longest, f.listed ? f.listed[0] : 0u, 0u, f.caps.fail ? f.caps.fail[1] : 0u, slots_total, (uint32_t)cut};
     publish_to_host(f.info_host, w, f.seq);
   }
 }
diff --git a/rtg_slam_amd/csrc/raster_common.h b/rtg_slam_amd/csrc/raster_common.h
--- a/rtg_slam_amd/csrc/raster_common.h
+++ b/rtg_slam_amd/csrc/raster_common.h
@@ -65,7 +65,8 @@
   size_t splats, tiles_touched, offsets, radii, clamped, sat, tile_count, cursor, info, block_counts, scan_temp, total;
   size_t scan_temp_bytes;
   size_t zero_begin, zero_end;
-  size_t tile_count1, ranges1_bwd, slice_hist, slice_cover, slice_ctr;
+  size_t tile_count1, ranges1_bwd, slice_ctr;
+  size_t slice_hist, slice_cover, cull_marks, cull_view;
   size_t zbin, cursor1, ranges1, mask2, block_counts1, bucket1, list1, uv, slice_ids;
   size_t vis_ids, block_counts_vis;
   size_t slot_count;
@@ -74,6 +75,7 @@
 };
 
 constexpr int SLICE_BINS = 256;
+constexpr int CULL_HIST_WORDS = 2 * SLICE_BINS + 2 * SLICE_BINS;
 constexpr int SLICE_MAX_LIST = 3072;
 constexpr float SLICE_MIN_COVER = 24.f;
 constexpr float SLICE_MIN_RATIO = 2.f;
diff --git a/rtg_slam_amd/csrc/raster_fwd.hip b/rtg_slam_amd/csrc/raster_fwd.hip
--- a/rtg_slam_amd/csrc/raster_fwd.hip
+++ b/rtg_slam_amd/csrc/raster_fwd.hip
@@ -29,6 +29,88 @@
   }
 }
 
+struct CullGeom {
+  float mx, my, mz, pcx, pcy, pcz, ca, cb, cc, idet, u, v;
+  int radius, touched;
+};
+template <bool RECT>
+__device__ __forceinline__ bool cull_geom(const RasterParams& p, const float* __restrict__ means,
+                                          const float* __restrict__ scales, const float* __restrict__ rots,
+                                          const int32_t* __restrict__ sat, int i, CullGeom& o) {
+#pragma clang fp contract(off)
+  const float* V = p.view;
+  const float mx = means[3 * i], my = means[3 * i + 1], mz = means[3 * i + 2];
+  const float pcx = V[0] * mx + V[4] * my + V[8] * mz + V[12];
+  const float pcy = V[1] * mx + V[5] * my + V[9] * mz + V[13];
+  const float pcz = V[2] * mx + V[6] * my + V[10] * mz + V[14];
+  if (!(pcz > 0.2f)) return false;
+
+  const float4 q4 = reinterpret_cast<const float4*>(rots)[i];
+  const float qr = q4.x, qx = q4.y, qy = q4.z, qz = q4.w;
+  const float sx = scales[3 * i] * p.scale_modifier, sy = scales[3 * i + 1] * p.scale_modifier,
+              sz = scales[3 * i + 2] * p.scale_modifier;
+  const float R00 = 1.f - 2.f * (qy * qy + qz * qz), R01 = 2.f * (qx * qy - qr * qz), R02 = 2.f * (qx * qz + qr * qy);
+  const float R10 = 2.f * (qx * qy + qr * qz), R11 = 1.f - 2.f * (qx * qx + qz * qz), R12 = 2.f * (qy * qz - qr * qx);
+  const float R20 = 2.f * (qx * qz - qr * qy), R21 = 2.f * (qy * qz + qr * qx), R22 = 1.f - 2.f * (qx * qx + qy * qy);
+  const float M00 = R00 * sx, M01 = R01 * sy, M02 = R02 * sz;
+  const float M10 = R10 * sx, M11 = R11 * sy, M12 = R12 * sz;
+  const float M20 = R20 * sx, M21 = R21 * sy, M22 = R22 * sz;
+  const float S00 = M00 * M00 + M01 * M01 + M02 * M02;
+  const float S01 = M00 * M10 + M01 * M11 + M02 * M12;
+  const float S02 = M00 * M20 + M01 * M21 + M02 * M22;
+  const float S11 = M10 * M10 + M11 * M11 + M12 * M12;
+  const float S12 = M10 * M20 + M11 * M21 + M12 * M22;
+  const float S22 = M20 * M20 + M21 * M21 + M22 * M22;
+
+  const float limx = 1.3f * p.tanfovx, limy = 1.3f * p.tanfovy;
+  const float txtz = pcx / pcz, tytz = pcy / pcz;
+  const float tx = fminf(limx, fmaxf(-limx, txtz)) * pcz;
+  const float ty = fminf(limy, fmaxf(-limy, tytz)) * pcz;
+  const float iz = 1.f / pcz;
+  const float J00 = p.fx * iz, J02 = -p.fx * tx * iz * iz;
+  const float J11 = p.fy * iz, J12 = -p.fy * ty * iz * iz;
+  const float T00 = J00 * V[0] + J02 * V[2], T01 = J00 * V[4] + J02 * V[6], T02 = J00 * V[8] + J02 * V[10];
+  const float T10 = J11 * V[1] + J12 * V[2], T11 = J11 * V[5] + J12 * V[6], T12 = J11 * V[9] + J12 * V[10];
+  const float a0 = S00 * T00 + S01 * T01 + S02 * T02;
+  const float a1 = S01 * T00 + S11 * T01 + S12 * T02;
+  const float a2 = S02 * T00 + S12 * T01 + S22 * T02;
+  const float b0 = S00 * T10 + S01 * T11 + S02 * T12;
+  const float b1 = S01 * T10 + S11 * T11 + S12 * T12;
+  const float b2 = S02 * T10 + S12 * T11 + S22 * T12;
+  const float ca = T00 * a0 + T01 * a1 + T02 * a2 + 0.3f;
+  const float cb = T00 * b0 + T01 * b1 + T02 * b2;
+  const float cc = T10 * b0 + T11 * b1 + T12 * b2 + 0.3f;
+  const float det = ca * cc - cb * cb;
+  if (det == 0.f) return false;
+  const float idet = 1.f / det;
+  const float mid = 0.5f * (ca + cc);
+  const float lam = mid + sqrtf(fmaxf(0.1f, mid * mid - det));
+  const int radius = (int)ceilf(p.color_sigma * sqrtf(lam));
+  const float u = p.fx * pcx / pcz + p.cx;
+  const float v = p.fy * pcy / pcz + p.cy;
+  int touched = 0;
+  if constexpr (RECT) {
+    int x0, y0, x1, y1;
+    tile_rect_of(u, v, radius, p.gx, p.gy, x0, y0, x1, y1);
+    if ((x1 - x0) * (y1 - y0) == 0) return false;
+    const int sw = p.gx + 1;
+    touched = sat ? sat[y1 * sw + x1] - sat[y0 * sw + x1] - sat[y1 * sw + x0] + sat[y0 * sw + x0]
+                  : (x1 - x0) * (y1 - y0);
+  }
+  o.mx = mx; o.my = my; o.mz = mz; o.pcx = pcx; o.pcy = pcy; o.pcz = pcz;
+  o.ca = ca; o.cb = cb; o.cc = cc; o.idet = idet; o.u = u; o.v = v; o.radius = radius; o.touched = touched;
+  return true;
+}
+__device__ __forceinline__ void cull_store(const CullGeom& g, int i, uint32_t* __restrict__ tiles_touched,
+                                           int32_t* __restrict__ radii, int32_t* __restrict__ out_radii,
+                                           uint8_t* __restrict__ zbin, float2* __restrict__ uv) {
+  radii[i] = g.radius;
+  if (out_radii) out_radii[i] = g.radius;
+  tiles_touched[i] = (uint32_t)g.touched;
+  zbin[i] = (uint8_t)slice_bin_of(g.pcz);
+  uv[i] = make_float2(g.u, g.v);
+}
+
 template <int MODE>
 __global__ void __launch_bounds__(256) preprocess_fwd_kernel(
     RasterParams p, const float* __restrict__ means, const float* __restrict__ opac,
@@ -36,11 +118,13 @@
     const float* __restrict__ normal_w, const int32_t* __restrict__ sat,
     Splat* __restrict__ splats, uint32_t* __restrict__ tiles_touched, int32_t* __restrict__ radii,
     uint8_t* __restrict__ clamped, int32_t* __restrict__ out_radii, uint32_t* __restrict__ zero_words, int zero_n,
-    uint8_t* __restrict__ zbin, float2* __restrict__ uv, SliceList list, SliceSel sel) {
+    uint8_t* __restrict__ zbin, float2* __restrict__ uv, SliceList list, SliceSel sel,
+    uint32_t* __restrict__ zero2, int zero2_n) {
 #pragma clang fp contract(off)
   int i = blockIdx.x * blockDim.x + threadIdx.x;
   if constexpr (MODE != 2) {
     for (int t = i; t < zero_n; t += gridDim.x * blockDim.x) zero_words[t] = 0u;
+    for (int t = i; t < zero2_n; t += gridDim.x * blockDim.x) zero2[t] = 0u;
     if (i >= p.P) return;
     tiles_touched[i] = 0;
     radii[i] = 0;
@@ -66,74 +150,20 @@
     }
   }
 
+  CullGeom cg;
+  if (!cull_geom<MODE != 2>(p, means, scales, rots, sat, i, cg)) return;
   const float* V = p.view;
-  const float mx = means[3 * i], my = means[3 * i + 1], mz = means[3 * i + 2];
-  const float pcx = V[0] * mx + V[4] * my + V[8] * mz + V[12];
-  const float pcy = V[1] * mx + V[5] * my + V[9] * mz + V[13];
-  const float pcz = V[2] * mx + V[6] * my + V[10] * mz + V[14];
-  if (!(pcz > 0.2f)) return;
-
-  const float4 q4 = reinterpret_cast<const float4*>(rots)[i];
-  const float qr = q4.x, qx = q4.y, qy = q4.z, qz = q4.w;
-  const float sx = scales[3 * i] * p.scale_modifier, sy = scales[3 * i + 1] * p.scale_modifier,
-              sz = scales[3 * i + 2] * p.scale_modifier;
-  const float R00 = 1.f - 2.f * (qy * qy + qz * qz), R01 = 2.f * (qx * qy - qr * qz), R02 = 2.f * (qx * qz + qr * qy);
-  const float R10 = 2.f * (qx * qy + qr * qz), R11 = 1.f - 2.f * (qx * qx + qz * qz), R12 = 2.f * (qy * qz - qr * qx);
-  const float R20 = 2.f * (qx * qz - qr * qy), R21 = 2.f * (qy * qz + qr * qx), R22 = 1.f - 2.f * (qx * qx + qy * qy);
-  const float M00 = R00 * sx, M01 = R01 * sy, M02 = R02 * sz;
-  const float M10 = R10 * sx, M11 = R11 * sy, M12 = R12 * sz;
-  const float M20 = R20 * sx, M21 = R21 * sy, M22 = R22 * sz;
-  const float S00 = M00 * M00 + M01 * M01 + M02 * M02;
-  const float S01 = M00 * M10 + M01 * M11 + M02 * M12;
-  const float S02 = M00 * M20 + M01 * M21 + M02 * M22;
-  const float S11 = M10 * M10 + M11 * M11 + M12 * M12;
-  const float S12 = M10 * M20 + M11 * M21 + M12 * M22;
-  const float S22 = M20 * M20 + M21 * M21 + M22 * M22;
-
-  const float limx = 1.3f * p.tanfovx, limy = 1.3f * p.tanfovy;
-  const float txtz = pcx / pcz, tytz = pcy / pcz;
-  const float tx = fminf(limx, fmaxf(-limx, txtz)) * pcz;
-  const float ty = fminf(limy, fmaxf(-limy, tytz)) * pcz;
-  const float iz = 1.f / pcz;
-  const float J00 = p.fx * iz, J02 = -p.fx * tx * iz * iz;
-  const float J11 = p.fy * iz, J12 = -p.fy * ty * iz * iz;
-  const float T00 = J00 * V[0] + J02 * V[2], T01 = J00 * V[4] + J02 * V[6], T02 = J00 * V[8] + J02 * V[10];
-  const float T10 = J11 * V[1] + J12 * V[2], T11 = J11 * V[5] + J12 * V[6], T12 = J11 * V[9] + J12 * V[10];
-  const float a0 = S00 * T00 + S01 * T01 + S02 * T02;
-  const float a1 = S01 * T00 + S11 * T01 + S12 * T02;
-  const float a2 = S02 * T00 + S12 * T01 + S22 * T02;
-  const float b0 = S00 * T10 + S01 * T11 + S02 * T12;
-  const float b1 = S01 * T10 + S11 * T11 + S12 * T12;
-  const float b2 = S02 * T10 + S12 * T11 + S22 * T12;
-  const float ca = T00 * a0 + T01 * a1 + T02 * a2 + 0.3f;
-  const float cb = T00 * b0 + T01 * b1 + T02 * b2;
-  const float cc = T10 * b0 + T11 * b1 + T12 * b2 + 0.3f;
-  const float det = ca * cc - cb * cb;
-  if (det == 0.f) return;
-  const float idet = 1.f / det;
-  const float mid = 0.5f * (ca + cc);
-  const float lam = mid + sqrtf(fmaxf(0.1f, mid * mid - det));
-  int radius = (int)ceilf(p.color_sigma * sqrtf(lam));
-  float u = p.fx * pcx / pcz + p.cx;
-  float v = p.fy * pcy / pcz + p.cy;
-  int touched = 0;
+  const float mx = cg.mx, my = cg.my, mz = cg.mz, pcx = cg.pcx, pcy = cg.pcy, pcz = cg.pcz;
+  const float ca = cg.ca, cb = cg.cb, cc = cg.cc, idet = cg.idet;
+  float u = cg.u, v = cg.v;
+  int radius = cg.radius;
+  const int touched = cg.touched;
   if constexpr (MODE == 2) {
     const float2 t = uv[i];
     u = t.x; v = t.y; radius = radii[i];
-  } else {
-    int x0, y0, x1, y1;
-    tile_rect_of(u, v, radius, p.gx, p.gy, x0, y0, x1, y1);
-    if ((x1 - x0) * (y1 - y0) == 0) return;
-    const int sw = p.gx + 1;
-    touched = sat ? sat[y1 * sw + x1] - sat[y0 * sw + x1] - sat[y1 * sw + x0] + sat[y0 * sw + x0]
-                  : (x1 - x0) * (y1 - y0);
   }
   if constexpr (MODE == 1) {
-    radii[i] = radius;
-    if (out_radii) out_radii[i] = radius;
-    tiles_touched[i] = (uint32_t)touched;
-    zbin[i] = (uint8_t)slice_bin_of(pcz);
-    uv[i] = make_float2(u, v);
+    cull_store(cg, i, tiles_touched, radii, out_radii, zbin, uv);
     return;
   }
 
@@ -606,16 +636,18 @@
   if (p.P == 0) return;
   hipLaunchKernelGGL(preprocess_fwd_kernel<0>, dim3((p.P + 255) / 256), dim3(256), 0, st, p, means, opac, shs, scales,
                      rots, normal_w, sat, splats, tiles_touched, radii, clamped, out_radii, zero_words, zero_n, zbin,
-                     (float2*)nullptr, SliceList{nullptr, nullptr}, SliceSel{0, nullptr, nullptr, 0u, 0u, nullptr, nullptr, nullptr});
+                     (float2*)nullptr, SliceList{nullptr, nullptr}, SliceSel{0, nullptr, nullptr, 0u, 0u, nullptr, nullptr, nullptr},
+                     (uint32_t*)nullptr, 0);
 }
 void launch_preprocess_cull(const RasterParams& p, const float* means, const float* scales, const float* rots,
                             uint32_t* tiles_touched, int32_t* radii, int32_t* out_radii, uint32_t* zero_words, int zero_n,
-                            uint8_t* zbin, float2* uv, hipStream_t st) {
+                            uint8_t* zbin, float2* uv, uint32_t* hist_words, hipStream_t st) {
   if (p.P == 0) return;
   hipLaunchKernelGGL(preprocess_fwd_kernel<1>, dim3((p.P + 255) / 256), dim3(256), 0, st, p, means, (const float*)nullptr,
                      (const float*)nullptr, scales, rots, (const float*)nullptr, (const int32_t*)nullptr, (Splat*)nullptr,
                      tiles_touched, radii, (uint8_t*)nullptr, out_radii, zero_words, zero_n, zbin, uv,
-                     SliceList{nullptr, nullptr}, SliceSel{0, nullptr, nullptr, 0u, 0u, nullptr, nullptr, nullptr});
+                     SliceList{nullptr, nullptr}, SliceSel{0, nullptr, nullptr, 0u, 0u, nullptr, nullptr, nullptr},
+                     hist_words, hist_words ? CULL_HIST_WORDS : 0);
 }
 void launch_preprocess_shade(const RasterParams& p, const float* means, const float* opac, const float* shs,
                              const float* scales, const float* rots, const float* normal_w, Splat* splats,
@@ -625,8 +657,142 @@
   const size_t n = list.ids ? (max_items < (size_t)p.P ? max_items : (size_t)p.P) : (size_t)p.P;
   hipLaunchKernelGGL(preprocess_fwd_kernel<2>, dim3((unsigned)((n + 255) / 256)), dim3(256), 0, st, p, means, opac, shs,
                      scales, rots, normal_w, (const int32_t*)nullptr, splats, (uint32_t*)nullptr, radii, clamped,
-                     (int32_t*)nullptr, (uint32_t*)nullptr, 0, (uint8_t*)nullptr, uv, list, sel);
-}
+                     (int32_t*)nullptr, (uint32_t*)nullptr, 0, (uint8_t*)nullptr, uv, list, sel, (uint32_t*)nullptr, 0);
+}
+constexpr int RECULL_ROWS = 1024;
+struct RecullArgs {
+  RasterParams p;
+  const float *means, *scales, *rots;
+  uint32_t* tiles_touched; int32_t* radii; int32_t* out_radii; uint8_t* zbin; float2* uv;
+  uint32_t* hist; unsigned long long* cover;
+  uint8_t* marks;
+  const float* view_copy;
+  uint32_t* zero_words; int zero_n;
+  int fail_idx;
+  BwdInfoInit bi;
+};
+__global__ void __launch_bounds__(256) recull_rows_kernel(RecullArgs a) {
+  __shared__ uint32_t s_h[SLICE_BINS], s_c[SLICE_BINS], s_r[SLICE_BINS];
+  __shared__ uint16_t s_list[RECULL_ROWS];
+  __shared__ uint32_t s_n;
+  const int tid = threadIdx.x;
+  const bool differs = tid < 16 && __float_as_uint(a.p.view[tid]) != __float_as_uint(a.view_copy[tid]);
+  s_h[tid] = 0; s_c[tid] = 0; s_r[tid] = 0;
+  if (tid == 0) s_n = 0;
+  const uint32_t moved = __syncthreads_or(differs ? 1 : 0) ? 1u : 0u;
+  if (a.bi.dst && blockIdx.x == 0 && tid == 0) {
+    a.bi.dst->slot_grads = a.bi.slot_grads; a.bi.dst->slots = a.bi.slots; a.bi.dst->use_slots = a.bi.use_slots;
+  }
+  {
+    const int nv = a.zero_n >> 2, stride = (int)gridDim.x * 256;
+    uint4* z4 = reinterpret_cast<uint4*>(a.zero_words);
+    for (int t = (int)blockIdx.x * 256 + tid; t < nv; t += stride) {
+      uint4 w = make_uint4(0u, 0u, 0u, 0u);
+      const int d = a.fail_idx - 4 * t;
+      if (d >= -1 && d < 4) {
+        if (d == 0 || d == -1) w.x = moved;
+        if (d == 1 || d == 0) w.y = moved;
+        if (d == 2 || d == 1) w.z = moved;
+        if (d == 3 || d == 2) w.w = moved;
+      }
+      z4[t] = w;
+    }
+    for (int t = 4 * nv + (int)blockIdx.x * 256 + tid; t < a.zero_n; t += stride)
+      a.zero_words[t] = (t == a.fail_idx || t == a.fail_idx + 1) ? moved : 0u;
+  }
+  if (moved) return;
+  const int P = a.p.P;
+  const int row0 = (int)blockIdx.x * RECULL_ROWS + tid * 4;
+  if (row0 < P) {
+    uint32_t* m4 = reinterpret_cast<uint32_t*>(a.marks + row0);
+    const uint32_t m = *m4;
+    if (m != 0u) {
+      uint32_t bits = 0;
+#pragma unroll
+      for (int k = 0; k < 4; ++k) bits |= (((m >> (8 * k)) & 0xffu) != 0u ? 1u : 0u) << k;
+      uint32_t at = atomicAdd(&s_n, (uint32_t)__popc(bits));
+      while (bits) {
+        const int k = __ffs((int)bits) - 1;
+        bits &= bits - 1u;
+        s_list[at++] = (uint16_t)(tid * 4 + k);
+      }
+      *m4 = 0u;
+    }
+  }
+  __syncthreads();
+  const int n = (int)s_n;
+  for (int q = tid; q < n; q += 256) {
+    const int i = (int)blockIdx.x * RECULL_ROWS + (int)s_list[q];
+    if (i >= P) continue;
+    const uint32_t zb0 = a.zbin[i], ar0 = a.tiles_touched[i], r0 = (uint32_t)min(a.radii[i], 256);
+    uint32_t zb = 255u, ar = 0u, r = 0u;
+    CullGeom cg;
+    if (cull_geom<true>(a.p, a.means, a.scales, a.rots, nullptr, i, cg)) {
+      cull_store(cg, i, a.tiles_touched, a.radii, a.out_radii, a.zbin, a.uv);
+      zb = slice_bin_of(cg.pcz); ar = (uint32_t)cg.touched; r = (uint32_t)min(cg.radius, 256);
+    } else if (zb0 != 255u) {
+      a.tiles_touched[i] = 0; a.radii[i] = 0;
+      if (a.out_radii) a.out_radii[i] = 0;
+      a.zbin[i] = 255;
+    }
+    if (zb != zb0 || ar != ar0 || r != r0) {
+      if (zb0 != 255u) { atomicSub(&s_h[zb0], ar0); atomicSub(&s_c[zb0], 1u); atomicSub(&s_r[zb0], r0 * r0); }
+      if (zb != 255u) { atomicAdd(&s_h[zb], ar); atomicAdd(&s_c[zb], 1u); atomicAdd(&s_r[zb], r * r); }
+    }
+  }
+  __syncthreads();
+  if (n > 0) {
+    const uint32_t dh = s_h[tid], dc = s_c[tid], dr = s_r[tid];
+    if (dh) atomicAdd(&a.hist[tid], dh);
+    if (dc) atomicAdd(&a.hist[SLICE_BINS + tid], dc);
+    if (dr) atomicAdd(&a.cover[tid], (unsigned long long)(long long)(int32_t)dr);
+  }
+}
+void launch_recull_rows(const RasterParams& p, const float* means, const float* scales, const float* rots,
+                        uint32_t* tiles_touched, int32_t* radii, int32_t* out_radii, uint32_t* zero_words, int zero_n,
+                        uint8_t* zbin, float2* uv, uint32_t* hist, unsigned long long* cover, uint8_t* marks,
+                        const float* view_copy, int fail_idx, BwdInfoInit bi, hipStream_t st) {
+  if (p.P == 0) return;
+  const RecullArgs a{p, means, scales, rots, tiles_touched, radii, out_radii, zbin, uv, hist, cover, marks, view_copy,
+                     zero_words, zero_n, fail_idx, bi};
+  hipLaunchKernelGGL(recull_rows_kernel, dim3((p.P + RECULL_ROWS - 1) / RECULL_ROWS), dim3(256), 0, st, a);
+}
+
+struct CullCheckArgs {
+  int P;
+  const uint32_t *tt_a, *tt_b; const int32_t *rad_a, *rad_b, *orad_a, *orad_b; const uint8_t *zb_a, *zb_b;
+  const uint2 *uv_a, *uv_b; const uint32_t *hist_a, *hist_b;
+  const uint32_t* skip;
+  unsigned long long* mismatches;
+};
+__global__ void __launch_bounds__(256) cull_check_kernel(CullCheckArgs a) {
+  if (*a.skip != 0u) return;
+  uint32_t bad = 0;
+  const int stride = (int)gridDim.x * 256;
+  for (int i = (int)blockIdx.x * 256 + (int)threadIdx.x; i < a.P; i += stride) {
+    bad += a.tt_a[i] != a.tt_b[i]; bad += a.rad_a[i] != a.rad_b[i]; bad += a.zb_a[i] != a.zb_b[i];
+    if (a.orad_a) bad += a.orad_a[i] != a.orad_b[i];
+    const uint2 x = a.uv_a[i], y = a.uv_b[i];
+    bad += x.x != y.x; bad += x.y != y.y;
+  }
+  if (blockIdx.x == 0)
+    for (int t = (int)threadIdx.x; t < CULL_HIST_WORDS; t += 256) bad += a.hist_a[t] != a.hist_b[t];
+#pragma unroll
+  for (int off = 32; off > 0; off >>= 1) bad += (uint32_t)__shfl_xor((int)bad, off);
+  if ((threadIdx.x & 63) == 0 && bad) atomicAdd(a.mismatches, (unsigned long long)bad);
+}
+void launch_cull_check(int P, const uint32_t* tt_a, const uint32_t* tt_b, const int32_t* rad_a, const int32_t* rad_b,
+                       const int32_t* orad_a, const int32_t* orad_b, const uint8_t* zb_a, const uint8_t* zb_b,
+                       const float2* uv_a, const float2* uv_b, const uint32_t* hist_a, const uint32_t* hist_b,
+                       const uint32_t* skip, unsigned long long* mismatches, hipStream_t st) {
+  if (P == 0) return;
+  int blocks = (P + 255) / 256;
+  if (blocks > 1024) blocks = 1024;
+  const CullCheckArgs a{P, tt_a, tt_b, rad_a, rad_b, orad_a, orad_b, zb_a, zb_b, (const uint2*)uv_a, (const uint2*)uv_b,
+                        hist_a, hist_b, skip, mismatches};
+  hipLaunchKernelGGL(cull_check_kernel, dim3(blocks), dim3(256), 0, st, a);
+}
+
 void launch_emit_keys(const RasterParams& p, const Splat* splats, const int32_t* radii, const uint32_t* offsets,
                       const int32_t* mask, uint64_t* keys, uint32_t* vals, hipStream_t st) {
   if (p.P == 0) return;
@@ -658,9 +824,9 @@
   if (threadIdx.x == 0) {
     const uint32_t L = (uint32_t)(s_l[0] + s_l[1] + s_l[2] + s_l[3]), F = (uint32_t)(s_f[0] + s_f[1] + s_f[2] + s_f[3]);
     ctr[0] = L; ctr[1] = F;
-    if (spec_fail) *spec_fail = L != 0u ? 1u : 0u;
+    if (spec_fail) *spec_fail = (L != 0u || *spec_fail != 0u) ? 1u : 0u;
     const uint32_t R1 = seg_count ? (uint32_t)(s_i[0] + s_i[1] + s_i[2] + s_i[3]) : r1[0];
-    const uint32_t w[7] = {ctr[2], 0u, L, F, R1, 0u, 0u};
+    const uint32_t w[7] = {ctr[2], 0u, L, F, R1, ctr[7], 0u};
     publish_to_host(host, w, seq);
   }
 }
diff --git a/rtg_slam_amd/map_optim.py b/rtg_slam_amd/map_optim.py
--- a/rtg_slam_amd/map_optim.py
+++ b/rtg_slam_amd/map_optim.py
@@ -193,6 +193,8 @@
         self._scope = "local"
         self._lr_scope = None
         self.version = 0
+        self._map_epoch = 0
+        self._epoch_seen = None
         self._gd_views = {}
         self._adam_dirty = None
         self._frozen_version = 0
@@ -635,6 +637,7 @@
         dev = st["xyz"]["p"].device
         if N == 0:
             raise RuntimeError("step_slam() on an empty map")
+        epoch = self._next_map_epoch()
         self.version += 1
         if self._scope == "global":
             self._frozen_version += 1
@@ -700,7 +703,9 @@
             C.pointer(attach) if attach is not None else None, P(confidence) if confidence is not None else None,
             int(self._act_valid), geom.cb, None, binning.cb, None, img.cb, None,
             float(normal_weight) if gt_normal is not None else 0.0, P(gt_normal) if gt_normal is not None else None,
-            int(nf), int(N), int(self.tail_mode), P(self.live_counts) if self.live_counts is not None else None)
+            int(nf), int(N), int(self.tail_mode), P(self.live_counts) if self.live_counts is not None else None,
+            int(epoch) if (self.world == 1 and not tile_band) else 0)
+        self._epoch_seen = self._epoch_state()
         R = C.c_int64(0)
         stream = torch.cuda.current_stream(dev).cuda_stream
         if tile_band and self.world > 1:
@@ -725,6 +730,16 @@
         self.last_num_rendered = int(R.value)
         self.last_losses = ws["loss"]
         return ws["loss"][0]
+
+    def _next_map_epoch(self) -> int:
+        same = (self.world == 1 and self._epoch_seen is not None and self._slam_ws is not None and self._act_valid
+                and self._epoch_seen == self._epoch_state())
+        if not same:
+            self._map_epoch += 1
+        return self._map_epoch
+
+    def _epoch_state(self):
+        return (int(self.version), id(self._slam_ws), self._scope, int(self.N), int(self.n_frozen))
 
     def band_tile_mask(self, tile_mask: torch.Tensor, with_region: bool = False):
         on = (tile_mask.reshape(-1) != 0)
diff --git a/rtg_slam_amd/rasterizer.py b/rtg_slam_amd/rasterizer.py
--- a/rtg_slam_amd/rasterizer.py
+++ b/rtg_slam_amd/rasterizer.py
@@ -76,6 +76,17 @@
         out = (C.c_int64 * 3)()
         _lib.check(_lib.load().rtgs_raster_speculation_stats_ctx(self.ptr, out), "rtgs_raster_speculation_stats")
         return dict(speculative=int(out[0]), failed=int(out[1]), not_eligible=int(out[2]))
+
+    def set_cull_cache(self, enable: bool):
+        _lib.load().rtgs_raster_set_cull_cache_ctx(self.ptr, int(bool(enable)))
+
+    def set_cull_cache_check(self, enable: bool):
+        _lib.load().rtgs_raster_set_cull_cache_check_ctx(self.ptr, int(bool(enable)))
+
+    def cull_cache_stats(self):
+        out = (C.c_int64 * 5)()
+        _lib.check(_lib.load().rtgs_raster_cull_cache_stats_ctx(self.ptr, out), "rtgs_raster_cull_cache_stats")
+        return dict(hits=int(out[0]), full=int(out[1]), disarmed=int(out[2]), view_redos=int(out[3]), check_mismatches=int(out[4]))
 
     def set_plain_onepass(self, enable: bool):
         _lib.load().rtgs_raster_set_plain_onepass_ctx(self.ptr, int(bool(enable)))
```

Measured after the change: 2807 units/s (median of 6 runs). 1.06x the previous value.
